# lppllppl920/EndoscopyDepthEstimation-Pytorch

Hardware: AMD Instinct MI355X
Metric: train frame-pairs/sec at 256x320 bs=8 (higher is better)
Workload: dtype f32

## Files before the change

endoscopydepthestimation-pytorch_amd/csrc/dgrad_wino_kernels.h:

```cpp
#pragma once

#include "dgrad_block_kernels.h"

namespace endo {

constexpr int kWinoDgradSlice = 16 * 12 * 16;
constexpr int kWinoDgradMaxLayers = 48;

struct WinoDgradTable {
    int layers;
    int start[kWinoDgradMaxLayers + 1];
    int cin[kWinoDgradMaxLayers];
    int groups[kWinoDgradMaxLayers];
    int64_t w_off[kWinoDgradMaxLayers];
    int64_t u_off[kWinoDgradMaxLayers];
};

static __global__ void __launch_bounds__(256) dgrad_wino_weights_kernel(const WinoDgradTable t, const float* __restrict__ params, float* __restrict__ u,
                                                                 int layout1_blocks = 0) {
    const int total = t.start[t.layers];
    for (int item = blockIdx.x * blockDim.x + threadIdx.x; item < total; item += gridDim.x * blockDim.x) {
        int l = 0;
        while (item >= t.start[l + 1]) ++l;
        const int e = item - t.start[l];
        const int j = e & 15, c = (e >> 4) % 12, grp = (e >> 4) / 12;
        const int ci = grp * 16 + j;
        float g[3][3];
#pragma unroll
        for (int a = 0; a < 3; ++a)
#pragma unroll
            for (int b = 0; b < 3; ++b) g[a][b] = 0.f;
        if (ci < t.cin[l]) {
            const float* src = params + t.w_off[l] + (static_cast<int64_t>(c) * t.cin[l] + ci) * 9;
#pragma unroll
            for (int a = 0; a < 3; ++a)
#pragma unroll
                for (int b = 0; b < 3; ++b) g[a][b] = src[(2 - a) * 3 + (2 - b)];
        }
        float h[4][3];
#pragma unroll
        for (int b = 0; b < 3; ++b) {
            h[0][b] = g[0][b];
            h[1][b] = 0.5f * (g[0][b] + g[1][b] + g[2][b]);
            h[2][b] = 0.5f * (g[0][b] - g[1][b] + g[2][b]);
            h[3][b] = g[2][b];
        }
        if ((layout1_blocks >> (l >> 2)) & 1) {
            float* dst = u + t.u_off[l] + static_cast<int64_t>(grp) * kWinoDgradSlice + (c * 64 + j) * 4;
#pragma unroll
            for (int a = 0; a < 4; ++a)
                *reinterpret_cast<f32x4*>(dst + a * 64) = f32x4{h[a][0], 0.5f * (h[a][0] + h[a][1] + h[a][2]), 0.5f * (h[a][0] - h[a][1] + h[a][2]), h[a][2]};
            continue;
        }
        float* dst = u + t.u_off[l] + static_cast<int64_t>(grp) * kWinoDgradSlice + c * 16 + j;
#pragma unroll
        for (int a = 0; a < 4; ++a) {
            dst[(4 * a + 0) * 192] = h[a][0];
            dst[(4 * a + 1) * 192] = 0.5f * (h[a][0] + h[a][1] + h[a][2]);
            dst[(4 * a + 2) * 192] = 0.5f * (h[a][0] - h[a][1] + h[a][2]);
            dst[(4 * a + 3) * 192] = h[a][2];
        }
    }
}

template <int NL>
struct DgradWino8Geom {
    static constexpr int kThreads = 512;
    static constexpr int kTileX = 32, kTileY = 8;
    static constexpr int kRows = kTileY + 2, kCols = kTileX + 2;
    static constexpr int kPlane = kRows * kCols;
    static constexpr int kCS = 352;
    static_assert(kCS >= kPlane && kCS % 64 == 32, "dY map stride");
    static constexpr int kU = kWinoDgradSlice;
    static constexpr int kUUnits = kU / 4;
    static constexpr int kRed = 4 * 16 * 2;
    static constexpr size_t kBytes = sizeof(float) * (NL * 12 * kCS + 2 * 2 * kU + 2 * 2 * kRed);
    static_assert(kBytes <= 160 * 1024, "one block per CU");
};

template <int NL, int EXP = 0>
__global__ void __launch_bounds__(512, 2) dgrad_wino8_kernel(const DgradBlockParams p0, const float* __restrict__ u0, const float* __restrict__ u1,
                                                             const float* __restrict__ u2, const float* __restrict__ u3) {
    using G = DgradWino8Geom<NL>;
    typedef float f32x2 __attribute__((ext_vector_type(2)));
    const int grp = p0.group_n > 0 ? blockIdx.z / p0.group_n : 0;
    const int n = blockIdx.z - grp * p0.group_n;
    const DgradBlockParams& p = p0;
    const int64_t grp_off = grp * p0.gs;
    extern __shared__ __attribute__((aligned(16))) float smem[];
    float* s_g = smem;
    float* s_u = s_g + NL * 12 * G::kCS;
    float* s_red = s_u + 4 * G::kU;

    const int tid = threadIdx.x;
    const int lane = tid & 63;
    const int wave = __builtin_amdgcn_readfirstlane(tid >> 6);
    const int half = wave >> 2, w4 = wave & 3;
    const int th = tid & 255;
    const int li = lane & 15;
    const int lk = lane >> 4;
    const int tile = (gridDim.x & 7) == 0 ? xcd_remap(blockIdx.x, gridDim.x) : blockIdx.x;
    const int x0 = (tile % p.tiles_x) * G::kTileX;
    const int y0 = (tile / p.tiles_x) * G::kTileY;
    const int px = x0 + 8 * lk;
    const int py = y0 + 2 * w4;
    const int ngroups = p.count / 16;
    const int g_per = (ngroups + gridDim.y - 1) / gridDim.y;
    const int g_begin = blockIdx.y * g_per;
    const int g_end = min(ngroups, g_begin + g_per);
    if (g_begin >= g_end) return;
    const int npairs = (g_end - g_begin + 1) / 2;
    const int nsteps = npairs * NL;
    const float* const u_layer[4] = {u0, u1, u2, u3};

    {
        int goff = 0;
        bool ok = false;
        if (tid < G::kPlane) {
            const int ry = tid / G::kCols, rx = tid - ry * G::kCols;
            const int gy = y0 - 1 + ry, gx = x0 - 1 + rx;
            if (gy >= 0 && gy < p.h && gx >= 0 && gx < p.w) { ok = true; goff = gy * p.g_w + gx; }
        }
        const float* g_n = p.g + grp_off + n * p.g_ns;
        const int e0 = wave * 64;
        if (e0 < G::kPlane) {
            for (int c = 0; c < NL * 12; ++c) {
                const float* src = ok ? g_n + static_cast<int64_t>(c) * p.g_cs + goff : g_pad_consts + 4;
                if (e0 + lane < G::kPlane) __builtin_amdgcn_global_load_lds((gptr_t)src, (lptr_t)(s_g + c * G::kCS + e0), 4, 0, 0);
            }
        }
    }

    auto step_group = [&](int step) { return g_begin + 2 * (step / NL) + half; };
    auto issue_weights = [&](int step, int buf) {
        const int gq = step_group(step), l = step % NL;
        if (gq >= g_end) return;
        const float* src = u_layer[l] + static_cast<int64_t>(gq) * G::kU + 4 * th;
        float* dst = s_u + (half * 2 + buf) * G::kU + w4 * 256;
#pragma unroll
        for (int k = 0; k < 3; ++k)
            __builtin_amdgcn_global_load_lds((gptr_t)(src + k * 1024), (lptr_t)(dst + k * 1024), 16, 0, 0);
    };

    const float* x_n = p.x + grp_off + n * p.ns;
    float* out_n = p.out + grp_off + n * p.ns;
    f32x4 xc[2][2], dc[2][2], total[2][2];
#pragma unroll
    for (int r = 0; r < 2; ++r)
#pragma unroll
        for (int hh = 0; hh < 2; ++hh) total[r][hh] = f32x4{0.f, 0.f, 0.f, 0.f};
    issue_weights(0, 0);
    asm volatile("s_waitcnt vmcnt(0)" ::: "memory");
    __syncthreads();

    for (int step = 0; step < nsteps; ++step) {
        const int buf = step & 1;
        const int gq = step_group(step), l = step % NL;
        const bool active = gq < g_end;
        const bool last_layer = (l == NL - 1);
        const int co = gq * 16 + li;
        float scale = 0.f, beta = 0.f, mean = 0.f, rstd = 0.f;
        if (active) {
            if (l == 0) {
#pragma unroll
                for (int r = 0; r < 2; ++r)
#pragma unroll
                    for (int hh = 0; hh < 2; ++hh) {
                        const int64_t o = static_cast<int64_t>(co) * p.cs + static_cast<int64_t>(py + r) * p.w + px + 4 * hh;
                        if constexpr ((EXP & 1) != 0) {
                            xc[r][hh] = f32x4{0.1f * lane, 0.2f, -0.3f, 0.4f}; dc[r][hh] = f32x4{0.f, 0.f, 0.f, 0.f};
                        } else {
                            xc[r][hh] = *reinterpret_cast<const f32x4*>(x_n + o);
                            dc[r][hh] = co >= p.acc_from ? *reinterpret_cast<const f32x4*>(out_n + o) : f32x4{0.f, 0.f, 0.f, 0.f};
                        }
                    }
            }
            mean = p.saved[l][grp_off + 2 * co]; rstd = p.saved[l][grp_off + 2 * co + 1];
            scale = p.gamma[l][co] * rstd;
            beta = p.beta[l][co];
        }
        if (step + 1 < nsteps && (!(EXP & 8) || step == 0)) issue_weights(step + 1, buf ^ 1);
        if (active) {
            f32x4 acc[16];
            const float* ub = s_u + (half * 2 + buf) * G::kU;
#pragma unroll
            for (int quad = 0; quad < 3; ++quad) {
                const float* a_base = s_g + (l * 12 + quad * 4 + lk) * G::kCS + (2 * w4) * G::kCols + 2 * li;
                const float* b_base = ub + (quad * 4 + lk) * 16 + li;
                f32x2 lo[4], hi[4];
#pragma unroll
                for (int row = 0; row < 4; ++row) {
                    lo[row] = *reinterpret_cast<const f32x2*>(a_base + row * G::kCols);
                    hi[row] = *reinterpret_cast<const f32x2*>(a_base + row * G::kCols + 2);
                }
                f32x2 tl[4], th2[4];
                tl[0] = lo[0] - lo[2]; th2[0] = hi[0] - hi[2];
                tl[1] = lo[1] + lo[2]; th2[1] = hi[1] + hi[2];
                tl[2] = lo[2] - lo[1]; th2[2] = hi[2] - hi[1];
                tl[3] = lo[1] - lo[3]; th2[3] = hi[1] - hi[3];
#pragma unroll
                for (int a = 0; a < 4; ++a) {
                    const float c0 = tl[a][0], c1 = tl[a][1], c2 = th2[a][0], c3 = th2[a][1];
                    float v0 = c0 - c2, v1 = c1 + c2, v2 = c2 - c1, v3 = c1 - c3;
                    if constexpr ((EXP & 64) != 0) { v0 = lo[a][0]; v1 = lo[a][1]; v2 = hi[a][0]; v3 = hi[a][1]; }
                    const float b0 = b_base[(4 * a + 0) * 192], b1 = b_base[(4 * a + 1) * 192];
                    const float b2 = b_base[(4 * a + 2) * 192], b3 = b_base[(4 * a + 3) * 192];
                    if constexpr ((EXP & 32) != 0) {
                        if (quad == 0) {
                            acc[4 * a + 0] = f32x4{v0 * b0, 0.f, 0.f, 0.f}; acc[4 * a + 1] = f32x4{v1 * b1, 0.f, 0.f, 0.f};
                            acc[4 * a + 2] = f32x4{v2 * b2, 0.f, 0.f, 0.f}; acc[4 * a + 3] = f32x4{v3 * b3, 0.f, 0.f, 0.f};
                        } else {
                            acc[4 * a + 0][quad] += v0 * b0; acc[4 * a + 1][quad] += v1 * b1;
                            acc[4 * a + 2][quad] += v2 * b2; acc[4 * a + 3][quad] += v3 * b3;
                        }
                    } else
                    if (quad == 0) {
                        const f32x4 zero = {0.f, 0.f, 0.f, 0.f};
                        acc[4 * a + 0] = __builtin_amdgcn_mfma_f32_16x16x4f32(v0, b0, zero, 0, 0, 0);
                        acc[4 * a + 1] = __builtin_amdgcn_mfma_f32_16x16x4f32(v1, b1, zero, 0, 0, 0);
                        acc[4 * a + 2] = __builtin_amdgcn_mfma_f32_16x16x4f32(v2, b2, zero, 0, 0, 0);
                        acc[4 * a + 3] = __builtin_amdgcn_mfma_f32_16x16x4f32(v3, b3, zero, 0, 0, 0);
                    } else {
                        acc[4 * a + 0] = __builtin_amdgcn_mfma_f32_16x16x4f32(v0, b0, acc[4 * a + 0], 0, 0, 0);
                        acc[4 * a + 1] = __builtin_amdgcn_mfma_f32_16x16x4f32(v1, b1, acc[4 * a + 1], 0, 0, 0);
                        acc[4 * a + 2] = __builtin_amdgcn_mfma_f32_16x16x4f32(v2, b2, acc[4 * a + 2], 0, 0, 0);
                        acc[4 * a + 3] = __builtin_amdgcn_mfma_f32_16x16x4f32(v3, b3, acc[4 * a + 3], 0, 0, 0);
                    }
                }
            }
            float s1 = 0.f, s2 = 0.f;
            if constexpr ((EXP & 128) != 0) {
#pragma unroll
                for (int r = 0; r < 2; ++r)
#pragma unroll
                    for (int hh = 0; hh < 2; ++hh)
#pragma unroll
                        for (int k = 0; k < 4; ++k)
                            total[r][hh][k] += acc[4 * (2 * r + hh) + k][0] + acc[4 * (2 * r + hh) + k][1] + acc[4 * (2 * r + hh) + k][2] + acc[4 * (2 * r + hh) + k][3] + xc[r][hh][k] * scale;
                s1 = total[0][0][0]; s2 = mean + beta;
            } else
#pragma unroll
            for (int e = 0; e < 4; ++e) {
                float u0r[4], u1r[4];
#pragma unroll
                for (int c = 0; c < 4; ++c) {
                    const float m0 = acc[c][e], m1 = acc[4 + c][e], m2 = acc[8 + c][e], m3 = acc[12 + c][e];
                    u0r[c] = m0 + m1 + m2;
                    u1r[c] = m1 - m2 - m3;
                }
                const float d[2][2] = {{u0r[0] + u0r[1] + u0r[2], u0r[1] - u0r[2] - u0r[3]},
                                       {u1r[0] + u1r[1] + u1r[2], u1r[1] - u1r[2] - u1r[3]}};
#pragma unroll
                for (int r = 0; r < 2; ++r)
#pragma unroll
                    for (int cx = 0; cx < 2; ++cx) {
                        const int hh = e >> 1, k = 2 * (e & 1) + cx;
                        const float xcen = xc[r][hh][k] - mean;
                        const float z = fmaf(xcen, scale, beta);
                        const float dz = z > 0.f ? d[r][cx] : 0.f;
                        s1 += dz;
                        s2 = fmaf(dz, xcen, s2);
                        total[r][hh][k] = fmaf(dz, scale, total[r][hh][k]);
                    }
            }
            if (last_layer) {
#pragma unroll
                for (int r = 0; r < 2; ++r)
#pragma unroll
                    for (int hh = 0; hh < 2; ++hh) {
                        f32x4 o = dc[r][hh];
#pragma unroll
                        for (int k = 0; k < 4; ++k) o[k] += total[r][hh][k];
                        if constexpr ((EXP & 2) != 0) asm volatile("" ::"v"(o[0]), "v"(o[1]), "v"(o[2]), "v"(o[3]));
                        else
                        *reinterpret_cast<f32x4*>(out_n + static_cast<int64_t>(co) * p.cs + static_cast<int64_t>(py + r) * p.w + px + 4 * hh) = o;
                        total[r][hh] = f32x4{0.f, 0.f, 0.f, 0.f};
                    }
            }
            s2 *= rstd;
            s1 += __shfl_xor(s1, 16, 64); s1 += __shfl_xor(s1, 32, 64);
            s2 += __shfl_xor(s2, 16, 64); s2 += __shfl_xor(s2, 32, 64);
            if (lk == 0) {
                float* red = s_red + (buf * 2 + half) * G::kRed;
                red[(w4 * 16 + li) * 2] = s1;
                red[(w4 * 16 + li) * 2 + 1] = s2;
            }
        }
        if (!(EXP & 16) || step + 1 >= nsteps) {
            asm volatile("s_waitcnt vmcnt(0)" ::: "memory");
            __syncthreads();
        }
        if (!(EXP & 4) && active && th < 32) {
            const int j = th >> 1, which = th & 1;
            const int cj = gq * 16 + j;
            const float* red = s_red + (buf * 2 + half) * G::kRed;
            double t = 0.0;
            for (int wv = 0; wv < 4; ++wv) t += static_cast<double>(red[(wv * 16 + j) * 2 + which]);
            atomicAdd(p.scratch[l] + bn_slot_offset(p.slot_stride) + grp_off / 2 + 2 * cj + which, t);
        }
    }
}

inline bool dgrad_wino_ok(const DgradBlockParams& p) {
    return dgrad_block_ok(p) && (p.w % 32 == 0) && (p.h % 8 == 0) && (p.count % 16 == 0) && p.count >= 32;
}

template <int NL, int EXP = 0>
inline int launch_dgrad_wino8(DgradBlockParams p, const float* const (&u)[4], hipStream_t stream) {
    using G = DgradWino8Geom<NL>;
    p.tiles_x = p.w / G::kTileX;
    const int tiles_y = p.h / G::kTileY;
    return launch_dyn(dgrad_wino8_kernel<NL, EXP>, dim3(p.tiles_x * tiles_y, 1, p.n), G::kThreads, G::kBytes, stream, p, u[0], u[1], u[2], u[3]);
}

}
```

endoscopydepthestimation-pytorch_amd/csrc/net.hip:

```cpp
#include <new>
#include <vector>

#include "dgrad_kernels.h"
#include "dgrad_block_kernels.h"
#include "dgrad_newmap_kernels.h"
#include "td_dgrad_kernels.h"
#include "td_fwd_kernels.h"
#include "wgrad_taps_kernels.h"
#include "wgrad1x1_kernels.h"
#include "wgrad_nsplit_kernels.h"
#include "wgrad_f34_kernels.h"
#include "wgrad_subpix_kernels.h"
#include "wino_fwd_kernels.h"
#include "wino4_fwd_kernels.h"
#include "dgrad_wino_kernels.h"
#include "dgrad_wino3_kernels.h"


namespace endo {

int run_dgrad_wino3_nl4(const DgradBlockParams& p, const float* const* u, hipStream_t stream);
bool dgrad_wino3p_applies(const DgradBlockParams& p);
int run_dgrad_wino3p_nl4(const DgradBlockParams& p, const float* const* u, int blocks, double* fw_parts, int* blocks_used, hipStream_t stream);

constexpr int kGrowth = 12;
constexpr int kLayers = 4;
constexpr int kFirst = 48;
constexpr int kLevels = 5;
constexpr int kNew = kGrowth * kLayers;
constexpr float kBnEps = 1.0e-5f;
constexpr float kBnMomentum = 0.1f;
constexpr int kSideStreamFromLevel = 0;

struct ConvP { int64_t w, b; int cout, cin, ks; int64_t u; int64_t ud; };
struct BnP { int64_t g, b; int c; int64_t run; int64_t saved; };

struct Table {
    ConvP first, final_;
    ConvP down_conv[kLevels][kLayers], td_conv[kLevels], bott_conv[kLayers], tu_conv[kLevels], up_conv[kLevels][kLayers];
    BnP down_bn[kLevels][kLayers], td_bn[kLevels], bott_bn[kLayers], up_bn[kLevels][kLayers];
    std::vector<int64_t> param_offsets;
    std::vector<BnP*> bn_order;
    int64_t param_floats = 0, bn_floats = 0, bn_width_total = 0;
    WinoWeightTable wino;
    WinoWeightTable wino4;
    int64_t wino4_floats = 0;
    int64_t wino_floats = 0;
    WinoDgradTable wino_dgrad;
    int64_t wino_dgrad_floats = 0;
};

inline int down_in(int level) { return kFirst + kNew * level; }
inline int level_channels(int level) { return level < kLevels ? 144 + down_in(level) : 288 + kNew; }

static const Table& table() {
    static Table* t = [] {
        Table* tb = new Table();
        int64_t off = 0;
        auto conv = [&](ConvP& c, int cout, int cin, int ks) {
            c.cout = cout; c.cin = cin; c.ks = ks; c.u = -1; c.ud = -1;
            c.w = off; tb->param_offsets.push_back(off); off += static_cast<int64_t>(cout) * cin * ks * ks;
            c.b = off; tb->param_offsets.push_back(off); off += cout;
        };
        int64_t run = 0, saved = 0;
        auto bn = [&](BnP& b, int c) {
            b.c = c;
            b.g = off; tb->param_offsets.push_back(off); off += c;
            b.b = off; tb->param_offsets.push_back(off); off += c;
            b.run = run; run += 2 * c;
            b.saved = saved; saved += c;
            tb->bn_order.push_back(&b);
        };
        conv(tb->first, kFirst, 3, 3);
        for (int l = 0; l < kLevels; ++l)
            for (int j = 0; j < kLayers; ++j) { bn(tb->down_bn[l][j], down_in(l) + kGrowth * j); conv(tb->down_conv[l][j], kGrowth, down_in(l) + kGrowth * j, 3); }
        for (int l = 0; l < kLevels; ++l) { bn(tb->td_bn[l], down_in(l) + kNew); conv(tb->td_conv[l], down_in(l) + kNew, down_in(l) + kNew, 1); }
        for (int j = 0; j < kLayers; ++j) { bn(tb->bott_bn[j], 288 + kGrowth * j); conv(tb->bott_conv[j], kGrowth, 288 + kGrowth * j, 3); }
        for (int i = 0; i < kLevels; ++i) conv(tb->tu_conv[i], kNew, kNew, 3);
        for (int i = 0; i < kLevels; ++i) {
            const int l = kLevels - 1 - i;
            for (int j = 0; j < kLayers; ++j) { const int cin = 96 + down_in(l) + kGrowth * j; bn(tb->up_bn[i][j], cin); conv(tb->up_conv[i][j], kGrowth, cin, 3); }
        }
        conv(tb->final_, 1, 192, 1);
        tb->param_floats = off;
        tb->bn_floats = run;
        tb->bn_width_total = saved;
        {
            WinoWeightTable& wt = tb->wino;
            wt.layers = 0; wt.start[0] = 0;
            int64_t uoff = 0;
            auto add = [&](ConvP& c) {
                const int l = wt.layers++;
                c.u = uoff;
                wt.cin[l] = c.cin; wt.cout[l] = c.cout; wt.w_off[l] = c.w; wt.u_off[l] = uoff;
                wt.start[l + 1] = wt.start[l] + c.cin * 16;
                uoff += static_cast<int64_t>(c.cin) * kWinoUStride;
            };
            for (int l = 0; l < kLevels; ++l) for (int j = 0; j < kLayers; ++j) add(tb->down_conv[l][j]);
            for (int j = 0; j < kLayers; ++j) add(tb->bott_conv[j]);
            for (int i = 0; i < kLevels; ++i) for (int j = 0; j < kLayers; ++j) add(tb->up_conv[i][j]);
            tb->wino_floats = uoff;
            tb->wino4 = wt;
            int64_t u4 = 0;
            for (int l = 0; l < wt.layers; ++l) { tb->wino4.u_off[l] = u4; u4 += static_cast<int64_t>(wt.cin[l]) * kW4UStride; }
            tb->wino4_floats = u4;
        }
        {
            WinoDgradTable& wd = tb->wino_dgrad;
            wd.layers = 0; wd.start[0] = 0;
            int64_t uoff = 0;
            auto add = [&](ConvP& c, int base) {
                const int l = wd.layers++;
                c.ud = uoff;
                wd.cin[l] = c.cin; wd.groups[l] = base / 16; wd.w_off[l] = c.w; wd.u_off[l] = uoff;
                wd.start[l + 1] = wd.start[l] + 16 * wd.groups[l] * 12;
                uoff += static_cast<int64_t>(wd.groups[l]) * kWinoDgradSlice;
            };
            for (int l = 0; l < kLevels; ++l) for (int j = 0; j < kLayers; ++j) add(tb->down_conv[l][j], down_in(l));
            for (int j = 0; j < kLayers; ++j) add(tb->bott_conv[j], 288);
            for (int i = 0; i < kLevels; ++i) for (int j = 0; j < kLayers; ++j) add(tb->up_conv[i][j], 96 + down_in(kLevels - 1 - i));
            tb->wino_dgrad_floats = uoff;
        }
        return tb;
    }();
    return *t;
}

}

using namespace endo;

namespace endo { struct FwdPlan; struct BwdPlan; }

struct endo_net {
    int n, h, w;
    int groups;
    int64_t gs;
    struct Level { int h, w, t; int64_t plane; int64_t act, grad; int64_t sums; int64_t pq; } lv[kLevels + 1];
    int64_t pre_off;
    int64_t saved_off;
    int64_t idx_off[kLevels];
    int64_t sums_off;
    int64_t sums_bytes;
    int64_t tape_floats;
    int64_t partial_off;
    int64_t wino_off;
    int64_t wino4_off;
    int64_t pq_off;
    int64_t pq_floats;
    int64_t scratch_off;
    int64_t scratch_bytes;
    int64_t slot_stride;
    int64_t wg_scratch_off;
    int64_t tuw_scratch_off;
    int64_t wd_off;
    int64_t gplane_off;
    int64_t bias_parts_off;
    int64_t fw_parts_off;
    int64_t bias_parts_floats;
    int64_t gradws_floats;
    hipStream_t wstream;
    hipEvent_t ev_fork, ev_join;
    int opt[ENDO_OPT_COUNT];
    FwdPlan* last_fwd;
    BwdPlan* last_bwd;
};

namespace endo {


constexpr int kBiasPartChannels = 2048;
constexpr int kBiasPartLaunches = 64;
constexpr int kFwPartBlocks = 512;
struct BiasReduceTable {
    int n;
    struct Entry { const float* parts; float* bias; int count; int nparts; } e[kBiasPartLaunches];
};
struct BiasParts {
    BiasReduceTable table;
    int64_t used;
};

struct BnFin4 {
    const double* scratch[4];
    const float* saved[4];
    const float* gamma[4];
    float* ggamma[4];
    float* gbeta[4];
};

__global__ void __launch_bounds__(256) prep_dy_kernel(float* __restrict__ dbuf, const float* __restrict__ x, int64_t ns, int plane,
                                                      const float* __restrict__ pq_p, const float* __restrict__ pq_q,
                                                      float* bias_grad, int group_n, int64_t gs, const BnFin4 fin, int nl,
                                                      double count, int training, int64_t slot_stride,
                                                      const float* __restrict__ vg, const float* __restrict__ vw, float* __restrict__ parts) {
    __shared__ double scratch[4];
    const int c = blockIdx.y;
    const int grp = blockIdx.z / group_n, n = blockIdx.z - grp * group_n;
    float pc = pq_p[grp * gs + c], qc = pq_q[grp * gs + c];
    if (nl > 0) {
        const int64_t go = grp * gs;
        double dp = 0.0, dq = 0.0;
#pragma unroll
        for (int j = 0; j < 4; ++j) {
            if (j >= nl) break;
            const double s1 = bn_slot_sum(fin.scratch[j] + go / 2 + 2 * c, slot_stride);
            const double s2 = bn_slot_sum(fin.scratch[j] + go / 2 + 2 * c + 1, slot_stride);
            if (blockIdx.x == 0 && n == 0 && threadIdx.x == 0) {
                atomicAdd(fin.ggamma[j] + c, static_cast<float>(s2));
                atomicAdd(fin.gbeta[j] + c, static_cast<float>(s1));
            }
            if (training) {
                const double mean = fin.saved[j][go + 2 * c], rstd = fin.saved[j][go + 2 * c + 1];
                const double scale = fin.gamma[j][c] * rstd;
                const double k = scale * rstd * s2 / count;
                dp += static_cast<double>(static_cast<float>(-k));
                dq += static_cast<double>(static_cast<float>(-scale * s1 / count + k * mean));
            }
        }
        pc += static_cast<float>(dp);
        qc += static_cast<float>(dq);
    }
    const int64_t base = grp * gs + n * ns + static_cast<int64_t>(c) * plane;
    const float* vg_n = vg ? vg + grp * gs + static_cast<int64_t>(n) * plane : nullptr;
    const float wf = vg ? vw[c] : 0.f;
    float part = 0.f;
    if ((plane & 3) == 0 && !vg_n) {
        const int stride = gridDim.x * blockDim.x * 4;
        int i = (blockIdx.x * blockDim.x + threadIdx.x) * 4;
        for (; i + stride < plane; i += 2 * stride) {
            f32x4 g0 = *reinterpret_cast<const f32x4*>(dbuf + base + i);
            f32x4 g1 = *reinterpret_cast<const f32x4*>(dbuf + base + i + stride);
            const f32x4 x0 = *reinterpret_cast<const f32x4*>(x + base + i);
            const f32x4 x1 = *reinterpret_cast<const f32x4*>(x + base + i + stride);
#pragma unroll
            for (int e = 0; e < 4; ++e) { g0[e] += fmaf(pc, x0[e], qc); part += g0[e]; }
#pragma unroll
            for (int e = 0; e < 4; ++e) { g1[e] += fmaf(pc, x1[e], qc); part += g1[e]; }
            *reinterpret_cast<f32x4*>(dbuf + base + i) = g0;
            *reinterpret_cast<f32x4*>(dbuf + base + i + stride) = g1;
        }
        for (; i < plane; i += stride) {
            f32x4 g = *reinterpret_cast<const f32x4*>(dbuf + base + i);
            const f32x4 xv = *reinterpret_cast<const f32x4*>(x + base + i);
#pragma unroll
            for (int e = 0; e < 4; ++e) { g[e] += fmaf(pc, xv[e], qc); part += g[e]; }
            *reinterpret_cast<f32x4*>(dbuf + base + i) = g;
        }
    } else if ((plane & 3) == 0) {
        for (int i = (blockIdx.x * blockDim.x + threadIdx.x) * 4; i < plane; i += gridDim.x * blockDim.x * 4) {
            f32x4 g;
            if (vg_n) {
                const f32x4 gv = *reinterpret_cast<const f32x4*>(vg_n + i);
                g = f32x4{gv[0] * wf, gv[1] * wf, gv[2] * wf, gv[3] * wf};
            } else {
                g = *reinterpret_cast<const f32x4*>(dbuf + base + i);
            }
            const f32x4 xv = *reinterpret_cast<const f32x4*>(x + base + i);
#pragma unroll
            for (int e = 0; e < 4; ++e) { g[e] += fmaf(pc, xv[e], qc); part += g[e]; }
            *reinterpret_cast<f32x4*>(dbuf + base + i) = g;
        }
    } else {
        for (int i = blockIdx.x * blockDim.x + threadIdx.x; i < plane; i += gridDim.x * blockDim.x) {
            const float g = (vg_n ? vg_n[i] * wf : dbuf[base + i]) + fmaf(pc, x[base + i], qc);
            dbuf[base + i] = g;
            part += g;
        }
    }
    const int lane = threadIdx.x & 63, wave = threadIdx.x >> 6;
    double v = wave_sum(static_cast<double>(part));
    if (lane == 0) scratch[wave] = v;
    __syncthreads();
    if (threadIdx.x == 0 && bias_grad) {
        const float t = static_cast<float>(scratch[0] + scratch[1] + scratch[2] + scratch[3]);
        if (parts) parts[(static_cast<int64_t>(c) * gridDim.z + blockIdx.z) * gridDim.x + blockIdx.x] = t;
        else atomicAdd(bias_grad + c, t);
    }
}

__global__ void __launch_bounds__(256) bias_reduce_kernel(const BiasReduceTable tb) {
    const BiasReduceTable::Entry& e = tb.e[blockIdx.x];
    const int lane = threadIdx.x & 63, wave = threadIdx.x >> 6;
    for (int c = blockIdx.y * 4 + wave; c < e.count; c += gridDim.y * 4) {
        const float* src = e.parts + static_cast<int64_t>(c) * e.nparts;
        double t = 0.0;
        for (int i = lane; i < e.nparts; i += 64) t += static_cast<double>(src[i]);
        t = wave_sum(t);
        if (lane == 0) e.bias[c] += static_cast<float>(t);
    }
}

__global__ void bn_bwd_finalize_kernel(const double* __restrict__ scratch, const float* __restrict__ saved,
                                       const float* __restrict__ gamma, float* __restrict__ ggamma, float* __restrict__ gbeta,
                                       float* __restrict__ pq_p, float* __restrict__ pq_q, int c_count, double count, int training,
                                       int64_t gs, int64_t slot_stride) {
    scratch += blockIdx.y * (gs / 2); saved += blockIdx.y * gs; pq_p += blockIdx.y * gs; pq_q += blockIdx.y * gs;
    for (int c = blockIdx.x * blockDim.x + threadIdx.x; c < c_count; c += gridDim.x * blockDim.x) {
        const double s1 = bn_slot_sum(scratch + 2 * c, slot_stride), s2 = bn_slot_sum(scratch + 2 * c + 1, slot_stride);
        atomicAdd(ggamma + c, static_cast<float>(s2));
        atomicAdd(gbeta + c, static_cast<float>(s1));
        if (training) {
            const double mean = saved[2 * c], rstd = saved[2 * c + 1];
            const double scale = gamma[c] * rstd;
            const double k = scale * rstd * s2 / count;
            pq_p[c] += static_cast<float>(-k);
            pq_q[c] += static_cast<float>(-scale * s1 / count + k * mean);
        }
    }
}

__global__ void bn_bwd_finalize4_kernel(const BnFin4 a, int nl, float* __restrict__ pq_p, float* __restrict__ pq_q, int c_count, double count,
                                        int training, int64_t gs, int64_t slot_stride) {
    const int64_t go = blockIdx.y * gs;
    pq_p += go; pq_q += go;
    for (int c = blockIdx.x * blockDim.x + threadIdx.x; c < c_count; c += gridDim.x * blockDim.x) {
        double dp = 0.0, dq = 0.0;
#pragma unroll
        for (int j = 0; j < 4; ++j) {
            if (j >= nl) break;
            const double s1 = bn_slot_sum(a.scratch[j] + go / 2 + 2 * c, slot_stride);
            const double s2 = bn_slot_sum(a.scratch[j] + go / 2 + 2 * c + 1, slot_stride);
            atomicAdd(a.ggamma[j] + c, static_cast<float>(s2));
            atomicAdd(a.gbeta[j] + c, static_cast<float>(s1));
            if (training) {
                const double mean = a.saved[j][go + 2 * c], rstd = a.saved[j][go + 2 * c + 1];
                const double scale = a.gamma[j][c] * rstd;
                const double k = scale * rstd * s2 / count;
                dp += static_cast<double>(static_cast<float>(-k));
                dq += static_cast<double>(static_cast<float>(-scale * s1 / count + k * mean));
            }
        }
        if (training) {
            pq_p[c] += static_cast<float>(dp);
            pq_q[c] += static_cast<float>(dq);
        }
    }
}

__global__ void tu_phase_weights_kernel(const float* __restrict__ w, int cout, int cin, float* __restrict__ out) {
    constexpr int kPhW = 2 * 12 * 16 + 16;
    const int total = 2 * cin * 2 * 12 * 16;
    for (int i = blockIdx.x * blockDim.x + threadIdx.x; i < total; i += gridDim.x * blockDim.x) {
        const int lane16 = i & 15;
        const int slot = (i >> 4) % 12;
        const int t = (i / (16 * 12)) & 1;
        const int ci = (i / (16 * 12 * 2)) % cin;
        const int a = i / (16 * 12 * 2 * cin);
        int ctap, tile;
        if (slot < 3) { ctap = 0; tile = slot; } else if (slot < 9) { ctap = 1; tile = slot - 3; } else { ctap = 2; tile = slot - 9 + 3; }
        const int b = tile / 3, co = (tile % 3) * 16 + lane16;
        float v = 0.f;
        if (co < cout) {
            const float* src = w + (static_cast<int64_t>(co) * cin + ci) * 9;
            const int ky0 = a == 0 ? (t == 0 ? 0 : 1) : (t == 0 ? 0 : 2), ky1 = a == 0 ? (t == 0 ? 0 : 2) : (t == 0 ? 1 : 2);
            int kx0, kx1;
            if (b == 0) { kx0 = ctap == 0 ? 0 : 1; kx1 = ctap == 0 ? 0 : 2; }
            else { kx0 = ctap == 1 ? 0 : 2; kx1 = ctap == 1 ? 1 : 2; }
            for (int ky = ky0; ky <= ky1; ++ky)
                for (int kx = kx0; kx <= kx1; ++kx) v += src[ky * 3 + kx];
        }
        out[(static_cast<int64_t>(a) * cin + ci) * kPhW + (t * 12 + slot) * 16 + lane16] = v;
    }
}

__global__ void tu_subpix_dgrad_weights_kernel(const float* __restrict__ w, int cout, int cin, float* __restrict__ out) {
    const int pitch = 4 * cin + 16;
    const int total = 4 * cout * 4 * cin;
    for (int i = blockIdx.x * blockDim.x + threadIdx.x; i < total; i += gridDim.x * blockDim.x) {
        const int ci = i % cin;
        const int tap = (i / cin) & 3;
        const int co = (i / (4 * cin)) % cout;
        const int ph = i / (4 * cin * cout);
        const int alpha = ph >> 1, beta = ph & 1, tyi = tap >> 1, txi = tap & 1;
        const int ky0 = alpha == 0 ? (tyi == 0 ? 1 : 0) : (tyi == 0 ? 2 : 0), ky1 = alpha == 0 ? (tyi == 0 ? 2 : 0) : (tyi == 0 ? 2 : 1);
        const int kx0 = beta == 0 ? (txi == 0 ? 1 : 0) : (txi == 0 ? 2 : 0), kx1 = beta == 0 ? (txi == 0 ? 2 : 0) : (txi == 0 ? 2 : 1);
        const float* src = w + (static_cast<int64_t>(co) * cin + ci) * 9;
        float v = 0.f;
        for (int ky = ky0; ky <= ky1; ++ky)
            for (int kx = kx0; kx <= kx1; ++kx) v += src[ky * 3 + kx];
        out[static_cast<int64_t>(ph * cout + co) * pitch + tap * cin + ci] = v;
    }
}

__global__ void __launch_bounds__(256) finalize_partial_kernel(const float* __restrict__ partial, int64_t split_stride, int ksplit,
                                                               int64_t pns, int plane, const float* __restrict__ bias,
                                                               float* __restrict__ out, int64_t out_ns, double* out_sums,
                                                               int group_n, int64_t gs) {
    __shared__ double scratch[2 * 4];
    const int c = blockIdx.y;
    const int grp = blockIdx.z / group_n, n = blockIdx.z - grp * group_n;
    partial += grp * gs; out += grp * gs;
    if (out_sums) out_sums += grp * (gs / 2);
    const float b = bias[c];
    float part[2] = {0.f, 0.f};
    for (int i = blockIdx.x * blockDim.x + threadIdx.x; i < plane; i += gridDim.x * blockDim.x) {
        float v = b;
        for (int s = 0; s < ksplit; ++s) v += partial[s * split_stride + n * pns + static_cast<int64_t>(c) * plane + i];
        out[n * out_ns + static_cast<int64_t>(c) * plane + i] = v;
        part[0] += v;
        part[1] += v * v;
    }
    if (out_sums) block_sum_atomic<2>(part, out_sums + 2 * c, scratch);
}

__global__ void __launch_bounds__(256) final_fwd_kernel(const float* __restrict__ u, int64_t ns, int plane, int cin,
                                                        const float* __restrict__ wgt, const float* __restrict__ bias,
                                                        float* __restrict__ pre, float* __restrict__ out, int group_n, int64_t gs, int c_first) {
    __shared__ float s_w[192];
    for (int c = threadIdx.x; c < cin; c += blockDim.x) s_w[c] = wgt[c];
    __syncthreads();
    const int grp = blockIdx.y / group_n, n = blockIdx.y - grp * group_n;
    u += grp * gs;
    if (pre) pre += grp * gs;
    out += static_cast<int64_t>(grp) * group_n * plane;
    const bool vec = (plane & 3) == 0;
    if (vec) {
        for (int i = (blockIdx.x * blockDim.x + threadIdx.x) * 4; i < plane; i += gridDim.x * blockDim.x * 4) {
            f32x4 acc = {0.f, 0.f, 0.f, 0.f};
            if (c_first > 0) acc = *reinterpret_cast<const f32x4*>(pre + static_cast<int64_t>(n) * plane + i);
            const float* src = u + n * ns + i;
            for (int c = c_first; c < cin; ++c) {
                const f32x4 v = *reinterpret_cast<const f32x4*>(src + static_cast<int64_t>(c) * plane);
                const float wc = s_w[c];
                acc[0] = fmaf(v[0], wc, acc[0]); acc[1] = fmaf(v[1], wc, acc[1]);
                acc[2] = fmaf(v[2], wc, acc[2]); acc[3] = fmaf(v[3], wc, acc[3]);
            }
            const float b = bias[0];
            f32x4 o;
            for (int e = 0; e < 4; ++e) { acc[e] += b; o[e] = fabsf(acc[e]); }
            if (pre) *reinterpret_cast<f32x4*>(pre + static_cast<int64_t>(n) * plane + i) = acc;
            *reinterpret_cast<f32x4*>(out + static_cast<int64_t>(n) * plane + i) = o;
        }
    } else {
        for (int i = blockIdx.x * blockDim.x + threadIdx.x; i < plane; i += gridDim.x * blockDim.x) {
            float acc = c_first > 0 ? pre[static_cast<int64_t>(n) * plane + i] : 0.f;
            for (int c = c_first; c < cin; ++c) acc = fmaf(u[n * ns + static_cast<int64_t>(c) * plane + i], s_w[c], acc);
            acc += bias[0];
            if (pre) pre[static_cast<int64_t>(n) * plane + i] = acc;
            out[static_cast<int64_t>(n) * plane + i] = fabsf(acc);
        }
    }
}

__device__ __forceinline__ float sign_of(float v) { return v > 0.f ? 1.f : (v < 0.f ? -1.f : 0.f); }

__global__ void __launch_bounds__(256) final_g_kernel(const float* __restrict__ gout, const float* __restrict__ pre, float* __restrict__ g,
                                                      int plane, int group_n, int64_t gs) {
    const int grp = blockIdx.y / group_n, n = blockIdx.y - grp * group_n;
    gout += static_cast<int64_t>(blockIdx.y) * plane; pre += grp * gs + static_cast<int64_t>(n) * plane; g += grp * gs + static_cast<int64_t>(n) * plane;
    for (int i = blockIdx.x * blockDim.x + threadIdx.x; i < plane; i += gridDim.x * blockDim.x) g[i] = gout[i] * sign_of(pre[i]);
}

__global__ void __launch_bounds__(256) final_bwd_data_kernel(const float* __restrict__ gout, const float* __restrict__ pre,
                                                             const float* __restrict__ wgt, float* __restrict__ dbuf,
                                                             int64_t ns, int plane, int cin, int group_n, int64_t gs, int c_first) {
    __shared__ float s_w[192];
    for (int c = threadIdx.x; c < cin; c += blockDim.x) s_w[c] = wgt[c];
    __syncthreads();
    const int grp = blockIdx.y / group_n, n = blockIdx.y - grp * group_n;
    gout += static_cast<int64_t>(grp) * group_n * plane; pre += grp * gs; dbuf += grp * gs;
    for (int i = blockIdx.x * blockDim.x + threadIdx.x; i < plane; i += gridDim.x * blockDim.x) {
        const float g = gout[static_cast<int64_t>(n) * plane + i] * sign_of(pre[static_cast<int64_t>(n) * plane + i]);
        for (int c = c_first; c < cin; ++c) dbuf[n * ns + static_cast<int64_t>(c) * plane + i] = g * s_w[c];
    }
}

__global__ void __launch_bounds__(256) final_bwd_weight_kernel(const float* __restrict__ gout, const float* __restrict__ pre,
                                                               const float* __restrict__ u, int64_t ns, int plane, int cin,
                                                               int group_n, int64_t gs, float* __restrict__ gw, float* __restrict__ gb, int c_first) {
    __shared__ double scratch[4];
    const int c = c_first + blockIdx.x;
    const int grp = blockIdx.z / group_n, n = blockIdx.z - grp * group_n;
    const float* gp = gout + static_cast<int64_t>(blockIdx.z) * plane;
    const float* pp = pre + grp * gs + static_cast<int64_t>(n) * plane;
    const float* up = u + grp * gs + n * ns + static_cast<int64_t>(c < cin ? c : 0) * plane;
    float part = 0.f, part2 = 0.f;
    if ((plane & 3) == 0) {
        const int stride = gridDim.y * blockDim.x * 4;
        for (int i = (blockIdx.y * blockDim.x + threadIdx.x) * 4; i < plane; i += stride) {
            const f32x4 gv = *reinterpret_cast<const f32x4*>(gp + i);
            const f32x4 pv = *reinterpret_cast<const f32x4*>(pp + i);
            f32x4 uv = {1.f, 1.f, 1.f, 1.f};
            if (c < cin) uv = *reinterpret_cast<const f32x4*>(up + i);
            part += gv[0] * sign_of(pv[0]) * uv[0] + gv[1] * sign_of(pv[1]) * uv[1];
            part2 += gv[2] * sign_of(pv[2]) * uv[2] + gv[3] * sign_of(pv[3]) * uv[3];
        }
    } else {
        for (int i = blockIdx.y * blockDim.x + threadIdx.x; i < plane; i += gridDim.y * blockDim.x)
            part += gp[i] * sign_of(pp[i]) * (c < cin ? up[i] : 1.f);
    }
    const int lane = threadIdx.x & 63, wave = threadIdx.x >> 6;
    double v = wave_sum(static_cast<double>(part + part2));
    if (lane == 0) scratch[wave] = v;
    __syncthreads();
    if (threadIdx.x == 0) {
        const float t = static_cast<float>(scratch[0] + scratch[1] + scratch[2] + scratch[3]);
        if (c < cin) atomicAdd(gw + c, t); else atomicAdd(gb, t);
    }
}

__global__ void __launch_bounds__(64) final_w_reduce_kernel(const double* __restrict__ parts, int nblocks, int count, float* __restrict__ gw) {
    const int c = blockIdx.x;
    double t = 0.0;
    for (int b = threadIdx.x; b < nblocks; b += 64) t += parts[static_cast<int64_t>(b) * count + c];
    t = wave_sum(t);
    if (threadIdx.x == 0) atomicAdd(gw + c, static_cast<float>(t));
}

constexpr int kBlocks = 2 * kLevels + 1, kDense = kBlocks * kLayers;

enum class DenseFwd { Wino4, Wino2_32x16, Wino2_32x8, SplitK, Direct32x8, Direct16x8, DirectAuto };
struct FwdPlan {
    struct Dense {
        DenseFwd form;
        int ksplit;
        bool chunk_weights;
    } dense[kDense];
    bool bf16;
    bool wino4_weights;
    bool fuse_final;
    bool td_persistent[kLevels];
    bool tu_subpix[kLevels];
};

enum class NewMap { Bf16, Persistent, Vec16, Dword };
enum class BasePass { Block8, Block8Bf16, Wino3, Wino3Persistent, Wino8 };
enum class DenseWgrad { F34, NSplit, Taps, Direct };
enum class TdDgrad { Persistent, Runs128, Dma, Staged };
enum class TuWgrad { Subpix, Taps, Direct };
enum class TuDgrad { Subpix32x8, Subpix16x8, Subpix16x4, Plain };
enum class FirstWgrad { F34Prep, F34, Taps, Direct };
struct BwdPlan {
    struct Block {
        bool fused;
        NewMap newmap[kLayers];
        BasePass base;
        bool wino3_layout;
    } block[kBlocks];
    DenseWgrad wgrad[kDense];
    bool td_wgrad_dma[kLevels];
    TdDgrad td_dgrad[kLevels];
    TuWgrad tu_wgrad[kLevels];
    TuDgrad tu_dgrad[kLevels];
    int overlap;
    bool bf16_wgrad, bf16_dgrad;
    bool dgrad_weights;
    bool use_virt;
    bool virt_base;
    bool virt_base_w;
    int materialise;
    int c_first;
    FirstWgrad first;
};

struct Ctx {
    const endo_net* net;
    const float* params;
    float* bn_running;
    float* tape;
    float* grads;
    float* gradws;
    int training;
    hipStream_t stream;
    BiasParts* bias_parts = nullptr;
    const float* x = nullptr;
    const FwdPlan* fwd = nullptr;
    const BwdPlan* bwd = nullptr;

    int nt() const { return net->n * net->groups; }
    int fork_wgrad(Ctx& side, int level) const {
        side = *this;
        if (!net->wstream || !bwd->overlap || level < kSideStreamFromLevel) return 0;
        ENDO_CHECK(hipEventRecord(net->ev_fork, stream));
        ENDO_CHECK(hipStreamWaitEvent(net->wstream, net->ev_fork, 0));
        side.stream = net->wstream;
        return 0;
    }
    float* act(int level) const { return tape + net->lv[level].act; }
    float* gbuf(int level) const { return gradws + net->lv[level].grad; }
    double* sums(int level) const { return reinterpret_cast<double*>(reinterpret_cast<char*>(tape) + net->sums_off) + net->lv[level].sums; }
    double* out_sums(int level, int channel) const { return training ? sums(level) + 2 * channel : nullptr; }
    float* saved(const BnP& b) const { return tape + net->saved_off + 2 * b.saved; }
    double* scratch(const BnP& b) const { return reinterpret_cast<double*>(reinterpret_cast<char*>(gradws) + net->scratch_off) + 2 * b.saved; }
    float* pq_p(int level) const { return gradws + net->pq_off + 2 * net->lv[level].pq; }
    float* pq_q(int level) const { return pq_p(level) + net->lv[level].t; }
    uint8_t* idx(int level) const { return reinterpret_cast<uint8_t*>(tape) + net->idx_off[level]; }
};

static void fill_bn_in(const Ctx& c, ConvParams& p, const BnP& b, int level, int ic0) {
    const auto& lv = c.net->lv[level];
    p.in_sums = c.sums(level) + 2 * ic0;
    p.gamma = c.params + b.g;
    p.beta = c.params + b.b;
    p.running_mean = c.bn_running + b.run;
    p.running_var = c.bn_running + b.run + b.c;
    p.saved = c.tape ? c.saved(b) : nullptr;
    p.count = static_cast<double>(c.net->n) * lv.h * lv.w;
    p.eps = kBnEps;
    p.momentum = kBnMomentum;
    p.training = c.training;
}

static void fill_in(const Ctx& c, ConvParams& p, const float* base, int level, int ic0, int cin) {
    const auto& lv = c.net->lv[level];
    p.in = base + ic0 * lv.plane;
    p.in_ns = lv.t * lv.plane;
    p.in_cs = static_cast<int>(lv.plane);
    p.in_w = lv.w;
    p.cin = cin;
}

static void fill_out(const Ctx& c, ConvParams& p, float* base, int level, int oc0, int cout) {
    const auto& lv = c.net->lv[level];
    p.out = base + oc0 * lv.plane;
    p.out_ns = lv.t * lv.plane;
    p.out_cs = static_cast<int>(lv.plane);
    p.out_w = lv.w;
    p.cout = cout;
}

static void fill_grid(const Ctx& c, ConvParams& p, int level) {
    const auto& lv = c.net->lv[level];
    p.n = c.nt(); p.h = lv.h; p.w = lv.w;
    p.group_n = c.net->n; p.gs = c.net->gs; p.in_gs = c.net->gs; p.out_gs = c.net->gs;
}

static double conv_flops(const endo_net* net, int level, int cin, int cout, int ks) {
    return 2.0 * net->n * net->groups * net->lv[level].plane * cin * cout * ks * ks;
}

static void default_options(int (&opt)[ENDO_OPT_COUNT]) {
    opt[ENDO_OPT_WINO_FWD] = 5;
    opt[ENDO_OPT_WINO_DGRAD] = 3;
    opt[ENDO_OPT_DGRAD_VEC] = 2;
    opt[ENDO_OPT_WINO_MIN_TILES] = 1024;
    opt[ENDO_OPT_MFMA_BF16] = 0;
    opt[ENDO_OPT_WGRAD_OVERLAP] = 1;
    opt[ENDO_OPT_WGRAD_F34] = 1;
    opt[ENDO_OPT_FINAL_VIRTUAL] = 1;
    opt[ENDO_OPT_TD_PERSIST] = 3;
    opt[ENDO_OPT_CHIP_DIVISOR] = 1;
}
static long chip_divisor(const endo_net* net) { const int d = net->opt[ENDO_OPT_CHIP_DIVISOR]; return d < 1 ? 1 : d; }
static int persistent_cus(const endo_net* net) { const int cus = static_cast<int>(device_cu_count() / chip_divisor(net)); return cus < 1 ? 1 : cus; }
static int bf16_mask(const int* opt) { const int v = opt[ENDO_OPT_MFMA_BF16]; return v == 1 ? 7 : (v >> 1); }

struct DenseBlock { int level, ic0, c0; const BnP* bn; const ConvP* cv; bool base_overwrite; };
static DenseBlock dense_block(int b) {
    const Table& tb = table();
    if (b < kLevels) return {b, 48, down_in(b), tb.down_bn[b], tb.down_conv[b], false};
    if (b == kLevels) return {kLevels, 0, 288, tb.bott_bn, tb.bott_conv, true};
    const int i = b - kLevels - 1, l = kLevels - 1 - i;
    return {l, 0, 96 + down_in(l), tb.up_bn[i], tb.up_conv[i], l > 0};
}
static long tile_count(const Ctx& c, int level, int tx, int ty) {
    const auto& lv = c.net->lv[level];
    return static_cast<long>((lv.w + tx - 1) / tx) * ((lv.h + ty - 1) / ty) * c.nt() * chip_divisor(c.net);
}

static ConvParams dense_fwd_params(const Ctx& c, const DenseBlock& k, int j, DenseFwd form) {
    const ConvP& cv = k.cv[j];
    const int oc0 = k.ic0 + k.c0 + kGrowth * j;
    ConvParams p{};
    fill_grid(c, p, k.level);
    fill_in(c, p, c.act(k.level), k.level, k.ic0, cv.cin);
    fill_bn_in(c, p, k.bn[j], k.level, k.ic0);
    p.wgt = c.params + cv.w; p.bias = c.params + cv.b; p.w_cout = cv.cout; p.w_cin = cv.cin;
    fill_out(c, p, c.act(k.level), k.level, oc0, cv.cout);
    p.out_sums = c.out_sums(k.level, oc0);
    if (form == DenseFwd::Wino4) p.wgt = c.tape + c.net->wino4_off + cv.u / kWinoUStride * kW4UStride;
    if (form == DenseFwd::Wino2_32x16 || form == DenseFwd::Wino2_32x8) p.wgt = c.tape + c.net->wino_off + cv.u;
    return p;
}

static ConvParams td_fwd_params(const Ctx& c, int level) {
    const BnP& b = table().td_bn[level];
    const ConvP& cv = table().td_conv[level];
    const int next = level + 1;
    const int oc0 = next < kLevels ? 48 : 0;
    ConvParams p{};
    fill_grid(c, p, level);
    fill_in(c, p, c.act(level), level, 48, cv.cin);
    fill_bn_in(c, p, b, level, 48);
    p.wgt = c.params + cv.w; p.bias = c.params + cv.b; p.w_cout = cv.cout; p.w_cin = cv.cin;
    fill_out(c, p, c.act(next), next, oc0, cv.cout);
    p.out_idx = c.idx(level);
    p.idx_ns = static_cast<int64_t>(cv.cout) * c.net->lv[next].plane;
    p.out_sums = c.out_sums(next, oc0);
    return p;
}

static FwdPlan plan_fwd(const Ctx& c) {
    const int* opt = c.net->opt;
    const int mode = opt[ENDO_OPT_WINO_FWD];
    const long min_tiles = opt[ENDO_OPT_WINO_MIN_TILES];
    FwdPlan pl{};
    pl.bf16 = (bf16_mask(opt) & 2) != 0;
    pl.wino4_weights = !pl.bf16 && mode == 5;
    for (int b = 0; b < kBlocks; ++b) {
        const DenseBlock k = dense_block(b);
        const long t64x16 = tile_count(c, k.level, 64, 16), t32x16 = tile_count(c, k.level, 32, 16), t32x8 = tile_count(c, k.level, 32, 8);
        const long t16x16 = tile_count(c, k.level, 16, 16), t16x8 = tile_count(c, k.level, 16, 8);
        const bool big = t32x16 >= min_tiles, small = t32x8 >= (min_tiles * 3) / 4;
        const bool wino4_tiles = mode == 5 && !pl.bf16 && 2 * t64x16 >= min_tiles;
        const bool wino2_tiles = mode != 0 && !pl.bf16 && (big || small);
        for (int j = 0; j < kLayers; ++j) {
            FwdPlan::Dense& d = pl.dense[b * kLayers + j];
            const int nchunks = (k.cv[j].cin + 15) / 16;
            d.chunk_weights = !pl.bf16 && !wino4_tiles && !wino2_tiles;
            if (wino4_tiles && wino4_fwd_ok(dense_fwd_params(c, k, j, DenseFwd::Wino4))) {
                d.form = DenseFwd::Wino4;
            } else if (wino2_tiles && wino_fwd_ok(dense_fwd_params(c, k, j, DenseFwd::Wino2_32x16))) {
                d.form = big ? DenseFwd::Wino2_32x16 : DenseFwd::Wino2_32x8;
            } else if (t32x16 < 512 && t16x16 < 384 && t16x8 < 512 && nchunks >= 4) {
                int want = static_cast<int>(((t16x8 < 256 ? 512 : 768) + t16x8 - 1) / t16x8);
                if (want > nchunks) want = nchunks;
                const int per = (nchunks + want - 1) / want;
                d.form = DenseFwd::SplitK;
                d.ksplit = (nchunks + per - 1) / per;
            } else {
                d.form = (t32x16 < 1024 && t32x8 >= 1024) ? DenseFwd::Direct32x8
                       : (t32x16 < 1024 && t16x8 >= 768) ? DenseFwd::Direct16x8 : DenseFwd::DirectAuto;
            }
        }
    }
    pl.fuse_final = opt[ENDO_OPT_FINAL_VIRTUAL] && pl.dense[kDense - 1].form == DenseFwd::Wino4;
    for (int l = 0; l < kLevels; ++l) {
        pl.td_persistent[l] = (opt[ENDO_OPT_TD_PERSIST] & 2) && !pl.bf16 && c.training && td_fwd_ok(td_fwd_params(c, l));
        const ConvP& tu = table().tu_conv[kLevels - 1 - l];
        pl.tu_subpix[l] = c.net->lv[l + 1].w % 4 == 0 && tu.cout == kNew && tu.cin % 4 == 0;
    }
    return pl;
}

static int dense_fwd(const Ctx& c, int b, int j) {
    const DenseBlock k = dense_block(b);
    const FwdPlan::Dense& d = c.fwd->dense[b * kLayers + j];
    const ConvP& cv = k.cv[j];
    const auto& lv = c.net->lv[k.level];
    const int oc0 = k.ic0 + k.c0 + kGrowth * j;
    ConvParams p = dense_fwd_params(c, k, j, d.form);
    ProfScope prof(kProfConv3x3Dense, c.stream, conv_flops(c.net, k.level, cv.cin, cv.cout, 3),
                   4.0 * c.nt() * lv.plane * (cv.cin + cv.cout));
    const float* chunk_weights = d.chunk_weights ? c.tape + c.net->wino_off + cv.u : nullptr;
    const bool bf16 = c.fwd->bf16;
    switch (d.form) {
        case DenseFwd::Wino4:
            if (c.fwd->fuse_final && b == kBlocks - 1 && j == kLayers - 1) { p.fin_w = c.params + table().final_.w + k.ic0; p.fin_out = c.tape + c.net->pre_off; }
            return launch_wino4_fwd(p, c.stream);
        case DenseFwd::Wino2_32x16:
            return launch_wino_fwd<2, 4, 2>(p, c.stream);
        case DenseFwd::Wino2_32x8:
            return launch_wino_fwd<1, 4, 3>(p, c.stream);
        case DenseFwd::SplitK: {
            float* partial = c.tape + c.net->partial_off;
            p.ksplit = d.ksplit;
            p.split_stride = static_cast<int64_t>(c.net->n) * cv.cout * lv.plane;
            p.out = partial; p.out_ns = static_cast<int64_t>(cv.cout) * lv.plane;
            p.bias = nullptr; p.out_sums = nullptr;
            p.wgt_chunks = chunk_weights;
            int rc = bf16 ? launch_conv_dma<3, 16, 1, IN_BNRELU, EPI_FWD, 1, 2, 2, 1, 1>(p, c.stream)
                          : launch_conv_dma<3, 16, 1, IN_BNRELU, EPI_FWD, 1, 2, 2, 1>(p, c.stream);
            if (rc) return rc;
            int bx = static_cast<int>((lv.plane + 255) / 256);
            bx = bx > 8 ? 8 : bx;
            finalize_partial_kernel<<<dim3(bx, cv.cout, c.nt()), 256, 0, c.stream>>>(
                partial, p.split_stride, d.ksplit, p.out_ns, static_cast<int>(lv.plane), c.params + cv.b, c.act(k.level) + oc0 * lv.plane,
                lv.t * lv.plane, c.out_sums(k.level, oc0), c.net->n, c.net->gs);
            ENDO_LAUNCH_CHECK();
            return 0;
        }
        case DenseFwd::Direct32x8:
            return bf16 ? launch_conv_dma<3, 4, 1, IN_BNRELU, EPI_FWD, 2, 4, 2, 1, 1>(p, c.stream) : launch_conv_dma<3, 4, 1, IN_BNRELU, EPI_FWD, 2, 4, 2, 1>(p, c.stream);
        case DenseFwd::Direct16x8:
            return bf16 ? launch_conv_dma<3, 8, 1, IN_BNRELU, EPI_FWD, 1, 2, 2, 1, 1>(p, c.stream) : launch_conv_dma<3, 8, 1, IN_BNRELU, EPI_FWD, 1, 2, 2, 1>(p, c.stream);
        case DenseFwd::DirectAuto:
            if (bf16) return launch_conv_dma_auto<3, 4, 1, IN_BNRELU, EPI_FWD, 8, 2, 1, 1>(p, c.stream);
            p.wgt_chunks = chunk_weights;
            return launch_conv_dma_auto<3, 4, 1, IN_BNRELU, EPI_FWD, 8, 2, 1>(p, c.stream);
    }
    return ENDO_E_BADARG;
}

static int td_fwd(const Ctx& c, int level) {
    const ConvP& cv = table().td_conv[level];
    const ConvParams p = td_fwd_params(c, level);
    ProfScope prof(kProfConv1x1Pool, c.stream, conv_flops(c.net, level, cv.cin, cv.cout, 1),
                   4.0 * c.nt() * c.net->lv[level].plane * (cv.cin + cv.cout / 4.0));
    if (c.fwd->td_persistent[level]) return launch_td_fwd(p, persistent_cus(c.net), c.stream);
    if (c.fwd->bf16) return launch_conv_dma_auto<1, 8, 3, IN_BNRELU, EPI_FWD_POOL, 4, 2, 1, 1>(p, c.stream);
    return launch_conv_dma_auto<1, 8, 3, IN_BNRELU, EPI_FWD_POOL, 4>(p, c.stream);
}

static int tu_fwd(const Ctx& c, int level, int src_level, int src_c0, const ConvP& cv) {
    ProfScope prof(kProfConv3x3Up, c.stream, conv_flops(c.net, level, cv.cin, cv.cout, 3),
                   4.0 * c.nt() * c.net->lv[level].plane * (cv.cin / 4.0 + cv.cout));
    if (c.fwd->tu_subpix[level]) {
        float* w3 = c.tape + c.net->partial_off;
        tu_phase_weights_kernel<<<(2 * cv.cin * 384 + 255) / 256, 256, 0, c.stream>>>(c.params + cv.w, cv.cout, cv.cin, w3);
        ENDO_LAUNCH_CHECK();
        ConvParams p{};
        fill_grid(c, p, src_level);
        fill_in(c, p, c.act(src_level), src_level, src_c0, cv.cin);
        p.wgt = w3; p.w_cout = 2 * cv.cout; p.w_cin = cv.cin;
        p.bias = c.params + cv.b;
        fill_out(c, p, c.act(level), level, 0, cv.cout);
        p.out_sums = c.out_sums(level, 0);
        return launch_conv_dma_vec<3, 4, 6, IN_PLAIN, EPI_FWD, 2, 4, 2, 1, 4, 0, 0, 2>(p, c.stream);
    }
    ConvParams p{};
    fill_grid(c, p, level);
    fill_in(c, p, c.act(src_level), src_level, src_c0, cv.cin);
    p.wgt = c.params + cv.w; p.bias = c.params + cv.b; p.w_cout = cv.cout; p.w_cin = cv.cin;
    fill_out(c, p, c.act(level), level, 0, cv.cout);
    p.out_sums = c.out_sums(level, 0);
    return launch_conv_dma_auto<3, 4, 3, IN_UPSAMPLE, EPI_FWD>(p, c.stream);
}

struct FinalVirt { const float* vg; const float* vw; float* gw; };

static int prep_dy(const Ctx& c, int level, int c0, int count, float* bias_grad, const BnFin4* fin = nullptr, int nl = 0, const FinalVirt* fv = nullptr) {
    const auto& lv = c.net->lv[level];
    BnFin4 none{};
    int bx = static_cast<int>((lv.plane + 4095) / 4096);
    bx = bx < 1 ? 1 : (bx > 32 ? 32 : bx);
    float* parts = nullptr;
    if (bias_grad && c.bias_parts) {
        BiasParts& bp = *c.bias_parts;
        const int64_t need = static_cast<int64_t>(count) * c.nt() * bx;
        if (bp.table.n >= kBiasPartLaunches || bp.used + need > c.net->bias_parts_floats) return ENDO_E_UNSUPPORTED;
        parts = c.gradws + c.net->bias_parts_off + bp.used;
        bp.table.e[bp.table.n++] = {parts, bias_grad, count, c.nt() * bx};
        bp.used += need;
    }
    ProfScope prof(kProfSmall, c.stream, 0.0, 12.0 * c.nt() * lv.plane * count);
    prep_dy_kernel<<<dim3(bx, count, c.nt()), 256, 0, c.stream>>>(c.gbuf(level) + c0 * lv.plane, c.act(level) + c0 * lv.plane,
                                                                     lv.t * lv.plane, static_cast<int>(lv.plane), c.pq_p(level) + c0,
                                                                     c.pq_q(level) + c0, bias_grad, c.net->n, c.net->gs, fin ? *fin : none, fin ? nl : 0,
                                                                     static_cast<double>(c.net->n) * lv.h * lv.w, c.training, c.net->slot_stride,
                                                                     fv ? fv->vg : nullptr, fv ? fv->vw + c0 : nullptr, parts);
    ENDO_LAUNCH_CHECK();
    return 0;
}

static int bn_finalize(const Ctx& c, const BnP& b, int level, int ic0, int first = 0, int count = -1) {
    const auto& lv = c.net->lv[level];
    if (count < 0) count = b.c - first;
    if (count <= 0) return 0;
    ProfScope prof(kProfSmall, c.stream, 0.0, 0.0);
    bn_bwd_finalize_kernel<<<dim3((count + 127) / 128, c.net->groups), 128, 0, c.stream>>>(c.scratch(b) + 2 * first, c.saved(b) + 2 * first, c.params + b.g + first,
                                                                       c.grads + b.g + first, c.grads + b.b + first,
                                                                       c.pq_p(level) + ic0 + first, c.pq_q(level) + ic0 + first, count,
                                                                       static_cast<double>(c.net->n) * lv.h * lv.w, c.training, c.net->gs, c.net->slot_stride);
    ENDO_LAUNCH_CHECK();
    return 0;
}

static void fill_wgrad_grid(const Ctx& c, WgradParams& p, int level) {
    const auto& lv = c.net->lv[level];
    p.n = c.nt(); p.h = lv.h; p.w = lv.w;
    p.group_n = c.net->n; p.gs = c.net->gs; p.in_gs = c.net->gs;
    p.tiles_x = (lv.w + kWgTileX - 1) / kWgTileX;
    p.tiles_y = (lv.h + kWgTileY - 1) / kWgTileY;
}

static WgradParams dense_wgrad_params(const Ctx& c, const DenseBlock& k, int j) {
    const auto& lv = c.net->lv[k.level];
    const BnP& b = k.bn[j];
    const ConvP& cv = k.cv[j];
    const int oc0 = k.ic0 + k.c0 + kGrowth * j;
    WgradParams p{};
    fill_wgrad_grid(c, p, k.level);
    p.in = c.act(k.level) + k.ic0 * lv.plane; p.in_ns = lv.t * lv.plane; p.in_cs = static_cast<int>(lv.plane); p.in_w = lv.w; p.cin = cv.cin;
    p.saved = c.saved(b); p.gamma = c.params + b.g; p.beta = c.params + b.b;
    p.dy = c.gbuf(k.level) + oc0 * lv.plane; p.dy_ns = lv.t * lv.plane; p.dy_cs = static_cast<int>(lv.plane); p.dy_w = lv.w; p.cout = cv.cout;
    p.dw = c.grads + cv.w;
    return p;
}

static void fill_dgrad_block(const Ctx& c, DgradBlockParams& p, int level) {
    const auto& lv = c.net->lv[level];
    p.n = c.nt(); p.h = lv.h; p.w = lv.w;
    p.group_n = c.net->n; p.gs = c.net->gs; p.slot_stride = c.net->slot_stride;
    p.g_ns = lv.t * lv.plane; p.g_cs = static_cast<int>(lv.plane); p.g_w = lv.w;
    p.ns = lv.t * lv.plane; p.cs = static_cast<int>(lv.plane);
}

static DgradBlockParams newmap_params(const Ctx& c, const DenseBlock& k, int j, BnFin4* a = nullptr) {
    const auto& lv = c.net->lv[k.level];
    const int nl = kLayers - j;
    const int t0 = k.c0 + kGrowth * (j - 1);
    DgradBlockParams p{};
    fill_dgrad_block(c, p, k.level);
    p.g = c.gbuf(k.level) + (k.ic0 + k.c0 + kGrowth * j) * lv.plane;
    p.x = c.act(k.level) + (k.ic0 + t0) * lv.plane;
    p.out = c.gbuf(k.level) + (k.ic0 + t0) * lv.plane;
    p.count = kGrowth;
    p.acc_from = 0;
    p.w_ci_off = t0;
    for (int l = 0; l < nl; ++l) {
        const BnP& b = k.bn[j + l];
        p.wgt[l] = c.params + k.cv[j + l].w; p.w_cin[l] = k.cv[j + l].cin;
        p.saved[l] = c.saved(b) + 2 * t0; p.gamma[l] = c.params + b.g + t0; p.beta[l] = c.params + b.b + t0;
        p.scratch[l] = c.scratch(b) + 2 * t0;
        if (a) { a->scratch[l] = p.scratch[l]; a->saved[l] = p.saved[l]; a->gamma[l] = p.gamma[l]; a->ggamma[l] = c.grads + b.g + t0; a->gbeta[l] = c.grads + b.b + t0; }
    }
    return p;
}

static DgradBlockParams base_pass_params(const Ctx& c, const DenseBlock& k) {
    const auto& lv = c.net->lv[k.level];
    DgradBlockParams p{};
    fill_dgrad_block(c, p, k.level);
    p.g = c.gbuf(k.level) + (k.ic0 + k.c0) * lv.plane;
    p.x = c.act(k.level) + k.ic0 * lv.plane;
    p.out = c.gbuf(k.level) + k.ic0 * lv.plane;
    p.count = k.c0;
    p.acc_from = k.base_overwrite ? k.c0 : 0;
    p.w_ci_off = 0;
    for (int j = 0; j < kLayers; ++j) {
        p.wgt[j] = c.params + k.cv[j].w; p.w_cin[j] = k.cv[j].cin;
        p.saved[j] = c.saved(k.bn[j]); p.gamma[j] = c.params + k.bn[j].g; p.beta[j] = c.params + k.bn[j].b;
        p.scratch[j] = c.scratch(k.bn[j]);
    }
    return p;
}

static WgradParams td_wgrad_params(const Ctx& c, int level) {
    const BnP& b = table().td_bn[level];
    const ConvP& cv = table().td_conv[level];
    const int next = level + 1, oc0 = next < kLevels ? 48 : 0;
    const auto& lv = c.net->lv[level];
    const auto& nx = c.net->lv[next];
    WgradParams p{};
    fill_wgrad_grid(c, p, level);
    p.in = c.act(level) + 48 * lv.plane; p.in_ns = lv.t * lv.plane; p.in_cs = static_cast<int>(lv.plane); p.in_w = lv.w; p.cin = cv.cin;
    p.saved = c.saved(b); p.gamma = c.params + b.g; p.beta = c.params + b.b;
    p.dy = c.gbuf(next) + oc0 * nx.plane; p.dy_ns = nx.t * nx.plane; p.dy_cs = static_cast<int>(nx.plane); p.dy_w = nx.w; p.cout = cv.cout;
    p.dy_idx = c.idx(level); p.idx_ns = static_cast<int64_t>(cv.cout) * nx.plane;
    p.dw = c.grads + cv.w;
    return p;
}

static ConvParams td_dgrad_params(const Ctx& c, int level) {
    const BnP& b = table().td_bn[level];
    const ConvP& cv = table().td_conv[level];
    const int next = level + 1, oc0 = next < kLevels ? 48 : 0;
    const auto& lv = c.net->lv[level];
    ConvParams p{};
    fill_grid(c, p, level);
    fill_in(c, p, c.gbuf(next), next, oc0, cv.cout);
    p.in_idx = c.idx(level); p.idx_ns = static_cast<int64_t>(cv.cout) * c.net->lv[next].plane;
    p.wgt = c.params + cv.w; p.w_cout = cv.cout; p.w_cin = cv.cin;
    fill_out(c, p, c.gbuf(level), level, 48, cv.cin);
    p.x = c.act(level) + 48 * lv.plane; p.x_ns = lv.t * lv.plane; p.x_cs = static_cast<int>(lv.plane);
    p.bn_saved = c.saved(b); p.bn_gamma = c.params + b.g; p.bn_beta = c.params + b.b;
    p.bn_scratch = c.scratch(b); p.bn_slot_stride = c.net->slot_stride;
    p.acc_from = 0;
    return p;
}

static WgradParams tu_wgrad_params(const Ctx& c, int level, bool subpix) {
    const ConvP& cv = table().tu_conv[kLevels - 1 - level];
    const int src_level = level + 1, src_c0 = src_level == kLevels ? 288 : 96 + down_in(src_level);
    const auto& lv = c.net->lv[level];
    const auto& sv = c.net->lv[src_level];
    WgradParams p{};
    fill_wgrad_grid(c, p, level);
    p.in = c.act(src_level) + src_c0 * sv.plane; p.in_ns = sv.t * sv.plane; p.in_cs = static_cast<int>(sv.plane); p.in_w = sv.w; p.cin = cv.cin;
    p.dy = c.gbuf(level); p.dy_ns = lv.t * lv.plane; p.dy_cs = static_cast<int>(lv.plane); p.dy_w = lv.w; p.cout = cv.cout;
    p.dw = c.grads + cv.w;
    if (subpix) { p.h = sv.h; p.w = sv.w; }
    return p;
}

static WgradParams first_wgrad_params(const Ctx& c) {
    const auto& lv = c.net->lv[0];
    WgradParams p{};
    fill_wgrad_grid(c, p, 0);
    p.in = c.x; p.in_ns = 3 * lv.plane; p.in_cs = static_cast<int>(lv.plane); p.in_w = lv.w; p.cin = 3;
    p.in_gs = c.net->n * p.in_ns;
    p.dy = c.gbuf(0) + 48 * lv.plane; p.dy_ns = lv.t * lv.plane; p.dy_cs = static_cast<int>(lv.plane); p.dy_w = lv.w; p.cout = kFirst;
    p.dw = c.grads + table().first.w;
    return p;
}

static BwdPlan plan_bwd(const Ctx& c) {
    const int* opt = c.net->opt;
    const int wino_dgrad = opt[ENDO_OPT_WINO_DGRAD];
    const long min_tiles = opt[ENDO_OPT_WINO_MIN_TILES];
    BwdPlan pl{};
    pl.overlap = opt[ENDO_OPT_WGRAD_OVERLAP];
    pl.bf16_wgrad = (bf16_mask(opt) & 1) != 0;
    pl.bf16_dgrad = (bf16_mask(opt) & 4) != 0;
    const bool f34 = opt[ENDO_OPT_WGRAD_F34] && !pl.bf16_wgrad;
    const long fill = chip_divisor(c.net);
    const long f34_min_tiles = (min_tiles / 4 + fill - 1) / fill;
    pl.dgrad_weights = wino_dgrad != 0 && !pl.bf16_dgrad;
    for (int b = 0; b < kBlocks; ++b) {
        const DenseBlock k = dense_block(b);
        const auto& lv = c.net->lv[k.level];
        BwdPlan::Block& bl = pl.block[b];
        const DgradBlockParams base = base_pass_params(c, k);
        bl.fused = dgrad_block_ok(base);
        const long wtiles = static_cast<long>(lv.w / 32) * (lv.h / 8) * c.nt() * fill;
        if (pl.bf16_dgrad) bl.base = BasePass::Block8Bf16;
        else if (wino_dgrad != 0 && dgrad_wino_ok(base) && wtiles >= min_tiles)
            bl.base = !((wino_dgrad == 1 || wino_dgrad == 3) && dgrad_wino3_ok(base)) ? BasePass::Wino8
                    : (wino_dgrad == 3 && dgrad_wino3p_applies(base)) ? BasePass::Wino3Persistent : BasePass::Wino3;
        else bl.base = BasePass::Block8;
        bl.wino3_layout = bl.base == BasePass::Wino3 || bl.base == BasePass::Wino3Persistent;
        for (int j = 1; j < kLayers; ++j) {
            const DgradBlockParams p = newmap_params(c, k, j);
            const bool vec = dgrad_block_vec_ok(p);
            bl.newmap[j] = (pl.bf16_dgrad && vec) ? NewMap::Bf16 : (vec && opt[ENDO_OPT_DGRAD_VEC] >= 2 && dgrad_newmap_ok(p)) ? NewMap::Persistent
                         : (vec && opt[ENDO_OPT_DGRAD_VEC] != 0) ? NewMap::Vec16 : NewMap::Dword;
        }
        for (int j = 0; j < kLayers; ++j) {
            const WgradParams p = dense_wgrad_params(c, k, j);
            pl.wgrad[b * kLayers + j] = (f34 && wgrad_f34_ok(p, f34_min_tiles)) ? DenseWgrad::F34 : wgrad_nsplit_ok(p, fill) ? DenseWgrad::NSplit
                                      : wgrad_taps_ok(p) ? DenseWgrad::Taps : DenseWgrad::Direct;
        }
    }
    for (int l = 0; l < kLevels; ++l) {
        const auto& sv = c.net->lv[l + 1];
        pl.td_wgrad_dma[l] = wgrad1x1_dma_ok(td_wgrad_params(c, l));
        const ConvParams td = td_dgrad_params(c, l);
        const bool persist = (opt[ENDO_OPT_TD_PERSIST] & 1) && !pl.bf16_dgrad;
        pl.td_dgrad[l] = (persist && td_dgrad_ok(td)) ? TdDgrad::Persistent : (persist && sv.w % 4 != 0 && td_dgrad_small_ok(td)) ? TdDgrad::Runs128
                       : sv.w % 4 == 0 ? TdDgrad::Dma : TdDgrad::Staged;
        const ConvP& tu = table().tu_conv[kLevels - 1 - l];
        pl.tu_wgrad[l] = tu_wgrad_subpix_ok(tu_wgrad_params(c, l, true)) ? TuWgrad::Subpix : wgrad_taps_ok(tu_wgrad_params(c, l, false), true) ? TuWgrad::Taps : TuWgrad::Direct;
        pl.tu_dgrad[l] = !(sv.w % 4 == 0 && tu.cin == kNew && tu.cout == kNew) ? TuDgrad::Plain : tile_count(c, l + 1, 32, 8) >= 1024 ? TuDgrad::Subpix32x8
                       : tile_count(c, l + 1, 16, 8) >= 512 ? TuDgrad::Subpix16x8 : TuDgrad::Subpix16x4;
    }
    const BwdPlan::Block& last = pl.block[kBlocks - 1];
    const int last_base = dense_block(kBlocks - 1).c0;
    pl.use_virt = opt[ENDO_OPT_FINAL_VIRTUAL] && last.fused;
    pl.virt_base = pl.use_virt && last.wino3_layout;
    pl.virt_base_w = pl.use_virt && last.base == BasePass::Wino3Persistent;
    pl.materialise = !pl.use_virt ? 192 : (pl.virt_base ? 0 : last_base);
    pl.c_first = pl.virt_base_w ? last_base : 0;
    const WgradParams first = first_wgrad_params(c);
    pl.first = (f34 && wgrad_f34_raw_ok(first, f34_min_tiles)) ? (opt[ENDO_OPT_FINAL_VIRTUAL] ? FirstWgrad::F34Prep : FirstWgrad::F34)
             : wgrad_taps_ok(first) ? FirstWgrad::Taps : FirstWgrad::Direct;
    return pl;
}

static int dense_wgrad(const Ctx& c, int b, int j, F34ReduceBatch* batch = nullptr, int slice = 0) {
    const DenseBlock k = dense_block(b);
    const ConvP& cv = k.cv[j];
    const auto& lv = c.net->lv[k.level];
    const WgradParams p = dense_wgrad_params(c, k, j);
    float* scratch = c.gradws + c.net->wg_scratch_off;
    ProfScope prof(kProfWgradDense, c.stream, conv_flops(c.net, k.level, cv.cin, cv.cout, 3), 4.0 * c.nt() * lv.plane * (cv.cin + cv.cout));
    switch (c.bwd->wgrad[b * kLayers + j]) {
        case DenseWgrad::F34: return launch_wgrad_f34(p, scratch + (batch ? slice : 0) * kF34ScratchFloats, c.stream, batch);
        case DenseWgrad::NSplit: return launch_wgrad_nsplit(p, scratch, c.stream, c.bwd->bf16_wgrad);
        case DenseWgrad::Taps: return c.bwd->bf16_wgrad ? launch_wgrad_taps<12, IN_BNRELU, 1>(p, c.stream) : launch_wgrad_taps<12, IN_BNRELU>(p, c.stream);
        case DenseWgrad::Direct: return launch_wgrad<3, 1, IN_BNRELU, DY_PLAIN>(p, c.stream);
    }
    return ENDO_E_BADARG;
}

static int dense_bwd(const Ctx& c, int b, int j, int acc_from) {
    const DenseBlock k = dense_block(b);
    const BnP& bn = k.bn[j];
    const ConvP& cv = k.cv[j];
    const int level = k.level, ic0 = k.ic0, oc0 = k.ic0 + k.c0 + kGrowth * j;
    const auto& lv = c.net->lv[level];
    int rc = prep_dy(c, level, oc0, cv.cout, c.grads + cv.b);
    if (rc) return rc;
    {
        Ctx cw;
        rc = c.fork_wgrad(cw, level);
        if (rc) return rc;
        rc = dense_wgrad(cw, b, j);
        if (rc) return rc;
    }
    {
        ConvParams p{};
        fill_grid(c, p, level);
        fill_in(c, p, c.gbuf(level), level, oc0, cv.cout);
        p.wgt = c.params + cv.w; p.w_cout = cv.cout; p.w_cin = cv.cin;
        fill_out(c, p, c.gbuf(level), level, ic0, cv.cin);
        p.x = c.act(level) + ic0 * lv.plane; p.x_ns = lv.t * lv.plane; p.x_cs = static_cast<int>(lv.plane);
        p.bn_saved = c.saved(bn); p.bn_gamma = c.params + bn.g; p.bn_beta = c.params + bn.b;
        p.bn_scratch = c.scratch(bn); p.bn_slot_stride = c.net->slot_stride;
        p.acc_from = acc_from - ic0;
        ProfScope prof(kProfDgradDense, c.stream, conv_flops(c.net, level, cv.cin, cv.cout, 3), 4.0 * c.nt() * lv.plane * (3.0 * cv.cin + cv.cout));
        rc = launch_dgrad_dense_auto(p, c.stream);
        if (rc) return rc;
    }
    return bn_finalize(c, bn, level, ic0);
}

template <int NL>
static int launch_newmap(NewMap form, const DgradBlockParams& p, int cus, hipStream_t stream) {
    switch (form) {
        case NewMap::Bf16: return launch_dgrad_block<NL, 2, 3, 1, 0, 4, 1>(p, stream);
        case NewMap::Persistent: return launch_dgrad_newmap<NL>(p, cus, stream);
        case NewMap::Vec16: return launch_dgrad_block<NL, 2, 3, 1, 0, 4>(p, stream);
        case NewMap::Dword: return launch_dgrad_block<NL, 2, 3>(p, stream);
    }
    return ENDO_E_BADARG;
}

static int dense_block_bwd(const Ctx& c, int b, const FinalVirt* fv = nullptr) {
    const DenseBlock k = dense_block(b);
    const BwdPlan::Block& bl = c.bwd->block[b];
    const int level = k.level, ic0 = k.ic0, c0 = k.c0, new0 = ic0 + c0;
    const auto& lv = c.net->lv[level];
    if (!bl.fused) {
        for (int j = kLayers - 1; j >= 0; --j) {
            const int acc_from = (j == kLayers - 1 && k.base_overwrite) ? new0 : 0;
            int rc = dense_bwd(c, b, j, acc_from < ic0 ? ic0 : acc_from);
            if (rc) return rc;
        }
        return 0;
    }
    BnFin4 pending{};
    int pending_nl = 0;
    F34ReduceBatch red{};
    for (int j = kLayers - 1; j >= 0; --j) {
        int rc = prep_dy(c, level, new0 + kGrowth * j, kGrowth, c.grads + k.cv[j].b, &pending, pending_nl, (fv && j == kLayers - 1) ? fv : nullptr);
        if (rc) return rc;
        const bool defer = c.bwd->overlap == 2;
        if (!defer || j == 0) {
            Ctx cw;
            rc = c.fork_wgrad(cw, level);
            if (rc) return rc;
            for (int jj = defer ? kLayers - 1 : j; jj >= j; --jj) {
                rc = dense_wgrad(cw, b, jj, &red, jj);
                if (rc) return rc;
            }
            if (j == 0 && red.count > 0) {
                ProfScope prof(kProfSmall, cw.stream, 0.0, 0.0);
                rc = launch_wgrad_f34_reduce_batch(red, cw.stream);
                if (rc) return rc;
            }
        }
        if (j > 0) {
            const int nl = kLayers - j;
            BnFin4 a{};
            DgradBlockParams p = newmap_params(c, k, j, &a);
            if (fv) { p.vg = fv->vg; p.vw = fv->vw + ic0 + p.w_ci_off; }
            ProfScope prof(kProfDgradDense, c.stream, 2.0 * c.nt() * lv.plane * kGrowth * kGrowth * 9 * nl,
                           4.0 * c.nt() * lv.plane * (3.0 * kGrowth + kGrowth * nl));
            const int cus = bl.newmap[j] == NewMap::Persistent ? persistent_cus(c.net) : 0;
            rc = nl == 1 ? launch_newmap<1>(bl.newmap[j], p, cus, c.stream) : nl == 2 ? launch_newmap<2>(bl.newmap[j], p, cus, c.stream) : launch_newmap<3>(bl.newmap[j], p, cus, c.stream);
            if (rc) return rc;
            pending = a;
            pending_nl = nl;
        }
    }
    {
        DgradBlockParams p = base_pass_params(c, k);
        const bool virt = fv && c.bwd->virt_base;
        if (virt) { p.vg = fv->vg; p.vw = fv->vw + ic0; }
        ProfScope prof(kProfDgradDense, c.stream, 2.0 * c.nt() * lv.plane * c0 * kGrowth * 9 * kLayers,
                       4.0 * c.nt() * lv.plane * (3.0 * c0 + kGrowth * kLayers));
        const float* ub = c.gradws + c.net->wd_off;
        const float* const u[4] = {ub + k.cv[0].ud, ub + k.cv[1].ud, ub + k.cv[2].ud, ub + k.cv[3].ud};
        int rc = 0;
        switch (bl.base) {
            case BasePass::Block8Bf16: rc = launch_dgrad_block8<4, 1>(p, c.stream); break;
            case BasePass::Block8: rc = launch_dgrad_block8<4>(p, c.stream); break;
            case BasePass::Wino8: rc = launch_dgrad_wino8<4>(p, u, c.stream); break;
            case BasePass::Wino3: rc = run_dgrad_wino3_nl4(p, u, c.stream); break;
            case BasePass::Wino3Persistent: {
                double* fwp = (virt && c.bwd->virt_base_w) ? reinterpret_cast<double*>(c.gradws + c.net->fw_parts_off) : nullptr;
                int used = 0;
                rc = run_dgrad_wino3p_nl4(p, u, std::min(persistent_cus(c.net), kFwPartBlocks), fwp, &used, c.stream);
                if (rc == 0 && fwp) {
                    final_w_reduce_kernel<<<c0, 64, 0, c.stream>>>(fwp, used, c0, fv->gw + ic0);
                    ENDO_LAUNCH_CHECK();
                }
                break;
            }
        }
        if (rc) return rc;
    }
    {
        BnFin4 a;
        for (int j = 0; j < kLayers; ++j) {
            a.scratch[j] = c.scratch(k.bn[j]); a.saved[j] = c.saved(k.bn[j]); a.gamma[j] = c.params + k.bn[j].g;
            a.ggamma[j] = c.grads + k.bn[j].g; a.gbeta[j] = c.grads + k.bn[j].b;
        }
        ProfScope prof(kProfSmall, c.stream, 0.0, 0.0);
        bn_bwd_finalize4_kernel<<<dim3((c0 + 127) / 128, c.net->groups), 128, 0, c.stream>>>(a, kLayers, c.pq_p(level) + ic0, c.pq_q(level) + ic0, c0,
                                                                         static_cast<double>(c.net->n) * lv.h * lv.w, c.training, c.net->gs,
                                                                         c.net->slot_stride);
        ENDO_LAUNCH_CHECK();
    }
    return 0;
}

static int td_bwd(const Ctx& c, int level) {
    const BnP& b = table().td_bn[level];
    const ConvP& cv = table().td_conv[level];
    const int next = level + 1;
    const auto& lv = c.net->lv[level];
    int rc = prep_dy(c, next, next < kLevels ? 48 : 0, cv.cout, c.grads + cv.b);
    if (rc) return rc;
    {
        const WgradParams p = td_wgrad_params(c, level);
        Ctx cw;
        rc = c.fork_wgrad(cw, level);
        if (rc) return rc;
        ProfScope prof(kProfWgradOther, cw.stream, conv_flops(c.net, level, cv.cin, cv.cout, 1), 4.0 * c.nt() * lv.plane * cv.cin);
        rc = !c.bwd->td_wgrad_dma[level] ? launch_wgrad1x1(p, cw.stream) : c.bwd->bf16_wgrad ? launch_wgrad1x1_dma<1>(p, cw.stream) : launch_wgrad1x1_dma<0>(p, cw.stream);
        if (rc) return rc;
    }
    {
        const ConvParams p = td_dgrad_params(c, level);
        ProfScope prof(kProfDgradOther, c.stream, conv_flops(c.net, level, cv.cin, cv.cout, 1), 4.0 * c.nt() * lv.plane * 3.0 * cv.cin);
        switch (c.bwd->td_dgrad[level]) {
            case TdDgrad::Persistent: rc = launch_td_dgrad(p, persistent_cus(c.net), c.stream); break;
            case TdDgrad::Runs128: rc = launch_td_dgrad_small(p, c.stream); break;
            case TdDgrad::Dma: rc = c.bwd->bf16_dgrad ? launch_conv_dma_auto<1, 16, 2, IN_UNPOOL, EPI_DGRAD_BN, 4, 2, 1, 1>(p, c.stream)
                                                      : launch_conv_dma_auto<1, 16, 2, IN_UNPOOL, EPI_DGRAD_BN, 4>(p, c.stream); break;
            case TdDgrad::Staged: rc = launch_conv_auto<1, 16, 3, IN_UNPOOL, EPI_DGRAD_BN, 4>(p, c.stream); break;
        }
        if (rc) return rc;
    }
    return bn_finalize(c, b, level, 48);
}

static int tu_bwd(const Ctx& c, int level, int src_level, int src_c0, const ConvP& cv) {
    const auto& lv = c.net->lv[level];
    int rc = prep_dy(c, level, 0, cv.cout, c.grads + cv.b);
    if (rc) return rc;
    {
        const TuWgrad form = c.bwd->tu_wgrad[level];
        const WgradParams p = tu_wgrad_params(c, level, form == TuWgrad::Subpix);
        Ctx cw;
        rc = c.fork_wgrad(cw, level);
        if (rc) return rc;
        ProfScope prof(kProfWgradOther, cw.stream, conv_flops(c.net, level, cv.cin, cv.cout, 3), 4.0 * c.nt() * lv.plane * (cv.cin / 4.0 + cv.cout));
        rc = form == TuWgrad::Subpix ? launch_tu_wgrad_subpix(p, c.gradws + c.net->wg_scratch_off, cw.stream)
           : form == TuWgrad::Taps ? launch_wgrad_taps<12, IN_UPSAMPLE>(p, cw.stream) : launch_wgrad<3, 1, IN_UPSAMPLE, DY_PLAIN>(p, cw.stream);
        if (rc) return rc;
    }
    ProfScope prof(kProfDgradOther, c.stream, conv_flops(c.net, level, cv.cin, cv.cout, 3), 4.0 * c.nt() * lv.plane * (cv.cout + cv.cin / 4.0));
    const TuDgrad form = c.bwd->tu_dgrad[level];
    if (form == TuDgrad::Plain) {
        ConvParams p{};
        fill_grid(c, p, level);
        fill_in(c, p, c.gbuf(level), level, 0, cv.cout);
        p.wgt = c.params + cv.w; p.w_cout = cv.cout; p.w_cin = cv.cin;
        fill_out(c, p, c.gbuf(src_level), src_level, src_c0, cv.cin);
        return launch_conv_dma_auto<3, 4, 3, IN_PLAIN, EPI_DGRAD_SUMPOOL, 4>(p, c.stream);
    }
    float* wd = c.gradws + c.net->tuw_scratch_off;
    tu_subpix_dgrad_weights_kernel<<<(16 * cv.cout * cv.cin + 255) / 256, 256, 0, c.stream>>>(c.params + cv.w, cv.cout, cv.cin, wd);
    ENDO_LAUNCH_CHECK();
    ConvParams p{};
    fill_grid(c, p, src_level);
    fill_in(c, p, c.gbuf(level), level, 0, 4 * cv.cout);
    p.sub_c = cv.cout;
    p.wgt = wd; p.w_cout = cv.cin; p.w_cin = 4 * cv.cout;
    fill_out(c, p, c.gbuf(src_level), src_level, src_c0, cv.cin);
    if (form == TuDgrad::Subpix32x8) return launch_conv_dma_vec<3, 8, 3, IN_SUBPIX, EPI_FWD, 2, 4, 2, 1, 1>(p, c.stream);
    if (form == TuDgrad::Subpix16x8) return launch_conv_dma_vec<3, 8, 3, IN_SUBPIX, EPI_FWD, 1, 2, 2, 1, 1>(p, c.stream);
    return launch_conv_dma_vec<3, 8, 3, IN_SUBPIX, EPI_FWD, 1, 1, 2, 1, 1>(p, c.stream);
}

static int64_t align_up(int64_t v, int64_t a) { return (v + a - 1) / a * a; }

}

extern "C" int endo_net_create_grouped(endo_net** out, int n, int h, int w, int groups) {
    if (!out || n <= 0 || h <= 0 || w <= 0 || groups <= 0) return ENDO_E_BADARG;
    if (groups > kMaxGroups) return ENDO_E_UNSUPPORTED;
    if ((h % 32) != 0 || (w % 32) != 0) return ENDO_E_UNSUPPORTED;
    const Table& tb = table();
    endo_net* net = new (std::nothrow) endo_net();
    if (!net) return ENDO_E_BADARG;
    net->n = n; net->h = h; net->w = w; net->groups = groups;
    net->wstream = nullptr; net->ev_fork = nullptr; net->ev_join = nullptr;
    net->last_fwd = nullptr; net->last_bwd = nullptr;
    default_options(net->opt);
    int64_t off = 0, sums = 0, pq = 0;
    for (int l = 0; l <= kLevels; ++l) {
        auto& lv = net->lv[l];
        lv.h = h >> l; lv.w = w >> l; lv.t = level_channels(l);
        lv.plane = static_cast<int64_t>(lv.h) * lv.w;
        lv.act = off; lv.grad = off;
        off += align_up(static_cast<int64_t>(n) * lv.t * lv.plane, 64);
        lv.sums = sums; sums += 2 * lv.t;
        lv.pq = pq; pq += lv.t;
    }
    const int64_t acts = off;
    net->pre_off = off; off += align_up(static_cast<int64_t>(n) * h * w, 64);
    net->saved_off = off; off += align_up(2 * tb.bn_width_total, 64);
    int64_t byte_off = off * 4;
    for (int l = 0; l < kLevels; ++l) {
        net->idx_off[l] = byte_off;
        byte_off += align_up(static_cast<int64_t>(n) * (down_in(l) + kNew) * net->lv[l + 1].plane, 256);
    }
    net->sums_off = byte_off;
    net->sums_bytes = sums * 8;
    byte_off += align_up(net->sums_bytes, 256);
    net->partial_off = byte_off / 4;
    byte_off += static_cast<int64_t>(kGrowth) * 163840 * 4;
    net->wino_off = byte_off / 4;
    byte_off += align_up(tb.wino_floats * 4, 256);
    net->wino4_off = byte_off / 4;
    byte_off += align_up(tb.wino4_floats * 4, 256);
    net->tape_floats = byte_off / 4;
    net->pq_off = acts;
    net->pq_floats = 2 * pq;
    net->scratch_off = align_up((acts + net->pq_floats) * 4, 256);
    net->slot_stride = align_up(tb.bn_width_total * 2, 32);
    net->scratch_bytes = net->slot_stride * 8 * kBnSlots;
    net->wg_scratch_off = (net->scratch_off + align_up(net->scratch_bytes, 256)) / 4;
    net->tuw_scratch_off = net->wg_scratch_off + std::max(std::max(kNsScratchFloats, kSpScratchFloats), 4 * kF34ScratchFloats);
    net->wd_off = align_up(net->tuw_scratch_off + 4 * kNew * (4 * kNew + 16), 64);
    net->gplane_off = align_up(net->wd_off + tb.wino_dgrad_floats, 64);
    net->bias_parts_off = net->gplane_off + align_up(static_cast<int64_t>(n) * h * w, 64);
    net->bias_parts_floats = static_cast<int64_t>(kBiasPartChannels) * n * groups * 32;
    {
        int launches = 1, channels = tb.first.cout;
        for (int l = 0; l < kLevels; ++l) {
            for (int j = 0; j < kLayers; ++j) { launches += 2; channels += tb.down_conv[l][j].cout + tb.up_conv[l][j].cout; }
            launches += 2; channels += tb.td_conv[l].cout + tb.tu_conv[l].cout;
        }
        for (int j = 0; j < kLayers; ++j) { ++launches; channels += tb.bott_conv[j].cout; }
        if (launches > kBiasPartLaunches || channels > kBiasPartChannels) { delete net; return ENDO_E_UNSUPPORTED; }
    }
    net->fw_parts_off = net->bias_parts_off + align_up(net->bias_parts_floats, 64);
    net->gradws_floats = net->fw_parts_off + 2 * static_cast<int64_t>(kFwPartBlocks) * 192;
    net->gs = align_up(net->tape_floats > net->gradws_floats ? net->tape_floats : net->gradws_floats, 64);
    *out = net;
    return 0;
}

extern "C" int endo_net_create(endo_net** out, int n, int h, int w) { return endo_net_create_grouped(out, n, h, w, 1); }

static bool option_id_ok(int id) { return id >= 0 && id < ENDO_OPT_COUNT && id != 6; }

extern "C" int endo_net_set_option(endo_net* net, int option_id, int value) {
    if (!net || !option_id_ok(option_id)) return ENDO_E_BADARG;
    const int old = net->opt[option_id];
    net->opt[option_id] = value;
    return old;
}

extern "C" int endo_net_get_option(const endo_net* net, int option_id) {
    if (!net || !option_id_ok(option_id)) return ENDO_E_BADARG;
    return net->opt[option_id];
}

extern "C" void endo_net_destroy(endo_net* net) {
    if (!net) return;
    if (net->ev_fork) (void)hipEventDestroy(net->ev_fork);
    if (net->ev_join) (void)hipEventDestroy(net->ev_join);
    if (net->wstream) (void)hipStreamDestroy(net->wstream);
    delete net->last_fwd;
    delete net->last_bwd;
    delete net;
}
extern "C" int64_t endo_net_param_floats(void) { return table().param_floats; }
extern "C" int64_t endo_net_bn_floats(void) { return table().bn_floats; }
extern "C" int64_t endo_net_tape_floats(const endo_net* net) { return !net ? 0 : (net->groups > 1 ? net->groups * net->gs : net->tape_floats); }
extern "C" int64_t endo_net_gradws_floats(const endo_net* net) { return !net ? 0 : (net->groups > 1 ? net->groups * net->gs : net->gradws_floats); }
extern "C" int endo_net_groups(const endo_net* net) { return net ? net->groups : 0; }
extern "C" int64_t endo_net_group_stride(const endo_net* net) { return net ? net->gs : 0; }
extern "C" int64_t endo_net_param_offset(int index) {
    const Table& tb = table();
    if (index < 0 || index >= static_cast<int>(tb.param_offsets.size())) return -1;
    return tb.param_offsets[index];
}
extern "C" int64_t endo_net_bn_offset(int bn_index, int which) {
    const Table& tb = table();
    if (bn_index < 0 || bn_index >= static_cast<int>(tb.bn_order.size()) || which < 0 || which > 1) return -1;
    return tb.bn_order[bn_index]->run + which * tb.bn_order[bn_index]->c;
}
extern "C" int endo_net_level_channels(int level) { return (level < 0 || level > kLevels) ? -1 : level_channels(level); }
extern "C" int64_t endo_net_act_offset(const endo_net* net, int level) { return (!net || level < 0 || level > kLevels) ? -1 : net->lv[level].act; }

extern "C" int64_t endo_net_tape_offset(const endo_net* net, int what, int index) {
    if (!net) return -1;
    const Table& tb = table();
    switch (what) {
        case ENDO_TAPE_PRE: return net->pre_off;
        case ENDO_TAPE_BN_SAVED:
            if (index < 0 || index >= static_cast<int>(tb.bn_order.size())) return -1;
            return net->saved_off + 2 * tb.bn_order[index]->saved;
        case ENDO_TAPE_POOL:
            if (index < 0 || index >= kLevels) return -1;
            return net->idx_off[index];
        default: return -1;
    }
}

extern "C" int endo_net_fwd(endo_net* net, const float* params, float* bn_running, const float* x, float* out, float* tape,
                            int training, void* stream_) {
    if (!net || !params || !bn_running || !x || !out || !tape) return ENDO_E_BADARG;
    const Table& tb = table();
    Ctx c{net, params, bn_running, tape, nullptr, nullptr, training, static_cast<hipStream_t>(stream_)};
    const FwdPlan plan = plan_fwd(c);
    c.fwd = &plan;
    if (!net->last_fwd) net->last_fwd = new (std::nothrow) FwdPlan;
    if (net->last_fwd) *net->last_fwd = plan;
    for (int g = 0; g < net->groups; ++g)
        ENDO_CHECK(hipMemsetAsync(reinterpret_cast<char*>(tape + g * net->gs) + net->sums_off, 0, net->sums_bytes, c.stream));
    if (!plan.bf16) {
        ProfScope prof(kProfSmall, c.stream, 0.0, 4.0 * (tb.wino_floats + tb.wino_floats * 9 / 16));
        WinoWeightTable wt = tb.wino;
        for (int l = 0; l < wt.layers; ++l) wt.mode[l] = plan.dense[l].chunk_weights ? 1 : 0;
        wino_fwd_weights_kernel<<<(wt.start[wt.layers] + 255) / 256, 256, 0, c.stream>>>(wt, params, tape + net->wino_off);
        ENDO_LAUNCH_CHECK();
        if (plan.wino4_weights) wino4_fwd_weights_kernel<<<(tb.wino4.start[tb.wino4.layers] + 255) / 256, 256, 0, c.stream>>>(tb.wino4, params, tape + net->wino4_off);
        ENDO_LAUNCH_CHECK();
    }
    int rc;
    {
        ConvParams p{};
        fill_grid(c, p, 0);
        p.in = x; p.in_ns = 3 * net->lv[0].plane; p.in_cs = static_cast<int>(net->lv[0].plane); p.in_w = net->w; p.cin = 3;
        p.in_gs = net->n * p.in_ns;
        p.wgt = params + tb.first.w; p.bias = params + tb.first.b; p.w_cout = kFirst; p.w_cin = 3;
        fill_out(c, p, c.act(0), 0, 48, kFirst);
        p.out_sums = c.out_sums(0, 48);
        ProfScope prof(kProfConvFirst, c.stream, conv_flops(net, 0, 3, kFirst, 3), 4.0 * c.nt() * net->lv[0].plane * (3 + kFirst));
        rc = launch_conv_dma_auto<3, 4, 3, IN_PLAIN, EPI_FWD>(p, c.stream);
        if (rc) return rc;
    }
    for (int b = 0; b < kBlocks; ++b) {
        if (b > kLevels) {
            const int i = b - kLevels - 1, l = kLevels - 1 - i;
            rc = tu_fwd(c, l, l + 1, (i == 0) ? 288 : 96 + down_in(l + 1), tb.tu_conv[i]);
            if (rc) return rc;
        }
        for (int j = 0; j < kLayers; ++j) {
            rc = dense_fwd(c, b, j);
            if (rc) return rc;
        }
        if (b < kLevels) {
            rc = td_fwd(c, b);
            if (rc) return rc;
        }
    }
    {
        const auto& lv = net->lv[0];
        const int c_first = plan.fuse_final ? 96 + down_in(0) + kGrowth * (kLayers - 1) : 0;
        ProfScope prof(kProfConvFinal, c.stream, 2.0 * c.nt() * lv.plane * 192, 4.0 * c.nt() * lv.plane * (194 - c_first));
        int bx = static_cast<int>((lv.plane / 4 + 255) / 256);
        bx = bx < 1 ? 1 : bx;
        final_fwd_kernel<<<dim3(bx, c.nt()), 256, 0, c.stream>>>(c.act(0), lv.t * lv.plane, static_cast<int>(lv.plane), 192,
                                                                 params + tb.final_.w, params + tb.final_.b, tape + net->pre_off, out,
                                                                 net->n, net->gs, c_first);
        ENDO_LAUNCH_CHECK();
    }
    return 0;
}

extern "C" int endo_net_bwd(endo_net* net, const float* params, const float* x, const float* tape, const float* grad_out,
                            float* grads, float* gradws, int training, void* stream_) {
    if (!net || !params || !x || !tape || !grad_out || !grads || !gradws) return ENDO_E_BADARG;
    const Table& tb = table();
    Ctx c{net, params, nullptr, const_cast<float*>(tape), grads, gradws, training, static_cast<hipStream_t>(stream_)};
    c.x = x;
    const BwdPlan plan = plan_bwd(c);
    c.bwd = &plan;
    if (!net->last_bwd) net->last_bwd = new (std::nothrow) BwdPlan;
    if (net->last_bwd) *net->last_bwd = plan;
    BiasParts bias_parts{};
    c.bias_parts = &bias_parts;
    if (!net->wstream) {
        ENDO_CHECK(hipStreamCreateWithFlags(&net->wstream, hipStreamNonBlocking));
        ENDO_CHECK(hipEventCreateWithFlags(&net->ev_fork, hipEventDisableTiming));
        ENDO_CHECK(hipEventCreateWithFlags(&net->ev_join, hipEventDisableTiming));
    }
    for (int g = 0; g < net->groups; ++g)
        ENDO_CHECK(hipMemsetAsync(gradws + g * net->gs + net->pq_off, 0,
                                  static_cast<size_t>(net->scratch_off + net->scratch_bytes - net->pq_off * 4), c.stream));
    if (plan.dgrad_weights) {
        ProfScope prof(kProfSmall, c.stream, 0.0, 4.0 * 2.0 * tb.wino_dgrad_floats);
        int layout1_blocks = 0;
        for (int b = 0; b < kBlocks; ++b) layout1_blocks |= plan.block[b].wino3_layout ? 1 << b : 0;
        dgrad_wino_weights_kernel<<<(tb.wino_dgrad.start[tb.wino_dgrad.layers] + 255) / 256, 256, 0, c.stream>>>(tb.wino_dgrad, params, gradws + net->wd_off, layout1_blocks);
        ENDO_LAUNCH_CHECK();
    }
    int rc;
    const FinalVirt virt{gradws + net->gplane_off, params + tb.final_.w, grads + tb.final_.w};
    {
        const auto& lv = net->lv[0];
        const int materialise = plan.materialise;
        {
            Ctx cw;
            rc = c.fork_wgrad(cw, 0);
            if (rc) return rc;
            const int c_first = plan.c_first;
            int by = static_cast<int>((lv.plane + 256 * 16 - 1) / (256 * 16));
            by = by < 1 ? 1 : (by > 16 ? 16 : by);
            ProfScope prof(kProfConvFinal, cw.stream, 2.0 * c.nt() * lv.plane * (192 - c_first), 4.0 * c.nt() * lv.plane * (192 - c_first + 2));
            final_bwd_weight_kernel<<<dim3(192 - c_first + 1, by, c.nt()), 256, 0, cw.stream>>>(grad_out, tape + net->pre_off, c.act(0), lv.t * lv.plane,
                                                                         static_cast<int>(lv.plane), 192, net->n, net->gs, grads + tb.final_.w,
                                                                         grads + tb.final_.b, c_first);
            ENDO_LAUNCH_CHECK();
        }
        ProfScope prof(kProfConvFinal, c.stream, 2.0 * c.nt() * lv.plane * 192, 4.0 * c.nt() * lv.plane * (materialise + 2));
        if (plan.use_virt) {
            int bx = static_cast<int>((lv.plane + 1023) / 1024);
            final_g_kernel<<<dim3(bx, c.nt()), 256, 0, c.stream>>>(grad_out, tape + net->pre_off, gradws + net->gplane_off, static_cast<int>(lv.plane), net->n, net->gs);
            ENDO_LAUNCH_CHECK();
        }
        if (materialise > 0) {
            int bx = static_cast<int>((lv.plane + 255) / 256);
            final_bwd_data_kernel<<<dim3(bx, c.nt()), 256, 0, c.stream>>>(grad_out, tape + net->pre_off, params + tb.final_.w, c.gbuf(0),
                                                                          lv.t * lv.plane, static_cast<int>(lv.plane), materialise, net->n, net->gs, 0);
            ENDO_LAUNCH_CHECK();
        }
    }
    for (int b = kBlocks - 1; b >= 0; --b) {
        if (b < kLevels) {
            rc = td_bwd(c, b);
            if (rc) return rc;
        }
        rc = dense_block_bwd(c, b, (b == kBlocks - 1 && plan.use_virt) ? &virt : nullptr);
        if (rc) return rc;
        if (b > kLevels) {
            const int i = b - kLevels - 1, l = kLevels - 1 - i;
            rc = tu_bwd(c, l, l + 1, (i == 0) ? 288 : 96 + down_in(l + 1), tb.tu_conv[i]);
            if (rc) return rc;
        }
    }
    {
        WgradParams p = first_wgrad_params(c);
        const auto& lv = net->lv[0];
        if (plan.first == FirstWgrad::F34Prep) {
            p.prep_x = c.act(0) + 48 * lv.plane;
            p.prep_p = c.pq_p(0) + 48; p.prep_q = c.pq_q(0) + 48;
            p.prep_bias = grads + tb.first.b;
        } else {
            rc = prep_dy(c, 0, 48, kFirst, grads + tb.first.b);
            if (rc) return rc;
        }
        Ctx cw;
        rc = c.fork_wgrad(cw, 0);
        if (rc) return rc;
        ProfScope prof(kProfWgradOther, cw.stream, conv_flops(net, 0, 3, kFirst, 3), 4.0 * c.nt() * lv.plane * (3 + kFirst));
        switch (plan.first) {
            case FirstWgrad::F34Prep: rc = launch_wgrad_f34<0, true, true>(p, gradws + net->wg_scratch_off, cw.stream); break;
            case FirstWgrad::F34: rc = launch_wgrad_f34<0, true>(p, gradws + net->wg_scratch_off, cw.stream); break;
            case FirstWgrad::Taps: rc = launch_wgrad_taps<12, IN_PLAIN>(p, cw.stream); break;
            case FirstWgrad::Direct: rc = launch_wgrad<3, 3, IN_PLAIN, DY_PLAIN>(p, cw.stream); break;
        }
        if (rc) return rc;
    }
    if (bias_parts.table.n > 0) {
        ProfScope prof(kProfSmall, c.stream, 0.0, 4.0 * bias_parts.used);
        bias_reduce_kernel<<<dim3(bias_parts.table.n, 8), 256, 0, c.stream>>>(bias_parts.table);
        ENDO_LAUNCH_CHECK();
    }
    if (net->wstream) {
        ENDO_CHECK(hipEventRecord(net->ev_join, net->wstream));
        ENDO_CHECK(hipStreamWaitEvent(c.stream, net->ev_join, 0));
    }
    return 0;
}

namespace endo {

struct PlanKind { const char* name; const char* const* values; int count; };
static const char* const kDenseFwdNames[] = {"Wino4", "Wino2_32x16", "Wino2_32x8", "SplitK", "Direct32x8", "Direct16x8", "DirectAuto"};
static const char* const kNewMapNames[] = {"Bf16", "Persistent", "Vec16", "Dword"};
static const char* const kBasePassNames[] = {"Block8", "Block8Bf16", "Wino3", "Wino3Persistent", "Wino8"};
static const char* const kDenseWgradNames[] = {"F34", "NSplit", "Taps", "Direct"};
static const char* const kTdDgradNames[] = {"Persistent", "Runs128", "Dma", "Staged"};
static const char* const kTuWgradNames[] = {"Subpix", "Taps", "Direct"};
static const char* const kTuDgradNames[] = {"Subpix32x8", "Subpix16x8", "Subpix16x4", "Plain"};
static const char* const kFirstWgradNames[] = {"F34Prep", "F34", "Taps", "Direct"};
static const char* const kTdFwdNames[] = {"PerTile", "Persistent"};
static const char* const kTuFwdNames[] = {"Upsample", "Subpix"};
static const char* const kBlockBwdNames[] = {"PerLayer", "Fused"};
static const char* const kTdWgradNames[] = {"Plain", "Dma"};
static_assert(static_cast<int>(DenseFwd::DirectAuto) == 6 && static_cast<int>(NewMap::Dword) == 3 && static_cast<int>(BasePass::Wino8) == 4 &&
              static_cast<int>(DenseWgrad::Direct) == 3 && static_cast<int>(TdDgrad::Staged) == 3 && static_cast<int>(TuWgrad::Direct) == 2 &&
              static_cast<int>(TuDgrad::Plain) == 3 && static_cast<int>(FirstWgrad::Direct) == 3, "the name tables follow the enums");
static const PlanKind kPlanKinds[ENDO_PLAN_KIND_COUNT] = {
    {"dense_fwd", kDenseFwdNames, 7}, {"dense_fwd_ksplit", nullptr, 0}, {"dense_fwd_chunk_weights", nullptr, 0}, {"fwd_bf16", nullptr, 0},
    {"wino4_weights", nullptr, 0}, {"fuse_final", nullptr, 0}, {"td_fwd", kTdFwdNames, 2}, {"tu_fwd", kTuFwdNames, 2},
    {"block_bwd", kBlockBwdNames, 2}, {"newmap", kNewMapNames, 4}, {"base_pass", kBasePassNames, 5}, {"wino3_layout", nullptr, 0},
    {"dense_wgrad", kDenseWgradNames, 4}, {"td_wgrad", kTdWgradNames, 2}, {"td_dgrad", kTdDgradNames, 4}, {"tu_wgrad", kTuWgradNames, 3},
    {"tu_dgrad", kTuDgradNames, 4}, {"wgrad_overlap", nullptr, 0}, {"bf16_wgrad", nullptr, 0}, {"bf16_dgrad", nullptr, 0},
    {"dgrad_weights", nullptr, 0}, {"use_virt", nullptr, 0}, {"virt_base", nullptr, 0}, {"virt_base_w", nullptr, 0},
    {"materialise", nullptr, 0}, {"c_first", nullptr, 0}, {"first_wgrad", kFirstWgradNames, 4},
};

struct PlanWriter {
    int32_t* out; int capacity; int count = 0;
    void put(int kind, int index, int level, int value) {
        if (count + 4 <= capacity) { out[count] = kind; out[count + 1] = index; out[count + 2] = level; out[count + 3] = value; }
        count += 4;
    }
};

static void write_plan(const FwdPlan& pl, PlanWriter& w) {
    for (int i = 0; i < kDense; ++i) {
        const int level = dense_block(i / kLayers).level;
        w.put(ENDO_PLAN_DENSE_FWD, i, level, static_cast<int>(pl.dense[i].form));
        w.put(ENDO_PLAN_DENSE_FWD_KSPLIT, i, level, pl.dense[i].ksplit);
        w.put(ENDO_PLAN_DENSE_FWD_CHUNK_WEIGHTS, i, level, pl.dense[i].chunk_weights);
    }
    w.put(ENDO_PLAN_FWD_BF16, 0, -1, pl.bf16);
    w.put(ENDO_PLAN_WINO4_WEIGHTS, 0, -1, pl.wino4_weights);
    w.put(ENDO_PLAN_FUSE_FINAL, 0, -1, pl.fuse_final);
    for (int l = 0; l < kLevels; ++l) {
        w.put(ENDO_PLAN_TD_FWD, l, l, pl.td_persistent[l]);
        w.put(ENDO_PLAN_TU_FWD, l, l, pl.tu_subpix[l]);
    }
}

static void write_plan(const BwdPlan& pl, PlanWriter& w) {
    for (int b = 0; b < kBlocks; ++b) {
        const int level = dense_block(b).level;
        const BwdPlan::Block& bl = pl.block[b];
        w.put(ENDO_PLAN_BLOCK_BWD, b, level, bl.fused);
        for (int j = 1; j < kLayers; ++j) w.put(ENDO_PLAN_NEWMAP, b * kLayers + j, level, static_cast<int>(bl.newmap[j]));
        w.put(ENDO_PLAN_BASE_PASS, b, level, static_cast<int>(bl.base));
        w.put(ENDO_PLAN_WINO3_LAYOUT, b, level, bl.wino3_layout);
    }
    for (int i = 0; i < kDense; ++i) w.put(ENDO_PLAN_DENSE_WGRAD, i, dense_block(i / kLayers).level, static_cast<int>(pl.wgrad[i]));
    for (int l = 0; l < kLevels; ++l) {
        w.put(ENDO_PLAN_TD_WGRAD, l, l, pl.td_wgrad_dma[l]);
        w.put(ENDO_PLAN_TD_DGRAD, l, l, static_cast<int>(pl.td_dgrad[l]));
        w.put(ENDO_PLAN_TU_WGRAD, l, l, static_cast<int>(pl.tu_wgrad[l]));
        w.put(ENDO_PLAN_TU_DGRAD, l, l, static_cast<int>(pl.tu_dgrad[l]));
    }
    w.put(ENDO_PLAN_WGRAD_OVERLAP, 0, -1, pl.overlap);
    w.put(ENDO_PLAN_BF16_WGRAD, 0, -1, pl.bf16_wgrad);
    w.put(ENDO_PLAN_BF16_DGRAD, 0, -1, pl.bf16_dgrad);
    w.put(ENDO_PLAN_DGRAD_WEIGHTS, 0, -1, pl.dgrad_weights);
    w.put(ENDO_PLAN_USE_VIRT, 0, -1, pl.use_virt);
    w.put(ENDO_PLAN_VIRT_BASE, 0, -1, pl.virt_base);
    w.put(ENDO_PLAN_VIRT_BASE_W, 0, -1, pl.virt_base_w);
    w.put(ENDO_PLAN_MATERIALISE, 0, -1, pl.materialise);
    w.put(ENDO_PLAN_C_FIRST, 0, -1, pl.c_first);
    w.put(ENDO_PLAN_FIRST_WGRAD, 0, 0, static_cast<int>(pl.first));
}

template <typename Plan>
static int serialise_plan(const Plan& pl, int32_t* out, int capacity) {
    PlanWriter w{out, capacity};
    write_plan(pl, w);
    return w.count <= capacity ? w.count : ENDO_E_BADARG;
}

}

extern "C" int endo_net_last_plan(const endo_net* net, int pass, int32_t* out, int capacity) {
    if (!net || !out || capacity < 0) return ENDO_E_BADARG;
    if (pass == ENDO_PASS_FWD) return net->last_fwd ? serialise_plan(*net->last_fwd, out, capacity) : ENDO_E_BADARG;
    if (pass == ENDO_PASS_BWD) return net->last_bwd ? serialise_plan(*net->last_bwd, out, capacity) : ENDO_E_BADARG;
    return ENDO_E_BADARG;
}

extern "C" int endo_net_plan_query(const endo_net* net, int pass, int training, const float* params, float* bn_running, const float* x,
                                   float* tape, float* grads, float* gradws, int32_t* out, int capacity) {
    if (!net || !out || capacity < 0 || !params || !tape) return ENDO_E_BADARG;
    if (pass == ENDO_PASS_FWD) {
        if (!bn_running) return ENDO_E_BADARG;
        const Ctx c{net, params, bn_running, tape, nullptr, nullptr, training, nullptr};
        return serialise_plan(plan_fwd(c), out, capacity);
    }
    if (pass == ENDO_PASS_BWD) {
        if (!x || !grads || !gradws) return ENDO_E_BADARG;
        Ctx c{net, params, nullptr, tape, grads, gradws, training, nullptr};
        c.x = x;
        return serialise_plan(plan_bwd(c), out, capacity);
    }
    return ENDO_E_BADARG;
}

extern "C" const char* endo_net_plan_name(int kind, int value) {
    if (kind < 0 || kind >= ENDO_PLAN_KIND_COUNT) return nullptr;
    const PlanKind& k = kPlanKinds[kind];
    if (value == -1) return k.name;
    return (k.values && value >= 0 && value < k.count) ? k.values[value] : nullptr;
}
```

endoscopydepthestimation-pytorch_amd/csrc/wino4_fwd_kernels.h:

```cpp
#pragma once

#include "conv_dma_kernels.h"
#include "wgrad_f34_kernels.h"
#include "wino_fwd_kernels.h"

namespace endo {

constexpr float kW4A = 0.625f, kW4B = 1.5f;
constexpr float kW4A2 = kW4A * kW4A, kW4B2 = kW4B * kW4B;
constexpr float kW4A3 = kW4A2 * kW4A, kW4B3 = kW4B2 * kW4B;
constexpr float kW4P = kW4A2 * kW4B2, kW4S = kW4A2 + kW4B2;
constexpr float kW4N0 = 1.f / kW4P;
constexpr float kW4NA = 1.f / (2.f * kW4A2 * (kW4A2 - kW4B2));
constexpr float kW4NB = 1.f / (2.f * kW4B2 * (kW4B2 - kW4A2));

constexpr int kW4UStride = 576;

__global__ void __launch_bounds__(256) wino4_fwd_weights_kernel(const WinoWeightTable t, const float* __restrict__ params, float* __restrict__ u) {
    const int total = t.start[t.layers];
    for (int item = blockIdx.x * blockDim.x + threadIdx.x; item < total; item += gridDim.x * blockDim.x) {
        int l = 0;
        while (item >= t.start[l + 1]) ++l;
        const int e = item - t.start[l];
        const int ci = e >> 4, j = e & 15;
        float g[3][3];
#pragma unroll
        for (int a = 0; a < 3; ++a)
#pragma unroll
            for (int b = 0; b < 3; ++b) g[a][b] = 0.f;
        if (j < t.cout[l]) {
            const float* src = params + t.w_off[l] + (static_cast<int64_t>(j) * t.cin[l] + ci) * 9;
#pragma unroll
            for (int a = 0; a < 3; ++a)
#pragma unroll
                for (int b = 0; b < 3; ++b) g[a][b] = src[a * 3 + b];
        }
        auto gt = [](float a, float b, float c, float (&o)[6]) {
            const float ea = fmaf(kW4A2, c, a), eb = fmaf(kW4B2, c, a);
            o[0] = kW4N0 * a;
            o[1] = kW4NA * fmaf(kW4A, b, ea);
            o[2] = kW4NA * fmaf(-kW4A, b, ea);
            o[3] = kW4NB * fmaf(kW4B, b, eb);
            o[4] = kW4NB * fmaf(-kW4B, b, eb);
            o[5] = c;
        };
        float h[6][3];
#pragma unroll
        for (int b = 0; b < 3; ++b) {
            float o[6];
            gt(g[0][b], g[1][b], g[2][b], o);
#pragma unroll
            for (int i = 0; i < 6; ++i) h[i][b] = o[i];
        }
        float* dst = u + t.u_off[l] + static_cast<int64_t>(ci) * kW4UStride + j * 12;
#pragma unroll
        for (int i = 0; i < 6; ++i) {
            float o[6];
            gt(h[i][0], h[i][1], h[i][2], o);
#pragma unroll
            for (int jj = 0; jj < 6; ++jj) dst[(i >> 1) * 192 + (i & 1) * 6 + jj] = o[jj];
        }
    }
}

struct Wino4Geom {
    static constexpr int kTileX = 64, kTileY = 16;
    static constexpr int kCols = kTileX + 8;
    static constexpr int kRows = kTileY + 2;
    static constexpr int kPlane = kRows * kCols;
    static constexpr int kKC = 4;
    static constexpr int kXUnits = kKC * kPlane / 4;
    static constexpr int kUUnits = kKC * kW4UStride / 4;
    static constexpr int kXRounds = (kXUnits + kConvThreads - 1) / kConvThreads;
    static constexpr int kURounds = (kUUnits + kConvThreads - 1) / kConvThreads;
    static constexpr int kBuf = kKC * kPlane + kKC * kW4UStride;
    static constexpr int kTail = 4 * 16 * 2;
    static size_t bytes(int bn_cap) { return sizeof(float) * (2 * kBuf + 4 * bn_cap + kTail); }
};

__device__ __forceinline__ void w4_at(const float m0, const float m1, const float m2, const float m3, const float m4, const float m5, float (&y)[4]) {
    const float s1 = m1 + m2, d1 = m1 - m2, s2 = m3 + m4, d2 = m3 - m4;
    y[0] = m0 + s1 + s2;
    y[1] = fmaf(kW4B, d2, kW4A * d1);
    y[2] = fmaf(kW4B2, s2, kW4A2 * s1);
    y[3] = fmaf(kW4B3, d2, fmaf(kW4A3, d1, m5));
}

template <typename T>
__device__ __forceinline__ void w4_bt(const T d0, const T d1, const T d2, const T d3, const T d4, const T d5, T (&t)[6]) {
    t[0] = f34_fma<T>(kW4P, d0, f34_fma<T>(-kW4S, d2, d4));
    const T pp = f34_fma<T>(-kW4B2, d2, d4), qh = f34_fma<T>(-kW4B2, d1, d3);
    t[1] = f34_fma<T>(kW4A, qh, pp);
    t[2] = f34_fma<T>(-kW4A, qh, pp);
    const T rr = f34_fma<T>(-kW4A2, d2, d4), sh = f34_fma<T>(-kW4A2, d1, d3);
    t[3] = f34_fma<T>(kW4B, sh, rr);
    t[4] = f34_fma<T>(-kW4B, sh, rr);
    t[5] = f34_fma<T>(kW4P, d1, f34_fma<T>(-kW4S, d3, d5));
}

template <bool FIN = false>
__global__ void __launch_bounds__(kConvThreads, 2) wino4_fwd_kernel(const ConvParams p0) {
    using G = Wino4Geom;
    extern __shared__ __attribute__((aligned(16))) float smem[];
    float* s_aux = smem + 2 * G::kBuf;
    int grp, n;
    group_of(p0, blockIdx.z, grp, n);
    const ConvParams p = group_view(p0, grp);
    const int groups = p0.group_n > 0 ? gridDim.z / p0.group_n : 1;
    const bool first_of_group = blockIdx.x == 0 && n == 0;
    const int cap = p.bn_cap;

    const int tid = threadIdx.x;
    const int lane = tid & 63;
    const int wave = __builtin_amdgcn_readfirstlane(tid >> 6);
    const int li = lane & 15;
    const int lk = lane >> 4;
    const int tile = (gridDim.x & 7) == 0 ? xcd_remap(blockIdx.x, gridDim.x) : blockIdx.x;
    const int x0 = (tile % p.tiles_x) * G::kTileX;
    const int y0 = (tile / p.tiles_x) * G::kTileY;

    for (int c = tid; c < p.cin; c += kConvThreads) {
        float scale, mean, beta;
        bn_input_constants(p, p0, grp, groups, first_of_group, c, scale, mean, beta);
        s_aux[c] = scale;
        s_aux[cap + c] = mean;
        s_aux[2 * cap + c] = beta;
        if constexpr (FIN) s_aux[3 * cap + G::kTail + c] = p.fin_w[c];
    }
    f32x4 fin[4];
#pragma unroll
    for (int r = 0; r < 4; ++r) fin[r] = f32x4{0.f, 0.f, 0.f, 0.f};

    f32x4 acc[36];
#pragma unroll
    for (int xi = 0; xi < 36; ++xi) acc[xi] = f32x4{0.f, 0.f, 0.f, 0.f};

    const __amdgpu_buffer_rsrc_t xr = f34_rsrc(p.in + n * p.in_ns, p.cin * p.in_cs * 4);
    const __amdgpu_buffer_rsrc_t ur = f34_rsrc(p.wgt, p.cin * kW4UStride * 4);
    unsigned x_vo[G::kXRounds];
#pragma unroll
    for (int k = 0; k < G::kXRounds; ++k) {
        const int e = tid + k * kConvThreads;
        x_vo[k] = 0x80000000u;
        if (e < G::kXUnits) {
            const int c = e / (G::kPlane / 4), u = e - c * (G::kPlane / 4);
            const int ry = u / (G::kCols / 4);
            const int rx = (u - ry * (G::kCols / 4)) * 4;
            const int gy = y0 - 1 + ry;
            const int gx = x0 - 4 + rx;
            if (gy >= 0 && gy < p.h && gx >= 0 && gx < p.w) x_vo[k] = 4u * static_cast<unsigned>(c * p.in_cs + gy * p.in_w + gx);
        }
    }
    const unsigned u_vo = 16u * static_cast<unsigned>(tid);
    const int nchunks = p.cin / G::kKC;

    auto issue_dma = [&](int chunk, int buf) {
        float* s_stage = smem + buf * G::kBuf + wave * 256;
        const unsigned xs = 4u * static_cast<unsigned>(chunk * G::kKC * p.in_cs);
        const unsigned us = 4u * static_cast<unsigned>(chunk * G::kKC * kW4UStride);
#pragma unroll
        for (int k = 0; k < G::kXRounds; ++k) {
            const int e0 = k * kConvThreads + wave * 64;
            if (e0 < G::kXUnits) {
                if (e0 + 64 <= G::kXUnits || e0 + lane < G::kXUnits)
                    __builtin_amdgcn_raw_ptr_buffer_load_lds(xr, (lptr_t)(s_stage + k * 4 * kConvThreads), 16, x_vo[k], xs, 0, 0);
            }
        }
        float* s_u = s_stage + G::kKC * G::kPlane;
#pragma unroll
        for (int k = 0; k < G::kURounds; ++k) {
            const int e0 = k * kConvThreads + wave * 64;
            if (e0 < G::kUUnits)
                __builtin_amdgcn_raw_ptr_buffer_load_lds(ur, (lptr_t)(s_u + k * 4 * kConvThreads), 16, u_vo + 16u * static_cast<unsigned>(k * kConvThreads), us, 0, 0);
        }
    };

    const bool l_out = x0 + 4 * li == 0, r_out = x0 + 4 * li + 4 >= p.w;
    const int py = y0 + 4 * wave - 1;
    const bool top_out = py < 0, bottom_out = py + 5 >= p.h;

    auto compute = [&](int chunk, int buf) {
        const float* s_in = smem + buf * G::kBuf;
        const float* s_u = s_in + G::kKC * G::kPlane;
        const int ch = chunk * G::kKC + lk;
        const float sc = s_aux[ch], mn = s_aux[cap + ch], bt = s_aux[2 * cap + ch];
        const float sh = fmaf(-mn, sc, bt);
        const f32x2 sc_m = {sc, sc}, sh_m = {sh, sh};
        const f32x2 sc_e = {l_out ? 0.f : sc, r_out ? 0.f : sc}, sh_e = {l_out ? 0.f : sh, r_out ? 0.f : sh};
        const float* a_base = s_in + lk * G::kPlane + (4 * wave) * G::kCols + 4 * li + 4;
        float wfin = 0.f;
        if constexpr (FIN) wfin = s_aux[3 * cap + G::kTail + ch];
        float d[6][6];
#pragma unroll
        for (int r = 0; r < 6; ++r) {
            const f32x4 m = *reinterpret_cast<const f32x4*>(a_base + r * G::kCols);
            if constexpr (FIN) {
                if (r >= 1 && r <= 4) {
#pragma unroll
                    for (int k = 0; k < 4; ++k) fin[r - 1][k] = fmaf(wfin, m[k], fin[r - 1][k]);
                }
            }
            const float hl = a_base[r * G::kCols - 1], hr = a_base[r * G::kCols + 4];
            const f32x2 e = __builtin_elementwise_fma(f32x2{hl, hr}, sc_e, sh_e);
            const f32x2 a = __builtin_elementwise_fma(f32x2{m[0], m[1]}, sc_m, sh_m);
            const f32x2 b = __builtin_elementwise_fma(f32x2{m[2], m[3]}, sc_m, sh_m);
            d[r][0] = fmaxf(e[0], 0.f); d[r][1] = fmaxf(e[1], 0.f);
            d[r][2] = fmaxf(a[0], 0.f); d[r][3] = fmaxf(a[1], 0.f);
            d[r][4] = fmaxf(b[0], 0.f); d[r][5] = fmaxf(b[1], 0.f);
        }
        if (top_out) {
#pragma unroll
            for (int e = 0; e < 6; ++e) d[0][e] = 0.f;
        }
        if (bottom_out) {
#pragma unroll
            for (int e = 0; e < 6; ++e) d[5][e] = 0.f;
        }
        f32x2 t05[6], t12[6], t34[6];
        w4_bt(f32x2{d[0][0], d[0][1]}, f32x2{d[1][0], d[1][1]}, f32x2{d[2][0], d[2][1]}, f32x2{d[3][0], d[3][1]}, f32x2{d[4][0], d[4][1]},
              f32x2{d[5][0], d[5][1]}, t05);
        w4_bt(f32x2{d[0][2], d[0][3]}, f32x2{d[1][2], d[1][3]}, f32x2{d[2][2], d[2][3]}, f32x2{d[3][2], d[3][3]}, f32x2{d[4][2], d[4][3]},
              f32x2{d[5][2], d[5][3]}, t12);
        w4_bt(f32x2{d[0][4], d[0][5]}, f32x2{d[1][4], d[1][5]}, f32x2{d[2][4], d[2][5]}, f32x2{d[3][4], d[3][5]}, f32x2{d[4][4], d[4][5]},
              f32x2{d[5][4], d[5][5]}, t34);
        const float* b_base = s_u + lk * kW4UStride + li * 12;
#pragma unroll
        for (int ip = 0; ip < 3; ++ip) {
            const f32x4 u0 = *reinterpret_cast<const f32x4*>(b_base + ip * 192);
            const f32x4 u1 = *reinterpret_cast<const f32x4*>(b_base + ip * 192 + 4);
            const f32x4 u2 = *reinterpret_cast<const f32x4*>(b_base + ip * 192 + 8);
            const float uu[12] = {u0[0], u0[1], u0[2], u0[3], u1[0], u1[1], u1[2], u1[3], u2[0], u2[1], u2[2], u2[3]};
#pragma unroll
            for (int h = 0; h < 2; ++h) {
                const int i = 2 * ip + h;
                const f32x2 p05 = t05[i], p12 = t12[i], p34 = t34[i];
                const float x0v = fmaf(kW4P, p05[0], fmaf(-kW4S, p12[1], p34[1]));
                const float x5v = fmaf(kW4P, p12[0], fmaf(-kW4S, p34[0], p05[1]));
                const f32x2 qp = f34_fma<f32x2>(-kW4B2, p12, p34);
                const f32x2 sr = f34_fma<f32x2>(-kW4A2, p12, p34);
                const float x1v = fmaf(kW4A, qp[0], qp[1]), x2v = fmaf(-kW4A, qp[0], qp[1]);
                const float x3v = fmaf(kW4B, sr[0], sr[1]), x4v = fmaf(-kW4B, sr[0], sr[1]);
                acc[6 * i + 0] = __builtin_amdgcn_mfma_f32_16x16x4f32(x0v, uu[6 * h + 0], acc[6 * i + 0], 0, 0, 0);
                acc[6 * i + 1] = __builtin_amdgcn_mfma_f32_16x16x4f32(x1v, uu[6 * h + 1], acc[6 * i + 1], 0, 0, 0);
                acc[6 * i + 2] = __builtin_amdgcn_mfma_f32_16x16x4f32(x2v, uu[6 * h + 2], acc[6 * i + 2], 0, 0, 0);
                acc[6 * i + 3] = __builtin_amdgcn_mfma_f32_16x16x4f32(x3v, uu[6 * h + 3], acc[6 * i + 3], 0, 0, 0);
                acc[6 * i + 4] = __builtin_amdgcn_mfma_f32_16x16x4f32(x4v, uu[6 * h + 4], acc[6 * i + 4], 0, 0, 0);
                acc[6 * i + 5] = __builtin_amdgcn_mfma_f32_16x16x4f32(x5v, uu[6 * h + 5], acc[6 * i + 5], 0, 0, 0);
            }
        }
    };

    if (nchunks > 0) issue_dma(0, 0);
    for (int chunk = 0; chunk < nchunks; ++chunk) {
        const int b = chunk & 1;
        asm volatile("s_waitcnt vmcnt(0)" ::: "memory");
        __syncthreads();
        if (chunk + 1 < nchunks) issue_dma(chunk + 1, b ^ 1);
        compute(chunk, b);
    }

    if constexpr (FIN) {
        f32x4 mine = fin[0];
#pragma unroll
        for (int r = 0; r < 4; ++r) {
#pragma unroll
            for (int k = 0; k < 4; ++k) {
                float v = fin[r][k];
                v += __shfl_xor(v, 16, 64);
                v += __shfl_xor(v, 32, 64);
                if (r == lk) mine[k] = v;
            }
        }
        const int fx = x0 + 4 * li, fy = y0 + 4 * wave + lk;
        if (fx < p.w && fy < p.h)
            *reinterpret_cast<f32x4*>(p.fin_out + static_cast<int64_t>(grp) * p0.gs + static_cast<int64_t>(n) * p.h * p.w + static_cast<int64_t>(fy) * p.w + fx) = mine;
    }

    float* s_red = s_aux + 3 * cap;
    const int co = li;
    const bool co_ok = co < p.cout;
    const float bias = (co_ok && p.bias) ? p.bias[co] : 0.f;
    const int y = y0 + 4 * wave;
    float s1 = 0.f, s2 = 0.f;
#pragma unroll
    for (int e = 0; e < 4; ++e) {
        float c4[4][6];
#pragma unroll
        for (int c = 0; c < 6; ++c) {
            float o[4];
            w4_at(acc[c][e], acc[6 + c][e], acc[12 + c][e], acc[18 + c][e], acc[24 + c][e], acc[30 + c][e], o);
#pragma unroll
            for (int a = 0; a < 4; ++a) c4[a][c] = o[a];
        }
        const int px = x0 + 4 * (4 * lk + e);
#pragma unroll
        for (int a = 0; a < 4; ++a) {
            float o[4];
            w4_at(c4[a][0], c4[a][1], c4[a][2], c4[a][3], c4[a][4], c4[a][5], o);
            const f32x4 v = {o[0] + bias, o[1] + bias, o[2] + bias, o[3] + bias};
            if (co_ok && px < p.w && y + a < p.h) {
                *reinterpret_cast<f32x4*>(p.out + n * p.out_ns + static_cast<int64_t>(co) * p.out_cs + static_cast<int64_t>(y + a) * p.out_w + px) = v;
#pragma unroll
                for (int k = 0; k < 4; ++k) { s1 += v[k]; s2 += v[k] * v[k]; }
            }
        }
    }
    if (p.out_sums) {
        s1 += __shfl_xor(s1, 16, 64); s1 += __shfl_xor(s1, 32, 64);
        s2 += __shfl_xor(s2, 16, 64); s2 += __shfl_xor(s2, 32, 64);
        if (lk == 0) {
            s_red[(wave * 16 + li) * 2] = s1;
            s_red[(wave * 16 + li) * 2 + 1] = s2;
        }
        __syncthreads();
        if (tid < 32) {
            const int j = tid >> 1, which = tid & 1;
            if (j < p.cout) {
                double t = 0.0;
                for (int wv = 0; wv < 4; ++wv) t += static_cast<double>(s_red[(wv * 16 + j) * 2 + which]);
                atomicAdd(p.out_sums + 2 * j + which, t);
            }
        }
    }
}

inline bool wino4_fwd_ok(const ConvParams& p) {
    return wino_fwd_ok(p) && (p.h % 4 == 0) && static_cast<int64_t>(p.cin) * p.in_cs * 4 < (1ll << 31);
}

template <bool FIN>
inline int launch_wino4_fwd_t(ConvParams p, hipStream_t stream) {
    using G = Wino4Geom;
    p.tiles_x = (p.w + G::kTileX - 1) / G::kTileX;
    p.bn_cap = (p.cin + 15) / 16 * 16;
    const int tiles_y = (p.h + G::kTileY - 1) / G::kTileY;
    return launch_dyn(wino4_fwd_kernel<FIN>, dim3(p.tiles_x * tiles_y, 1, p.n), kConvThreads, G::bytes(p.bn_cap), stream, p);
}
inline int launch_wino4_fwd(const ConvParams& p, hipStream_t stream) {
    return p.fin_w ? launch_wino4_fwd_t<true>(p, stream) : launch_wino4_fwd_t<false>(p, stream);
}

}
```

endoscopydepthestimation-pytorch_amd/csrc/wino_fwd_kernels.h:

```cpp
#pragma once

#include "conv_dma_kernels.h"

namespace endo {

constexpr int kWinoUStride = 16 * 16 + 16;
constexpr int kWinoMaxLayers = 48;

struct WinoWeightTable {
    int layers;
    int start[kWinoMaxLayers + 1];
    int cin[kWinoMaxLayers];
    int cout[kWinoMaxLayers];
    int64_t w_off[kWinoMaxLayers];
    int64_t u_off[kWinoMaxLayers];
    int mode[kWinoMaxLayers];
};
constexpr int kDenseChunkFloats = 9 * 16 * 16;

__global__ void __launch_bounds__(256) wino_fwd_weights_kernel(const WinoWeightTable t, const float* __restrict__ params, float* __restrict__ u) {
    const int total = t.start[t.layers];
    for (int item = blockIdx.x * blockDim.x + threadIdx.x; item < total; item += gridDim.x * blockDim.x) {
        int l = 0;
        while (item >= t.start[l + 1]) ++l;
        const int e = item - t.start[l];
        const int ci = e >> 4, j = e & 15;
        float g[3][3];
#pragma unroll
        for (int a = 0; a < 3; ++a)
#pragma unroll
            for (int b = 0; b < 3; ++b) g[a][b] = 0.f;
        if (j < t.cout[l]) {
            const float* src = params + t.w_off[l] + (static_cast<int64_t>(j) * t.cin[l] + ci) * 9;
#pragma unroll
            for (int a = 0; a < 3; ++a)
#pragma unroll
                for (int b = 0; b < 3; ++b) g[a][b] = src[a * 3 + b];
        }
        if (t.mode[l] == 1) {
            float* dst = u + t.u_off[l] + static_cast<int64_t>(ci >> 4) * kDenseChunkFloats + (ci & 15) * 16 + j;
#pragma unroll
            for (int tap = 0; tap < 9; ++tap) dst[tap * 256] = g[tap / 3][tap % 3];
            if (ci == t.cin[l] - 1)
                for (int cz = (ci & 15) + 1; cz < 16; ++cz)
#pragma unroll
                    for (int tap = 0; tap < 9; ++tap) dst[tap * 256 + (cz - (ci & 15)) * 16] = 0.f;
            continue;
        }
        float h[4][3];
#pragma unroll
        for (int b = 0; b < 3; ++b) {
            h[0][b] = g[0][b];
            h[1][b] = 0.5f * (g[0][b] + g[1][b] + g[2][b]);
            h[2][b] = 0.5f * (g[0][b] - g[1][b] + g[2][b]);
            h[3][b] = g[2][b];
        }
        float* dst = u + t.u_off[l] + static_cast<int64_t>(ci) * kWinoUStride + j;
#pragma unroll
        for (int a = 0; a < 4; ++a) {
            dst[(4 * a + 0) * 16] = h[a][0];
            dst[(4 * a + 1) * 16] = 0.5f * (h[a][0] + h[a][1] + h[a][2]);
            dst[(4 * a + 2) * 16] = 0.5f * (h[a][0] - h[a][1] + h[a][2]);
            dst[(4 * a + 3) * 16] = h[a][2];
        }
        if (j == 0) {
#pragma unroll
            for (int k = 0; k < 16; ++k) dst[256 + k] = 0.f;
        }
    }
}

constexpr int kWinoFwdStages = 2;

template <int R, int KC>
struct WinoFwdGeom {
    static constexpr int kTileX = 32;
    static constexpr int kTileY = 8 * R;
    static constexpr int kLeft = 4;
    static constexpr int kCols = kTileX + 2 * kLeft;
    static constexpr int kRows = kTileY + 2;
    static constexpr int kPlane = kRows * kCols;
    static constexpr int kCS = ((kPlane - 32 + 63) / 64) * 64 + 32;
    static constexpr int kUnits = kCS / 4;
    static constexpr int kPos = (kUnits + kConvThreads - 1) / kConvThreads;
    static constexpr int kUUnits = KC * kWinoUStride / 4;
    static constexpr int kUPos = (kUUnits + kConvThreads - 1) / kConvThreads;
    static constexpr int kFlat = KC * kUnits + kUUnits;
    static constexpr int kDma = (kFlat + kConvThreads - 1) / kConvThreads;
    static constexpr int kDmaMin = (kFlat - (kDma - 1) * kConvThreads > 3 * 64) ? kDma : kDma - 1;
    static_assert(kCS == 4 * kUnits, "a stage is one contiguous array of DMA units");
    static constexpr int kBuf = KC * kCS + KC * kWinoUStride;
    static constexpr int kTail = 4 * 16 * 2;
    static size_t bytes(int bn_cap) { return sizeof(float) * (kWinoFwdStages * kBuf + 3 * bn_cap + kTail); }
};

template <int R, int KC, int MINW, int EXP = 0>
__global__ void __launch_bounds__(kConvThreads, MINW) wino_fwd_kernel(const ConvParams p0) {
    using G = WinoFwdGeom<R, KC>;
    constexpr int NS = kWinoFwdStages;
    typedef float f32x2 __attribute__((ext_vector_type(2)));
    extern __shared__ __attribute__((aligned(16))) float smem[];
    float* s_aux = smem + NS * G::kBuf;
    int grp, n;
    group_of(p0, blockIdx.z, grp, n);
    const ConvParams p = group_view(p0, grp);
    const int groups = p0.group_n > 0 ? gridDim.z / p0.group_n : 1;
    const bool first_of_group = blockIdx.x == 0 && n == 0;
    const int cap = p.bn_cap;

    const int tid = threadIdx.x;
    const int lane = tid & 63;
    const int wave = __builtin_amdgcn_readfirstlane(tid >> 6);
    const int li = lane & 15;
    const int lk = lane >> 4;
    const int tile = (gridDim.x & 7) == 0 ? xcd_remap(blockIdx.x, gridDim.x) : blockIdx.x;
    const int x0 = (tile % p.tiles_x) * G::kTileX;
    const int y0 = (tile / p.tiles_x) * G::kTileY;

    for (int c = tid; c < p.cin; c += kConvThreads) {
        float scale, mean, beta;
        bn_input_constants(p, p0, grp, groups, first_of_group, c, scale, mean, beta);
        s_aux[c] = scale;
        s_aux[cap + c] = mean;
        s_aux[2 * cap + c] = beta;
    }
    for (int c = p.cin + tid; c < ((p.cin + KC - 1) / KC) * KC; c += kConvThreads) {
        s_aux[c] = 0.f; s_aux[cap + c] = 0.f; s_aux[2 * cap + c] = 0.f;
    }

    f32x4 acc[R][16];
#pragma unroll
    for (int r = 0; r < R; ++r)
#pragma unroll
        for (int xi = 0; xi < 16; ++xi) acc[r][xi] = f32x4{0.f, 0.f, 0.f, 0.f};

    const float* d_ptr[G::kDma];
    unsigned d_stride[G::kDma];
    {
        const float* in_n = p.in + n * p.in_ns;
#pragma unroll
        for (int k = 0; k < G::kDma; ++k) {
            const int e = tid + k * kConvThreads;
            d_ptr[k] = g_pad_consts;
            d_stride[k] = 0;
            if (e < KC * G::kUnits) {
                const int c = e / G::kUnits, u = e - c * G::kUnits;
                const int ry = u / (G::kCols / 4);
                const int rx = (u - ry * (G::kCols / 4)) * 4;
                const int gy = y0 - 1 + ry;
                const int gx = x0 - G::kLeft + rx;
                if (ry < G::kRows && gy >= 0 && gy < p.h && gx >= 0 && gx < p.w) {
                    d_ptr[k] = in_n + static_cast<int64_t>(c) * p.in_cs + gy * p.in_w + gx;
                    d_stride[k] = static_cast<unsigned>(KC) * static_cast<unsigned>(p.in_cs) * 4u;
                }
            } else if (e < G::kFlat) {
                d_ptr[k] = p.wgt + 4 * (e - KC * G::kUnits);
                d_stride[k] = KC * kWinoUStride * 4u;
            }
        }
    }
    const int nchunks = p.cin / KC;

    auto issue_dma = [&](int buf) {
        float* s_stage = smem + buf * G::kBuf + wave * 256;
#pragma unroll
        for (int k = 0; k < G::kDma; ++k) {
            if (k + 1 < G::kDma) {
                __builtin_amdgcn_global_load_lds((gptr_t)d_ptr[k], (lptr_t)(s_stage + k * 4 * kConvThreads), 16, 0, 0);
            } else {
                const int e0 = k * kConvThreads + wave * 64;
                if (e0 < G::kFlat && e0 + lane < G::kFlat)
                    __builtin_amdgcn_global_load_lds((gptr_t)d_ptr[k], (lptr_t)(s_stage + k * 4 * kConvThreads), 16, 0, 0);
            }
            d_ptr[k] = reinterpret_cast<const float*>(reinterpret_cast<const char*>(d_ptr[k]) + d_stride[k]);
        }
    };

    auto compute = [&](int chunk, int buf) {
        const float* s_in = smem + buf * G::kBuf;
        const float* s_u = s_in + KC * G::kCS;
#pragma unroll
        for (int quad = 0; quad < KC / 4; ++quad) {
            const int ch = chunk * KC + quad * 4 + lk;
            const float sc = s_aux[ch], mn = s_aux[cap + ch], bt = s_aux[2 * cap + ch];
            const f32x2 mn2 = {mn, mn}, sc2 = {sc, sc}, bt2 = {bt, bt};
            const float* b_base = s_u + (quad * 4 + lk) * kWinoUStride + li;
            float b[16];
#pragma unroll
            for (int xi = 0; xi < 16; ++xi) b[xi] = (EXP & 16) ? static_cast<float>(xi + lane) : b_base[xi * 16];
            const float* a_base = s_in + (quad * 4 + lk) * G::kCS + (2 * wave * R) * G::kCols + 2 * li + 2;
            f32x2 mid[2 * R + 2], end[2 * R + 2];
#pragma unroll
            for (int row = 0; row < 2 * R + 2; ++row) {
                f32x2 m, e;
                if constexpr ((EXP & 8) != 0) {
                    m = f32x2{sc + row, mn + row}; e = f32x2{bt + row, sc - row};
                } else {
                    const f32x2 left = *reinterpret_cast<const f32x2*>(a_base + row * G::kCols);
                    const f32x2 right = *reinterpret_cast<const f32x2*>(a_base + row * G::kCols + 4);
                    m = *reinterpret_cast<const f32x2*>(a_base + row * G::kCols + 2);
                    e = f32x2{left[1], right[0]};
                }
                if constexpr ((EXP & 2) == 0) {
                    m = __builtin_elementwise_fma(m - mn2, sc2, bt2);
                    e = __builtin_elementwise_fma(e - mn2, sc2, bt2);
                    mid[row] = f32x2{__builtin_fmaxf(m[0], 0.f), __builtin_fmaxf(m[1], 0.f)};
                    end[row] = f32x2{__builtin_fmaxf(e[0], 0.f), __builtin_fmaxf(e[1], 0.f)};
                } else {
                    mid[row] = m; end[row] = e;
                }
            }
#pragma unroll
            for (int r = 0; r < R; ++r) {
                f32x2 tm[4], te[4];
                if constexpr ((EXP & 4) == 0) {
                    tm[0] = mid[2 * r] - mid[2 * r + 2];     te[0] = end[2 * r] - end[2 * r + 2];
                    tm[1] = mid[2 * r + 1] + mid[2 * r + 2]; te[1] = end[2 * r + 1] + end[2 * r + 2];
                    tm[2] = mid[2 * r + 2] - mid[2 * r + 1]; te[2] = end[2 * r + 2] - end[2 * r + 1];
                    tm[3] = mid[2 * r + 1] - mid[2 * r + 3]; te[3] = end[2 * r + 1] - end[2 * r + 3];
                } else {
#pragma unroll
                    for (int a = 0; a < 4; ++a) { tm[a] = mid[2 * r + a]; te[a] = end[2 * r + a]; }
                }
#pragma unroll
                for (int a = 0; a < 4; ++a) {
                    const float c0 = te[a][0], c1 = tm[a][0], c2 = tm[a][1], c3 = te[a][1];
                    float v0 = c0 - c2, v1 = c1 + c2, v2 = c2 - c1, v3 = c1 - c3;
                    if constexpr ((EXP & 4) != 0) { v0 = c0; v1 = c1; v2 = c2; v3 = c3; }
                    if constexpr ((EXP & 64) != 0) {
                        acc[r][4 * a + 0][0] += v0 * b[4 * a]; acc[r][4 * a + 1][0] += v1 * b[4 * a + 1];
                        acc[r][4 * a + 2][0] += v2 * b[4 * a + 2]; acc[r][4 * a + 3][0] += v3 * b[4 * a + 3];
                    } else {
                        acc[r][4 * a + 0] = __builtin_amdgcn_mfma_f32_16x16x4f32(v0, b[4 * a + 0], acc[r][4 * a + 0], 0, 0, 0);
                        acc[r][4 * a + 1] = __builtin_amdgcn_mfma_f32_16x16x4f32(v1, b[4 * a + 1], acc[r][4 * a + 1], 0, 0, 0);
                        acc[r][4 * a + 2] = __builtin_amdgcn_mfma_f32_16x16x4f32(v2, b[4 * a + 2], acc[r][4 * a + 2], 0, 0, 0);
                        acc[r][4 * a + 3] = __builtin_amdgcn_mfma_f32_16x16x4f32(v3, b[4 * a + 3], acc[r][4 * a + 3], 0, 0, 0);
                    }
                }
            }
        }
    };

#pragma unroll
    for (int s0 = 0; s0 < NS - 1; ++s0)
        if (s0 < nchunks) issue_dma(s0);
    for (int chunk = 0; chunk < nchunks; ++chunk) {
        const int b = chunk % NS;
        const int newer = min(nchunks - 1 - chunk, NS - 2);
        if ((EXP & 32) && chunk > 0) {}
        else if (newer >= NS - 2 && NS > 2) asm volatile("s_waitcnt vmcnt(%0)" ::"n"((NS - 2) * G::kDmaMin) : "memory");
        else if (newer == 1 && NS > 3) asm volatile("s_waitcnt vmcnt(%0)" ::"n"(G::kDmaMin) : "memory");
        else asm volatile("s_waitcnt vmcnt(0)" ::: "memory");
        if (!(EXP & 32) || chunk == 0) __syncthreads();
        if (chunk + NS - 1 < nchunks && !(EXP & 1)) issue_dma((chunk + NS - 1) % NS);
        compute(chunk, b);
    }

    float* s_red = s_aux + 3 * cap;
    const int co = li;
    const bool co_ok = co < p.cout;
    const float bias = (co_ok && p.bias) ? p.bias[co] : 0.f;
    const int px = x0 + 8 * lk;
    float s1 = 0.f, s2 = 0.f;
#pragma unroll
    for (int r = 0; r < R; ++r) {
        const int y = y0 + 2 * (wave * R + r);
        f32x4 row0[2], row1[2];
#pragma unroll
        for (int e = 0; e < 4; ++e) {
            float u0[4], u1[4];
#pragma unroll
            for (int c = 0; c < 4; ++c) {
                const float m0 = acc[r][c][e], m1 = acc[r][4 + c][e], m2 = acc[r][8 + c][e], m3 = acc[r][12 + c][e];
                u0[c] = m0 + m1 + m2;
                u1[c] = m1 - m2 - m3;
            }
            row0[e >> 1][2 * (e & 1)] = u0[0] + u0[1] + u0[2] + bias;
            row0[e >> 1][2 * (e & 1) + 1] = u0[1] - u0[2] - u0[3] + bias;
            row1[e >> 1][2 * (e & 1)] = u1[0] + u1[1] + u1[2] + bias;
            row1[e >> 1][2 * (e & 1) + 1] = u1[1] - u1[2] - u1[3] + bias;
        }
        if (co_ok) {
#pragma unroll
            for (int half = 0; half < 2; ++half) {
                if (px + 4 * half + 3 < p.w) {
                    float* dst = p.out + n * p.out_ns + static_cast<int64_t>(co) * p.out_cs + static_cast<int64_t>(y) * p.out_w + px + 4 * half;
                    if (y < p.h) {
                        *reinterpret_cast<f32x4*>(dst) = row0[half];
#pragma unroll
                        for (int e = 0; e < 4; ++e) { s1 += row0[half][e]; s2 += row0[half][e] * row0[half][e]; }
                    }
                    if (y + 1 < p.h) {
                        *reinterpret_cast<f32x4*>(dst + p.out_w) = row1[half];
#pragma unroll
                        for (int e = 0; e < 4; ++e) { s1 += row1[half][e]; s2 += row1[half][e] * row1[half][e]; }
                    }
                }
            }
        }
    }
    if (p.out_sums) {
        s1 += __shfl_xor(s1, 16, 64); s1 += __shfl_xor(s1, 32, 64);
        s2 += __shfl_xor(s2, 16, 64); s2 += __shfl_xor(s2, 32, 64);
        if (lk == 0) {
            s_red[(wave * 16 + li) * 2] = s1;
            s_red[(wave * 16 + li) * 2 + 1] = s2;
        }
        __syncthreads();
        if (tid < 32) {
            const int j = tid >> 1, which = tid & 1;
            if (j < p.cout) {
                double t = 0.0;
                for (int wv = 0; wv < 4; ++wv) t += static_cast<double>(s_red[(wv * 16 + j) * 2 + which]);
                atomicAdd(p.out_sums + 2 * j + which, t);
            }
        }
    }
}

inline bool wino_fwd_ok(const ConvParams& p) {
    return p.cout <= 16 && (p.w % 4 == 0) && (p.in_w % 4 == 0) && (p.out_w % 4 == 0) && (p.in_cs % 4 == 0) && (p.in_ns % 4 == 0) &&
           (p.out_cs % 4 == 0) && (p.out_ns % 4 == 0) && (reinterpret_cast<uintptr_t>(p.in) % 16 == 0) &&
           (reinterpret_cast<uintptr_t>(p.out) % 16 == 0) && (reinterpret_cast<uintptr_t>(p.wgt) % 16 == 0) && p.ksplit == 0 &&
           p.cin % 4 == 0 && p.cin >= 8;
}

template <int R, int KC, int MINW, int EXP = 0>
inline int launch_wino_fwd(ConvParams p, hipStream_t stream) {
    using G = WinoFwdGeom<R, KC>;
    p.tiles_x = (p.w + G::kTileX - 1) / G::kTileX;
    p.bn_cap = ((p.cin + KC - 1) / KC * KC + 15) / 16 * 16;
    const int tiles_y = (p.h + G::kTileY - 1) / G::kTileY;
    return launch_dyn(wino_fwd_kernel<R, KC, MINW, EXP>, dim3(p.tiles_x * tiles_y, 1, p.n), kConvThreads, G::bytes(p.bn_cap), stream, p);
}


}
```

Baseline: 514.1.

## Fuse all weight-transform prep into one launch and precompute backward weights during forward

Turns the per-layer weight transforms (forward Winograd, wino4, transposed-up phase weights, dgrad Winograd, subpixel dgrad weights) into device item functions. A single table-driven weight-prep kernel now produces all of them into tape-resident buffers before the forward pass, and the backward pass reads those instead of launching its own transform kernels. This removes several small kernel launches and serial dependencies from the forward and backward paths. In exchange the tape holds extra per-level weight buffers, the backward forms must be planned in advance during the forward, and a prepared-tape cache is added.

```diff
diff --git a/endoscopydepthestimation-pytorch_amd/csrc/dgrad_wino_kernels.h b/endoscopydepthestimation-pytorch_amd/csrc/dgrad_wino_kernels.h
--- a/endoscopydepthestimation-pytorch_amd/csrc/dgrad_wino_kernels.h
+++ b/endoscopydepthestimation-pytorch_amd/csrc/dgrad_wino_kernels.h
@@ -16,50 +16,54 @@
     int64_t u_off[kWinoDgradMaxLayers];
 };
 
+__device__ __forceinline__ void dgrad_wino_weights_item(const float* __restrict__ params, float* __restrict__ u, int cin, int64_t w_off, int64_t u_off,
+                                                        bool layout1, int e) {
+    const int j = e & 15, c = (e >> 4) % 12, grp = (e >> 4) / 12;
+    const int ci = grp * 16 + j;
+    float g[3][3];
+#pragma unroll
+    for (int a = 0; a < 3; ++a)
+#pragma unroll
+        for (int b = 0; b < 3; ++b) g[a][b] = 0.f;
+    if (ci < cin) {
+        const float* src = params + w_off + (static_cast<int64_t>(c) * cin + ci) * 9;
+#pragma unroll
+        for (int a = 0; a < 3; ++a)
+#pragma unroll
+            for (int b = 0; b < 3; ++b) g[a][b] = src[(2 - a) * 3 + (2 - b)];
+    }
+    float h[4][3];
+#pragma unroll
+    for (int b = 0; b < 3; ++b) {
+        h[0][b] = g[0][b];
+        h[1][b] = 0.5f * (g[0][b] + g[1][b] + g[2][b]);
+        h[2][b] = 0.5f * (g[0][b] - g[1][b] + g[2][b]);
+        h[3][b] = g[2][b];
+    }
+    if (layout1) {
+        float* dst = u + u_off + static_cast<int64_t>(grp) * kWinoDgradSlice + (c * 64 + j) * 4;
+#pragma unroll
+        for (int a = 0; a < 4; ++a)
+            *reinterpret_cast<f32x4*>(dst + a * 64) = f32x4{h[a][0], 0.5f * (h[a][0] + h[a][1] + h[a][2]), 0.5f * (h[a][0] - h[a][1] + h[a][2]), h[a][2]};
+        return;
+    }
+    float* dst = u + u_off + static_cast<int64_t>(grp) * kWinoDgradSlice + c * 16 + j;
+#pragma unroll
+    for (int a = 0; a < 4; ++a) {
+        dst[(4 * a + 0) * 192] = h[a][0];
+        dst[(4 * a + 1) * 192] = 0.5f * (h[a][0] + h[a][1] + h[a][2]);
+        dst[(4 * a + 2) * 192] = 0.5f * (h[a][0] - h[a][1] + h[a][2]);
+        dst[(4 * a + 3) * 192] = h[a][2];
+    }
+}
+
 static __global__ void __launch_bounds__(256) dgrad_wino_weights_kernel(const WinoDgradTable t, const float* __restrict__ params, float* __restrict__ u,
                                                                  int layout1_blocks = 0) {
     const int total = t.start[t.layers];
     for (int item = blockIdx.x * blockDim.x + threadIdx.x; item < total; item += gridDim.x * blockDim.x) {
         int l = 0;
         while (item >= t.start[l + 1]) ++l;
-        const int e = item - t.start[l];
-        const int j = e & 15, c = (e >> 4) % 12, grp = (e >> 4) / 12;
-        const int ci = grp * 16 + j;
-        float g[3][3];
-#pragma unroll
-        for (int a = 0; a < 3; ++a)
-#pragma unroll
-            for (int b = 0; b < 3; ++b) g[a][b] = 0.f;
-        if (ci < t.cin[l]) {
-            const float* src = params + t.w_off[l] + (static_cast<int64_t>(c) * t.cin[l] + ci) * 9;
-#pragma unroll
-            for (int a = 0; a < 3; ++a)
-#pragma unroll
-                for (int b = 0; b < 3; ++b) g[a][b] = src[(2 - a) * 3 + (2 - b)];
-        }
-        float h[4][3];
-#pragma unroll
-        for (int b = 0; b < 3; ++b) {
-            h[0][b] = g[0][b];
-            h[1][b] = 0.5f * (g[0][b] + g[1][b] + g[2][b]);
-            h[2][b] = 0.5f * (g[0][b] - g[1][b] + g[2][b]);
-            h[3][b] = g[2][b];
-        }
-        if ((layout1_blocks >> (l >> 2)) & 1) {
-            float* dst = u + t.u_off[l] + static_cast<int64_t>(grp) * kWinoDgradSlice + (c * 64 + j) * 4;
-#pragma unroll
-            for (int a = 0; a < 4; ++a)
-                *reinterpret_cast<f32x4*>(dst + a * 64) = f32x4{h[a][0], 0.5f * (h[a][0] + h[a][1] + h[a][2]), 0.5f * (h[a][0] - h[a][1] + h[a][2]), h[a][2]};
-            continue;
-        }
-        float* dst = u + t.u_off[l] + static_cast<int64_t>(grp) * kWinoDgradSlice + c * 16 + j;
-#pragma unroll
-        for (int a = 0; a < 4; ++a) {
-            dst[(4 * a + 0) * 192] = h[a][0];
-            dst[(4 * a + 1) * 192] = 0.5f * (h[a][0] + h[a][1] + h[a][2]);
-            dst[(4 * a + 2) * 192] = 0.5f * (h[a][0] - h[a][1] + h[a][2]);
-            dst[(4 * a + 3) * 192] = h[a][2];
-        }
+        dgrad_wino_weights_item(params, u, t.cin[l], t.w_off[l], t.u_off[l], ((layout1_blocks >> (l >> 2)) & 1) != 0, item - t.start[l]);
     }
 }
 
diff --git a/endoscopydepthestimation-pytorch_amd/csrc/net.hip b/endoscopydepthestimation-pytorch_amd/csrc/net.hip
--- a/endoscopydepthestimation-pytorch_amd/csrc/net.hip
+++ b/endoscopydepthestimation-pytorch_amd/csrc/net.hip
@@ -15,6 +15,7 @@
 #include "wino4_fwd_kernels.h"
 #include "dgrad_wino_kernels.h"
 #include "dgrad_wino3_kernels.h"
+#include "weight_prep_kernels.h"
 
 
 namespace endo {
@@ -30,6 +31,7 @@
 constexpr int kNew = kGrowth * kLayers;
 constexpr float kBnEps = 1.0e-5f;
 constexpr float kBnMomentum = 0.1f;
+constexpr int kPreparedTapes = 8;
 constexpr int kSideStreamFromLevel = 0;
 
 struct ConvP { int64_t w, b; int cout, cin, ks; int64_t u; int64_t ud; };
@@ -146,14 +148,15 @@
     int64_t partial_off;
     int64_t wino_off;
     int64_t wino4_off;
+    int64_t tu_phase_off[kLevels];
+    int64_t dgrad_wino_off;
+    int64_t tu_subpix_off[kLevels];
     int64_t pq_off;
     int64_t pq_floats;
     int64_t scratch_off;
     int64_t scratch_bytes;
     int64_t slot_stride;
     int64_t wg_scratch_off;
-    int64_t tuw_scratch_off;
-    int64_t wd_off;
     int64_t gplane_off;
     int64_t bias_parts_off;
     int64_t fw_parts_off;
@@ -164,6 +167,12 @@
     int opt[ENDO_OPT_COUNT];
     FwdPlan* last_fwd;
     BwdPlan* last_bwd;
+    struct Prepared {
+        const float* tape;
+        bool dgrad_wino;
+        int layout1_blocks;
+        int tu_subpix_levels;
+    } prepared[kPreparedTapes];
 };
 
 namespace endo {
@@ -338,51 +347,6 @@
     }
 }
 
-__global__ void tu_phase_weights_kernel(const float* __restrict__ w, int cout, int cin, float* __restrict__ out) {
-    constexpr int kPhW = 2 * 12 * 16 + 16;
-    const int total = 2 * cin * 2 * 12 * 16;
-    for (int i = blockIdx.x * blockDim.x + threadIdx.x; i < total; i += gridDim.x * blockDim.x) {
-        const int lane16 = i & 15;
-        const int slot = (i >> 4) % 12;
-        const int t = (i / (16 * 12)) & 1;
-        const int ci = (i / (16 * 12 * 2)) % cin;
-        const int a = i / (16 * 12 * 2 * cin);
-        int ctap, tile;
-        if (slot < 3) { ctap = 0; tile = slot; } else if (slot < 9) { ctap = 1; tile = slot - 3; } else { ctap = 2; tile = slot - 9 + 3; }
-        const int b = tile / 3, co = (tile % 3) * 16 + lane16;
-        float v = 0.f;
-        if (co < cout) {
-            const float* src = w + (static_cast<int64_t>(co) * cin + ci) * 9;
-            const int ky0 = a == 0 ? (t == 0 ? 0 : 1) : (t == 0 ? 0 : 2), ky1 = a == 0 ? (t == 0 ? 0 : 2) : (t == 0 ? 1 : 2);
-            int kx0, kx1;
-            if (b == 0) { kx0 = ctap == 0 ? 0 : 1; kx1 = ctap == 0 ? 0 : 2; }
-            else { kx0 = ctap == 1 ? 0 : 2; kx1 = ctap == 1 ? 1 : 2; }
-            for (int ky = ky0; ky <= ky1; ++ky)
-                for (int kx = kx0; kx <= kx1; ++kx) v += src[ky * 3 + kx];
-        }
-        out[(static_cast<int64_t>(a) * cin + ci) * kPhW + (t * 12 + slot) * 16 + lane16] = v;
-    }
-}
-
-__global__ void tu_subpix_dgrad_weights_kernel(const float* __restrict__ w, int cout, int cin, float* __restrict__ out) {
-    const int pitch = 4 * cin + 16;
-    const int total = 4 * cout * 4 * cin;
-    for (int i = blockIdx.x * blockDim.x + threadIdx.x; i < total; i += gridDim.x * blockDim.x) {
-        const int ci = i % cin;
-        const int tap = (i / cin) & 3;
-        const int co = (i / (4 * cin)) % cout;
-        const int ph = i / (4 * cin * cout);
-        const int alpha = ph >> 1, beta = ph & 1, tyi = tap >> 1, txi = tap & 1;
-        const int ky0 = alpha == 0 ? (tyi == 0 ? 1 : 0) : (tyi == 0 ? 2 : 0), ky1 = alpha == 0 ? (tyi == 0 ? 2 : 0) : (tyi == 0 ? 2 : 1);
-        const int kx0 = beta == 0 ? (txi == 0 ? 1 : 0) : (txi == 0 ? 2 : 0), kx1 = beta == 0 ? (txi == 0 ? 2 : 0) : (txi == 0 ? 2 : 1);
-        const float* src = w + (static_cast<int64_t>(co) * cin + ci) * 9;
-        float v = 0.f;
-        for (int ky = ky0; ky <= ky1; ++ky)
-            for (int kx = kx0; kx <= kx1; ++kx) v += src[ky * 3 + kx];
-        out[static_cast<int64_t>(ph * cout + co) * pitch + tap * cin + ci] = v;
-    }
-}
-
 __global__ void __launch_bounds__(256) finalize_partial_kernel(const float* __restrict__ partial, int64_t split_stride, int ksplit,
                                                                int64_t pns, int plane, const float* __restrict__ bias,
                                                                float* __restrict__ out, int64_t out_ns, double* out_sums,
@@ -510,6 +474,12 @@
 
 constexpr int kBlocks = 2 * kLevels + 1, kDense = kBlocks * kLayers;
 
+struct BwdWeightForms {
+    bool dgrad_wino;
+    int layout1_blocks;
+    int tu_subpix_levels;
+};
+
 enum class DenseFwd { Wino4, Wino2_32x16, Wino2_32x8, SplitK, Direct32x8, Direct16x8, DirectAuto };
 struct FwdPlan {
     struct Dense {
@@ -522,6 +492,8 @@
     bool fuse_final;
     bool td_persistent[kLevels];
     bool tu_subpix[kLevels];
+    bool prepares_bwd;
+    BwdWeightForms bwd_weights;
 };
 
 enum class NewMap { Bf16, Persistent, Vec16, Dword };
@@ -690,6 +662,8 @@
     p.out_sums = c.out_sums(next, oc0);
     return p;
 }
+
+static BwdWeightForms bwd_weight_forms(const Ctx& c);
 
 static FwdPlan plan_fwd(const Ctx& c) {
     const int* opt = c.net->opt;
@@ -730,6 +704,12 @@
         pl.td_persistent[l] = (opt[ENDO_OPT_TD_PERSIST] & 2) && !pl.bf16 && c.training && td_fwd_ok(td_fwd_params(c, l));
         const ConvP& tu = table().tu_conv[kLevels - 1 - l];
         pl.tu_subpix[l] = c.net->lv[l + 1].w % 4 == 0 && tu.cout == kNew && tu.cin % 4 == 0;
+    }
+    pl.prepares_bwd = c.training != 0;
+    if (pl.prepares_bwd) {
+        Ctx cb = c;
+        cb.gradws = c.tape;
+        pl.bwd_weights = bwd_weight_forms(cb);
     }
     return pl;
 }
@@ -797,9 +777,7 @@
     ProfScope prof(kProfConv3x3Up, c.stream, conv_flops(c.net, level, cv.cin, cv.cout, 3),
                    4.0 * c.nt() * c.net->lv[level].plane * (cv.cin / 4.0 + cv.cout));
     if (c.fwd->tu_subpix[level]) {
-        float* w3 = c.tape + c.net->partial_off;
-        tu_phase_weights_kernel<<<(2 * cv.cin * 384 + 255) / 256, 256, 0, c.stream>>>(c.params + cv.w, cv.cout, cv.cin, w3);
-        ENDO_LAUNCH_CHECK();
+        const float* w3 = c.tape + c.net->tu_phase_off[level];
         ConvParams p{};
         fill_grid(c, p, src_level);
         fill_in(c, p, c.act(src_level), src_level, src_c0, cv.cin);
@@ -986,9 +964,37 @@
     return p;
 }
 
+static BasePass base_pass_form(const Ctx& c, int b) {
+    const int* opt = c.net->opt;
+    const int wino_dgrad = opt[ENDO_OPT_WINO_DGRAD];
+    const DenseBlock k = dense_block(b);
+    const auto& lv = c.net->lv[k.level];
+    const DgradBlockParams base = base_pass_params(c, k);
+    const long wtiles = static_cast<long>(lv.w / 32) * (lv.h / 8) * c.nt() * chip_divisor(c.net);
+    if ((bf16_mask(opt) & 4) != 0) return BasePass::Block8Bf16;
+    if (wino_dgrad != 0 && dgrad_wino_ok(base) && wtiles >= opt[ENDO_OPT_WINO_MIN_TILES])
+        return !((wino_dgrad == 1 || wino_dgrad == 3) && dgrad_wino3_ok(base)) ? BasePass::Wino8
+             : (wino_dgrad == 3 && dgrad_wino3p_applies(base)) ? BasePass::Wino3Persistent : BasePass::Wino3;
+    return BasePass::Block8;
+}
+static bool base_pass_layout1(BasePass base) { return base == BasePass::Wino3 || base == BasePass::Wino3Persistent; }
+static bool dgrad_wino_weights_wanted(const int* opt) { return opt[ENDO_OPT_WINO_DGRAD] != 0 && (bf16_mask(opt) & 4) == 0; }
+static bool tu_dgrad_subpix(const endo_net* net, int l) {
+    const ConvP& tu = table().tu_conv[kLevels - 1 - l];
+    return net->lv[l + 1].w % 4 == 0 && tu.cin == kNew && tu.cout == kNew;
+}
+
+static BwdWeightForms bwd_weight_forms(const Ctx& c) {
+    BwdWeightForms f{};
+    f.dgrad_wino = dgrad_wino_weights_wanted(c.net->opt);
+    if (f.dgrad_wino)
+        for (int b = 0; b < kBlocks; ++b) f.layout1_blocks |= base_pass_layout1(base_pass_form(c, b)) ? 1 << b : 0;
+    for (int l = 0; l < kLevels; ++l) f.tu_subpix_levels |= tu_dgrad_subpix(c.net, l) ? 1 << l : 0;
+    return f;
+}
+
 static BwdPlan plan_bwd(const Ctx& c) {
     const int* opt = c.net->opt;
-    const int wino_dgrad = opt[ENDO_OPT_WINO_DGRAD];
     const long min_tiles = opt[ENDO_OPT_WINO_MIN_TILES];
     BwdPlan pl{};
     pl.overlap = opt[ENDO_OPT_WGRAD_OVERLAP];
@@ -997,20 +1003,14 @@
     const bool f34 = opt[ENDO_OPT_WGRAD_F34] && !pl.bf16_wgrad;
     const long fill = chip_divisor(c.net);
     const long f34_min_tiles = (min_tiles / 4 + fill - 1) / fill;
-    pl.dgrad_weights = wino_dgrad != 0 && !pl.bf16_dgrad;
+    pl.dgrad_weights = dgrad_wino_weights_wanted(opt);
     for (int b = 0; b < kBlocks; ++b) {
         const DenseBlock k = dense_block(b);
-        const auto& lv = c.net->lv[k.level];
         BwdPlan::Block& bl = pl.block[b];
         const DgradBlockParams base = base_pass_params(c, k);
         bl.fused = dgrad_block_ok(base);
-        const long wtiles = static_cast<long>(lv.w / 32) * (lv.h / 8) * c.nt() * fill;
-        if (pl.bf16_dgrad) bl.base = BasePass::Block8Bf16;
-        else if (wino_dgrad != 0 && dgrad_wino_ok(base) && wtiles >= min_tiles)
-            bl.base = !((wino_dgrad == 1 || wino_dgrad == 3) && dgrad_wino3_ok(base)) ? BasePass::Wino8
-                    : (wino_dgrad == 3 && dgrad_wino3p_applies(base)) ? BasePass::Wino3Persistent : BasePass::Wino3;
-        else bl.base = BasePass::Block8;
-        bl.wino3_layout = bl.base == BasePass::Wino3 || bl.base == BasePass::Wino3Persistent;
+        bl.base = base_pass_form(c, b);
+        bl.wino3_layout = base_pass_layout1(bl.base);
         for (int j = 1; j < kLayers; ++j) {
             const DgradBlockParams p = newmap_params(c, k, j);
             const bool vec = dgrad_block_vec_ok(p);
@@ -1030,9 +1030,8 @@
         const bool persist = (opt[ENDO_OPT_TD_PERSIST] & 1) && !pl.bf16_dgrad;
         pl.td_dgrad[l] = (persist && td_dgrad_ok(td)) ? TdDgrad::Persistent : (persist && sv.w % 4 != 0 && td_dgrad_small_ok(td)) ? TdDgrad::Runs128
                        : sv.w % 4 == 0 ? TdDgrad::Dma : TdDgrad::Staged;
-        const ConvP& tu = table().tu_conv[kLevels - 1 - l];
         pl.tu_wgrad[l] = tu_wgrad_subpix_ok(tu_wgrad_params(c, l, true)) ? TuWgrad::Subpix : wgrad_taps_ok(tu_wgrad_params(c, l, false), true) ? TuWgrad::Taps : TuWgrad::Direct;
-        pl.tu_dgrad[l] = !(sv.w % 4 == 0 && tu.cin == kNew && tu.cout == kNew) ? TuDgrad::Plain : tile_count(c, l + 1, 32, 8) >= 1024 ? TuDgrad::Subpix32x8
+        pl.tu_dgrad[l] = !tu_dgrad_subpix(c.net, l) ? TuDgrad::Plain : tile_count(c, l + 1, 32, 8) >= 1024 ? TuDgrad::Subpix32x8
                        : tile_count(c, l + 1, 16, 8) >= 512 ? TuDgrad::Subpix16x8 : TuDgrad::Subpix16x4;
     }
     const BwdPlan::Block& last = pl.block[kBlocks - 1];
@@ -1161,7 +1160,7 @@
         if (virt) { p.vg = fv->vg; p.vw = fv->vw + ic0; }
         ProfScope prof(kProfDgradDense, c.stream, 2.0 * c.nt() * lv.plane * c0 * kGrowth * 9 * kLayers,
                        4.0 * c.nt() * lv.plane * (3.0 * c0 + kGrowth * kLayers));
-        const float* ub = c.gradws + c.net->wd_off;
+        const float* ub = c.tape + c.net->dgrad_wino_off;
         const float* const u[4] = {ub + k.cv[0].ud, ub + k.cv[1].ud, ub + k.cv[2].ud, ub + k.cv[3].ud};
         int rc = 0;
         switch (bl.base) {
@@ -1253,9 +1252,7 @@
         fill_out(c, p, c.gbuf(src_level), src_level, src_c0, cv.cin);
         return launch_conv_dma_auto<3, 4, 3, IN_PLAIN, EPI_DGRAD_SUMPOOL, 4>(p, c.stream);
     }
-    float* wd = c.gradws + c.net->tuw_scratch_off;
-    tu_subpix_dgrad_weights_kernel<<<(16 * cv.cout * cv.cin + 255) / 256, 256, 0, c.stream>>>(c.params + cv.w, cv.cout, cv.cin, wd);
-    ENDO_LAUNCH_CHECK();
+    const float* wd = c.tape + c.net->tu_subpix_off[level];
     ConvParams p{};
     fill_grid(c, p, src_level);
     fill_in(c, p, c.gbuf(level), level, 0, 4 * cv.cout);
@@ -1265,6 +1262,46 @@
     if (form == TuDgrad::Subpix32x8) return launch_conv_dma_vec<3, 8, 3, IN_SUBPIX, EPI_FWD, 2, 4, 2, 1, 1>(p, c.stream);
     if (form == TuDgrad::Subpix16x8) return launch_conv_dma_vec<3, 8, 3, IN_SUBPIX, EPI_FWD, 1, 2, 2, 1, 1>(p, c.stream);
     return launch_conv_dma_vec<3, 8, 3, IN_SUBPIX, EPI_FWD, 1, 1, 2, 1, 1>(p, c.stream);
+}
+
+static int launch_weight_prep(const Ctx& c, const FwdPlan* fwd, const BwdWeightForms* bwd, bool zero_sums) {
+    const Table& tb = table();
+    const endo_net* net = c.net;
+    const int64_t base = net->wino_off;
+    WeightPrepTable t{};
+    bool ok = true;
+    if (fwd && !fwd->bf16) {
+        const WinoWeightTable& w = tb.wino;
+        for (int l = 0; l < w.layers; ++l)
+            ok = ok && weight_prep_add(t, kPrepWinoFwd, w.cin[l], w.cout[l], fwd->dense[l].chunk_weights ? 1 : 0, w.w_off[l], w.u_off[l]);
+        if (fwd->wino4_weights)
+            for (int l = 0; l < w.layers; ++l)
+                ok = ok && weight_prep_add(t, kPrepWino4Fwd, w.cin[l], w.cout[l], 0, w.w_off[l], net->wino4_off - base + tb.wino4.u_off[l]);
+    }
+    if (fwd)
+        for (int l = 0; l < kLevels; ++l) {
+            const ConvP& tu = tb.tu_conv[kLevels - 1 - l];
+            if (fwd->tu_subpix[l]) ok = ok && weight_prep_add(t, kPrepTuPhase, tu.cin, tu.cout, 0, tu.w, net->tu_phase_off[l] - base);
+        }
+    if (bwd && bwd->dgrad_wino) {
+        const WinoDgradTable& w = tb.wino_dgrad;
+        for (int l = 0; l < w.layers; ++l)
+            ok = ok && weight_prep_add(t, kPrepDgradWino, w.cin[l], w.groups[l], (bwd->layout1_blocks >> (l / kLayers)) & 1, w.w_off[l],
+                                       net->dgrad_wino_off - base + w.u_off[l]);
+    }
+    if (bwd)
+        for (int l = 0; l < kLevels; ++l) {
+            const ConvP& tu = tb.tu_conv[kLevels - 1 - l];
+            if ((bwd->tu_subpix_levels >> l) & 1) ok = ok && weight_prep_add(t, kPrepTuSubpixDgrad, tu.cin, tu.cout, 0, tu.w, net->tu_subpix_off[l] - base);
+        }
+    if (!ok) return ENDO_E_UNSUPPORTED;
+    const int sums_count = zero_sums ? static_cast<int>(net->sums_bytes / 8) : 0;
+    const int blocks = t.blocks + (sums_count * net->groups + kWeightPrepThreads - 1) / kWeightPrepThreads;
+    if (blocks == 0) return 0;
+    ProfScope prof(kProfSmall, c.stream, 0.0, 8.0 * t.blocks * kWeightPrepThreads);
+    weight_prep_kernel<<<blocks, kWeightPrepThreads, 0, c.stream>>>(t, c.params, c.tape + base, zero_sums ? c.sums(0) : nullptr, sums_count, net->gs / 2, net->groups);
+    ENDO_LAUNCH_CHECK();
+    return 0;
 }
 
 static int64_t align_up(int64_t v, int64_t a) { return (v + a - 1) / a * a; }
@@ -1281,6 +1318,7 @@
     net->n = n; net->h = h; net->w = w; net->groups = groups;
     net->wstream = nullptr; net->ev_fork = nullptr; net->ev_join = nullptr;
     net->last_fwd = nullptr; net->last_bwd = nullptr;
+    for (auto& pr : net->prepared) pr = {nullptr, false, 0, 0};
     default_options(net->opt);
     int64_t off = 0, sums = 0, pq = 0;
     for (int l = 0; l <= kLevels; ++l) {
@@ -1309,6 +1347,17 @@
     byte_off += align_up(tb.wino_floats * 4, 256);
     net->wino4_off = byte_off / 4;
     byte_off += align_up(tb.wino4_floats * 4, 256);
+    for (int l = 0; l < kLevels; ++l) {
+        net->tu_phase_off[l] = byte_off / 4;
+        byte_off += align_up(tu_phase_weight_floats(tb.tu_conv[kLevels - 1 - l].cin) * 4, 256);
+    }
+    net->dgrad_wino_off = byte_off / 4;
+    byte_off += align_up(tb.wino_dgrad_floats * 4, 256);
+    for (int l = 0; l < kLevels; ++l) {
+        const ConvP& tu = tb.tu_conv[kLevels - 1 - l];
+        net->tu_subpix_off[l] = byte_off / 4;
+        byte_off += align_up(tu_subpix_dgrad_weight_floats(tu.cout, tu.cin) * 4, 256);
+    }
     net->tape_floats = byte_off / 4;
     net->pq_off = acts;
     net->pq_floats = 2 * pq;
@@ -1316,9 +1365,7 @@
     net->slot_stride = align_up(tb.bn_width_total * 2, 32);
     net->scratch_bytes = net->slot_stride * 8 * kBnSlots;
     net->wg_scratch_off = (net->scratch_off + align_up(net->scratch_bytes, 256)) / 4;
-    net->tuw_scratch_off = net->wg_scratch_off + std::max(std::max(kNsScratchFloats, kSpScratchFloats), 4 * kF34ScratchFloats);
-    net->wd_off = align_up(net->tuw_scratch_off + 4 * kNew * (4 * kNew + 16), 64);
-    net->gplane_off = align_up(net->wd_off + tb.wino_dgrad_floats, 64);
+    net->gplane_off = align_up(net->wg_scratch_off + std::max(std::max(kNsScratchFloats, kSpScratchFloats), 4 * kF34ScratchFloats), 64);
     net->bias_parts_off = net->gplane_off + align_up(static_cast<int64_t>(n) * h * w, 64);
     net->bias_parts_floats = static_cast<int64_t>(kBiasPartChannels) * n * groups * 32;
     {
@@ -1405,18 +1452,16 @@
     c.fwd = &plan;
     if (!net->last_fwd) net->last_fwd = new (std::nothrow) FwdPlan;
     if (net->last_fwd) *net->last_fwd = plan;
-    for (int g = 0; g < net->groups; ++g)
-        ENDO_CHECK(hipMemsetAsync(reinterpret_cast<char*>(tape + g * net->gs) + net->sums_off, 0, net->sums_bytes, c.stream));
-    if (!plan.bf16) {
-        ProfScope prof(kProfSmall, c.stream, 0.0, 4.0 * (tb.wino_floats + tb.wino_floats * 9 / 16));
-        WinoWeightTable wt = tb.wino;
-        for (int l = 0; l < wt.layers; ++l) wt.mode[l] = plan.dense[l].chunk_weights ? 1 : 0;
-        wino_fwd_weights_kernel<<<(wt.start[wt.layers] + 255) / 256, 256, 0, c.stream>>>(wt, params, tape + net->wino_off);
-        ENDO_LAUNCH_CHECK();
-        if (plan.wino4_weights) wino4_fwd_weights_kernel<<<(tb.wino4.start[tb.wino4.layers] + 255) / 256, 256, 0, c.stream>>>(tb.wino4, params, tape + net->wino4_off);
-        ENDO_LAUNCH_CHECK();
-    }
-    int rc;
+    int rc = launch_weight_prep(c, &plan, plan.prepares_bwd ? &plan.bwd_weights : nullptr, true);
+    if (rc) return rc;
+    {
+        endo_net::Prepared* pr = net->prepared;
+        int at = kPreparedTapes - 1;
+        for (int i = 0; i < kPreparedTapes; ++i) if (pr[i].tape == tape) { at = i; break; }
+        for (int i = at; i > 0; --i) pr[i] = pr[i - 1];
+        pr[0] = {tape, false, 0, 0};
+        if (plan.prepares_bwd) pr[0] = {tape, plan.bwd_weights.dgrad_wino, plan.bwd_weights.layout1_blocks, plan.bwd_weights.tu_subpix_levels};
+    }
     {
         ConvParams p{};
         fill_grid(c, p, 0);
@@ -1478,14 +1523,26 @@
     for (int g = 0; g < net->groups; ++g)
         ENDO_CHECK(hipMemsetAsync(gradws + g * net->gs + net->pq_off, 0,
                                   static_cast<size_t>(net->scratch_off + net->scratch_bytes - net->pq_off * 4), c.stream));
-    if (plan.dgrad_weights) {
-        ProfScope prof(kProfSmall, c.stream, 0.0, 4.0 * 2.0 * tb.wino_dgrad_floats);
-        int layout1_blocks = 0;
-        for (int b = 0; b < kBlocks; ++b) layout1_blocks |= plan.block[b].wino3_layout ? 1 << b : 0;
-        dgrad_wino_weights_kernel<<<(tb.wino_dgrad.start[tb.wino_dgrad.layers] + 255) / 256, 256, 0, c.stream>>>(tb.wino_dgrad, params, gradws + net->wd_off, layout1_blocks);
-        ENDO_LAUNCH_CHECK();
-    }
     int rc;
+    {
+        BwdWeightForms want{};
+        want.dgrad_wino = plan.dgrad_weights;
+        for (int b = 0; b < kBlocks; ++b) want.layout1_blocks |= (plan.dgrad_weights && plan.block[b].wino3_layout) ? 1 << b : 0;
+        for (int l = 0; l < kLevels; ++l) want.tu_subpix_levels |= plan.tu_dgrad[l] != TuDgrad::Plain ? 1 << l : 0;
+        endo_net::Prepared* have = nullptr;
+        for (auto& pr : net->prepared) if (pr.tape == tape) { have = &pr; break; }
+        const bool fresh = have && (!want.dgrad_wino || (have->dgrad_wino && have->layout1_blocks == want.layout1_blocks)) &&
+                           (want.tu_subpix_levels & ~have->tu_subpix_levels) == 0;
+        if (!fresh) {
+            rc = launch_weight_prep(c, nullptr, &want, false);
+            if (rc) return rc;
+            if (!have) {
+                for (int i = kPreparedTapes - 1; i > 0; --i) net->prepared[i] = net->prepared[i - 1];
+                have = net->prepared;
+            }
+            *have = {tape, want.dgrad_wino, want.layout1_blocks, want.tu_subpix_levels};
+        }
+    }
     const FinalVirt virt{gradws + net->gplane_off, params + tb.final_.w, grads + tb.final_.w};
     {
         const auto& lv = net->lv[0];
diff --git a/endoscopydepthestimation-pytorch_amd/csrc/weight_prep_kernels.h b/endoscopydepthestimation-pytorch_amd/csrc/weight_prep_kernels.h
--- /dev/null
+++ b/endoscopydepthestimation-pytorch_amd/csrc/weight_prep_kernels.h
@@ -0,0 +1,122 @@
+#pragma once
+
+#include "wino_fwd_kernels.h"
+#include "wino4_fwd_kernels.h"
+#include "dgrad_wino_kernels.h"
+
+namespace endo {
+
+constexpr int kTuPhaseStride = 2 * 12 * 16 + 16;
+__device__ __forceinline__ void tu_phase_weights_item(const float* __restrict__ w, int cout, int cin, float* __restrict__ out, int i) {
+    const int lane16 = i & 15;
+    const int slot = (i >> 4) % 12;
+    const int t = (i / (16 * 12)) & 1;
+    const int ci = (i / (16 * 12 * 2)) % cin;
+    const int a = i / (16 * 12 * 2 * cin);
+    int ctap, tile;
+    if (slot < 3) { ctap = 0; tile = slot; } else if (slot < 9) { ctap = 1; tile = slot - 3; } else { ctap = 2; tile = slot - 9 + 3; }
+    const int b = tile / 3, co = (tile % 3) * 16 + lane16;
+    float v = 0.f;
+    if (co < cout) {
+        const float* src = w + (static_cast<int64_t>(co) * cin + ci) * 9;
+        const int ky0 = a == 0 ? (t == 0 ? 0 : 1) : (t == 0 ? 0 : 2), ky1 = a == 0 ? (t == 0 ? 0 : 2) : (t == 0 ? 1 : 2);
+        int kx0, kx1;
+        if (b == 0) { kx0 = ctap == 0 ? 0 : 1; kx1 = ctap == 0 ? 0 : 2; }
+        else { kx0 = ctap == 1 ? 0 : 2; kx1 = ctap == 1 ? 1 : 2; }
+        for (int ky = ky0; ky <= ky1; ++ky)
+            for (int kx = kx0; kx <= kx1; ++kx) v += src[ky * 3 + kx];
+    }
+    out[(static_cast<int64_t>(a) * cin + ci) * kTuPhaseStride + (t * 12 + slot) * 16 + lane16] = v;
+}
+inline int64_t tu_phase_weight_floats(int cin) { return 2ll * cin * kTuPhaseStride; }
+
+__device__ __forceinline__ void tu_subpix_dgrad_weights_item(const float* __restrict__ w, int cout, int cin, float* __restrict__ out, int i) {
+    const int pitch = 4 * cin + 16;
+    const int ci = i % cin;
+    const int tap = (i / cin) & 3;
+    const int co = (i / (4 * cin)) % cout;
+    const int ph = i / (4 * cin * cout);
+    const int alpha = ph >> 1, beta = ph & 1, tyi = tap >> 1, txi = tap & 1;
+    const int ky0 = alpha == 0 ? (tyi == 0 ? 1 : 0) : (tyi == 0 ? 2 : 0), ky1 = alpha == 0 ? (tyi == 0 ? 2 : 0) : (tyi == 0 ? 2 : 1);
+    const int kx0 = beta == 0 ? (txi == 0 ? 1 : 0) : (txi == 0 ? 2 : 0), kx1 = beta == 0 ? (txi == 0 ? 2 : 0) : (txi == 0 ? 2 : 1);
+    const float* src = w + (static_cast<int64_t>(co) * cin + ci) * 9;
+    float v = 0.f;
+    for (int ky = ky0; ky <= ky1; ++ky)
+        for (int kx = kx0; kx <= kx1; ++kx) v += src[ky * 3 + kx];
+    out[static_cast<int64_t>(ph * cout + co) * pitch + tap * cin + ci] = v;
+}
+inline int64_t tu_subpix_dgrad_weight_floats(int cout, int cin) { return 4ll * cout * (4 * cin + 16); }
+
+enum WeightPrepKind : unsigned char {
+    kPrepWinoFwd,
+    kPrepWino4Fwd,
+    kPrepTuPhase,
+    kPrepDgradWino,
+    kPrepTuSubpixDgrad,
+};
+constexpr int kWeightPrepMaxJobs = 144;
+constexpr int kWeightPrepThreads = 256;
+
+struct WeightPrepTable {
+    int jobs;
+    int blocks;
+    struct Job {
+        int block0;
+        int w_off;
+        int dst_off;
+        short cin;
+        unsigned char kind, n2, flag, pad;
+    } job[kWeightPrepMaxJobs];
+};
+static_assert(sizeof(WeightPrepTable) + 64 <= 4096, "the table travels as a kernel argument");
+
+__host__ __device__ inline int weight_prep_items(int kind, int cin, int n2) {
+    switch (kind) {
+        case kPrepWinoFwd: case kPrepWino4Fwd: return cin * 16;
+        case kPrepTuPhase: return 2 * cin * 2 * 12 * 16;
+        case kPrepDgradWino: return 16 * n2 * 12;
+        default: return 4 * n2 * 4 * cin;
+    }
+}
+
+inline bool weight_prep_add(WeightPrepTable& t, int kind, int cin, int n2, int flag, int64_t w_off, int64_t dst_off) {
+    if (t.jobs >= kWeightPrepMaxJobs || w_off > 0x7fffffff || dst_off > 0x7fffffff || n2 > 255) return false;
+    WeightPrepTable::Job& j = t.job[t.jobs++];
+    j.block0 = t.blocks;
+    j.w_off = static_cast<int>(w_off); j.dst_off = static_cast<int>(dst_off);
+    j.cin = static_cast<short>(cin);
+    j.kind = static_cast<unsigned char>(kind); j.n2 = static_cast<unsigned char>(n2); j.flag = static_cast<unsigned char>(flag); j.pad = 0;
+    t.blocks += (weight_prep_items(kind, cin, n2) + kWeightPrepThreads - 1) / kWeightPrepThreads;
+    return true;
+}
+
+__global__ void __launch_bounds__(kWeightPrepThreads) weight_prep_kernel(const WeightPrepTable t, const float* __restrict__ params, float* __restrict__ prepared,
+                                                                         double* __restrict__ sums, int sums_count, int64_t group_stride, int groups) {
+    const int block = blockIdx.x;
+    if (block >= t.blocks) {
+        const int i = (block - t.blocks) * kWeightPrepThreads + threadIdx.x;
+        if (sums && i < sums_count * groups) {
+            const int g = i / sums_count;
+            sums[g * group_stride + (i - g * sums_count)] = 0.0;
+        }
+        return;
+    }
+    int lo = 0, hi = t.jobs - 1;
+    while (lo < hi) {
+        const int mid = (lo + hi + 1) >> 1;
+        if (t.job[mid].block0 <= block) lo = mid; else hi = mid - 1;
+    }
+    const WeightPrepTable::Job& j = t.job[lo];
+    const int kind = j.kind, cin = j.cin, n2 = j.n2;
+    const int e = (block - j.block0) * kWeightPrepThreads + threadIdx.x;
+    if (e >= weight_prep_items(kind, cin, n2)) return;
+    switch (kind) {
+        case kPrepWinoFwd: wino_fwd_weights_item(params, prepared, cin, n2, j.w_off, j.dst_off, j.flag, e); break;
+        case kPrepWino4Fwd: wino4_fwd_weights_item(params, prepared, cin, n2, j.w_off, j.dst_off, e); break;
+        case kPrepTuPhase: tu_phase_weights_item(params + j.w_off, n2, cin, prepared + j.dst_off, e); break;
+        case kPrepDgradWino: dgrad_wino_weights_item(params, prepared, cin, j.w_off, j.dst_off, j.flag != 0, e); break;
+        default: tu_subpix_dgrad_weights_item(params + j.w_off, n2, cin, prepared + j.dst_off, e); break;
+    }
+}
+
+}
diff --git a/endoscopydepthestimation-pytorch_amd/csrc/wino4_fwd_kernels.h b/endoscopydepthestimation-pytorch_amd/csrc/wino4_fwd_kernels.h
--- a/endoscopydepthestimation-pytorch_amd/csrc/wino4_fwd_kernels.h
+++ b/endoscopydepthestimation-pytorch_amd/csrc/wino4_fwd_kernels.h
@@ -16,50 +16,53 @@
 
 constexpr int kW4UStride = 576;
 
+__device__ __forceinline__ void wino4_fwd_weights_item(const float* __restrict__ params, float* __restrict__ u, int cin, int cout, int64_t w_off, int64_t u_off, int e) {
+    const int ci = e >> 4, j = e & 15;
+    float g[3][3];
+#pragma unroll
+    for (int a = 0; a < 3; ++a)
+#pragma unroll
+        for (int b = 0; b < 3; ++b) g[a][b] = 0.f;
+    if (j < cout) {
+        const float* src = params + w_off + (static_cast<int64_t>(j) * cin + ci) * 9;
+#pragma unroll
+        for (int a = 0; a < 3; ++a)
+#pragma unroll
+            for (int b = 0; b < 3; ++b) g[a][b] = src[a * 3 + b];
+    }
+    auto gt = [](float a, float b, float c, float (&o)[6]) {
+        const float ea = fmaf(kW4A2, c, a), eb = fmaf(kW4B2, c, a);
+        o[0] = kW4N0 * a;
+        o[1] = kW4NA * fmaf(kW4A, b, ea);
+        o[2] = kW4NA * fmaf(-kW4A, b, ea);
+        o[3] = kW4NB * fmaf(kW4B, b, eb);
+        o[4] = kW4NB * fmaf(-kW4B, b, eb);
+        o[5] = c;
+    };
+    float h[6][3];
+#pragma unroll
+    for (int b = 0; b < 3; ++b) {
+        float o[6];
+        gt(g[0][b], g[1][b], g[2][b], o);
+#pragma unroll
+        for (int i = 0; i < 6; ++i) h[i][b] = o[i];
+    }
+    float* dst = u + u_off + static_cast<int64_t>(ci) * kW4UStride + j * 12;
+#pragma unroll
+    for (int i = 0; i < 6; ++i) {
+        float o[6];
+        gt(h[i][0], h[i][1], h[i][2], o);
+#pragma unroll
+        for (int jj = 0; jj < 6; ++jj) dst[(i >> 1) * 192 + (i & 1) * 6 + jj] = o[jj];
+    }
+}
+
 __global__ void __launch_bounds__(256) wino4_fwd_weights_kernel(const WinoWeightTable t, const float* __restrict__ params, float* __restrict__ u) {
     const int total = t.start[t.layers];
     for (int item = blockIdx.x * blockDim.x + threadIdx.x; item < total; item += gridDim.x * blockDim.x) {
         int l = 0;
         while (item >= t.start[l + 1]) ++l;
-        const int e = item - t.start[l];
-        const int ci = e >> 4, j = e & 15;
-        float g[3][3];
-#pragma unroll
-        for (int a = 0; a < 3; ++a)
-#pragma unroll
-            for (int b = 0; b < 3; ++b) g[a][b] = 0.f;
-        if (j < t.cout[l]) {
-            const float* src = params + t.w_off[l] + (static_cast<int64_t>(j) * t.cin[l] + ci) * 9;
-#pragma unroll
-            for (int a = 0; a < 3; ++a)
-#pragma unroll
-                for (int b = 0; b < 3; ++b) g[a][b] = src[a * 3 + b];
-        }
-        auto gt = [](float a, float b, float c, float (&o)[6]) {
-            const float ea = fmaf(kW4A2, c, a), eb = fmaf(kW4B2, c, a);
-            o[0] = kW4N0 * a;
-            o[1] = kW4NA * fmaf(kW4A, b, ea);
-            o[2] = kW4NA * fmaf(-kW4A, b, ea);
-            o[3] = kW4NB * fmaf(kW4B, b, eb);
-            o[4] = kW4NB * fmaf(-kW4B, b, eb);
-            o[5] = c;
-        };
-        float h[6][3];
-#pragma unroll
-        for (int b = 0; b < 3; ++b) {
-            float o[6];
-            gt(g[0][b], g[1][b], g[2][b], o);
-#pragma unroll
-            for (int i = 0; i < 6; ++i) h[i][b] = o[i];
-        }
-        float* dst = u + t.u_off[l] + static_cast<int64_t>(ci) * kW4UStride + j * 12;
-#pragma unroll
-        for (int i = 0; i < 6; ++i) {
-            float o[6];
-            gt(h[i][0], h[i][1], h[i][2], o);
-#pragma unroll
-            for (int jj = 0; jj < 6; ++jj) dst[(i >> 1) * 192 + (i & 1) * 6 + jj] = o[jj];
-        }
+        wino4_fwd_weights_item(params, u, t.cin[l], t.cout[l], t.w_off[l], t.u_off[l], item - t.start[l]);
     }
 }
 
diff --git a/endoscopydepthestimation-pytorch_amd/csrc/wino_fwd_kernels.h b/endoscopydepthestimation-pytorch_amd/csrc/wino_fwd_kernels.h
--- a/endoscopydepthestimation-pytorch_amd/csrc/wino_fwd_kernels.h
+++ b/endoscopydepthestimation-pytorch_amd/csrc/wino_fwd_kernels.h
@@ -18,55 +18,59 @@
 };
 constexpr int kDenseChunkFloats = 9 * 16 * 16;
 
+__device__ __forceinline__ void wino_fwd_weights_item(const float* __restrict__ params, float* __restrict__ u, int cin, int cout, int64_t w_off, int64_t u_off,
+                                                      int mode, int e) {
+    const int ci = e >> 4, j = e & 15;
+    float g[3][3];
+#pragma unroll
+    for (int a = 0; a < 3; ++a)
+#pragma unroll
+        for (int b = 0; b < 3; ++b) g[a][b] = 0.f;
+    if (j < cout) {
+        const float* src = params + w_off + (static_cast<int64_t>(j) * cin + ci) * 9;
+#pragma unroll
+        for (int a = 0; a < 3; ++a)
+#pragma unroll
+            for (int b = 0; b < 3; ++b) g[a][b] = src[a * 3 + b];
+    }
+    if (mode == 1) {
+        float* dst = u + u_off + static_cast<int64_t>(ci >> 4) * kDenseChunkFloats + (ci & 15) * 16 + j;
+#pragma unroll
+        for (int tap = 0; tap < 9; ++tap) dst[tap * 256] = g[tap / 3][tap % 3];
+        if (ci == cin - 1)
+            for (int cz = (ci & 15) + 1; cz < 16; ++cz)
+#pragma unroll
+                for (int tap = 0; tap < 9; ++tap) dst[tap * 256 + (cz - (ci & 15)) * 16] = 0.f;
+        return;
+    }
+    float h[4][3];
+#pragma unroll
+    for (int b = 0; b < 3; ++b) {
+        h[0][b] = g[0][b];
+        h[1][b] = 0.5f * (g[0][b] + g[1][b] + g[2][b]);
+        h[2][b] = 0.5f * (g[0][b] - g[1][b] + g[2][b]);
+        h[3][b] = g[2][b];
+    }
+    float* dst = u + u_off + static_cast<int64_t>(ci) * kWinoUStride + j;
+#pragma unroll
+    for (int a = 0; a < 4; ++a) {
+        dst[(4 * a + 0) * 16] = h[a][0];
+        dst[(4 * a + 1) * 16] = 0.5f * (h[a][0] + h[a][1] + h[a][2]);
+        dst[(4 * a + 2) * 16] = 0.5f * (h[a][0] - h[a][1] + h[a][2]);
+        dst[(4 * a + 3) * 16] = h[a][2];
+    }
+    if (j == 0) {
+#pragma unroll
+        for (int k = 0; k < 16; ++k) dst[256 + k] = 0.f;
+    }
+}
+
 __global__ void __launch_bounds__(256) wino_fwd_weights_kernel(const WinoWeightTable t, const float* __restrict__ params, float* __restrict__ u) {
     const int total = t.start[t.layers];
     for (int item = blockIdx.x * blockDim.x + threadIdx.x; item < total; item += gridDim.x * blockDim.x) {
         int l = 0;
         while (item >= t.start[l + 1]) ++l;
-        const int e = item - t.start[l];
-        const int ci = e >> 4, j = e & 15;
-        float g[3][3];
-#pragma unroll
-        for (int a = 0; a < 3; ++a)
-#pragma unroll
-            for (int b = 0; b < 3; ++b) g[a][b] = 0.f;
-        if (j < t.cout[l]) {
-            const float* src = params + t.w_off[l] + (static_cast<int64_t>(j) * t.cin[l] + ci) * 9;
-#pragma unroll
-            for (int a = 0; a < 3; ++a)
-#pragma unroll
-                for (int b = 0; b < 3; ++b) g[a][b] = src[a * 3 + b];
-        }
-        if (t.mode[l] == 1) {
-            float* dst = u + t.u_off[l] + static_cast<int64_t>(ci >> 4) * kDenseChunkFloats + (ci & 15) * 16 + j;
-#pragma unroll
-            for (int tap = 0; tap < 9; ++tap) dst[tap * 256] = g[tap / 3][tap % 3];
-            if (ci == t.cin[l] - 1)
-                for (int cz = (ci & 15) + 1; cz < 16; ++cz)
-#pragma unroll
-                    for (int tap = 0; tap < 9; ++tap) dst[tap * 256 + (cz - (ci & 15)) * 16] = 0.f;
-            continue;
-        }
-        float h[4][3];
-#pragma unroll
-        for (int b = 0; b < 3; ++b) {
-            h[0][b] = g[0][b];
-            h[1][b] = 0.5f * (g[0][b] + g[1][b] + g[2][b]);
-            h[2][b] = 0.5f * (g[0][b] - g[1][b] + g[2][b]);
-            h[3][b] = g[2][b];
-        }
-        float* dst = u + t.u_off[l] + static_cast<int64_t>(ci) * kWinoUStride + j;
-#pragma unroll
-        for (int a = 0; a < 4; ++a) {
-            dst[(4 * a + 0) * 16] = h[a][0];
-            dst[(4 * a + 1) * 16] = 0.5f * (h[a][0] + h[a][1] + h[a][2]);
-            dst[(4 * a + 2) * 16] = 0.5f * (h[a][0] - h[a][1] + h[a][2]);
-            dst[(4 * a + 3) * 16] = h[a][2];
-        }
-        if (j == 0) {
-#pragma unroll
-            for (int k = 0; k < 16; ++k) dst[256 + k] = 0.f;
-        }
+        wino_fwd_weights_item(params, u, t.cin[l], t.cout[l], t.w_off[l], t.u_off[l], t.mode[l], item - t.start[l]);
     }
 }
 
```

Result: no change. 515.9, median of 6 (+0.4%).
